# RchalYang/torchrl

Measured on AMD Instinct MI355X. Metric: env_steps_per_sec_ppo_2048env_halfcheetah_shape, higher is better.
Workload: dtype f32

## Files before the change

torchrl_amd/build.py:

```python
import os
import shutil
import subprocess
import sys

HERE = os.path.dirname(os.path.abspath(__file__))
CSRC = os.path.join(HERE, "csrc")
LIB_DIR = os.path.join(HERE, "lib")
LIB = os.path.join(LIB_DIR, "libtrl_hip.so")
NOISE_LIB = os.path.join(LIB_DIR, "libtrl_noise.so")
NOISE_SRC = "trl_noise_ext.cpp"
SOURCES = ["trl_host.cpp", "trl_mtjump.cpp", "k_gae.hip", "k_gather.hip", "k_ppo.hip", "k_ppo_generic.hip", "k_categorical.hip", "k_gauss_sd.hip", "k_layernorm.hip", "k_vmpo.hip", "k_trpo.hip", "k_rollout.hip", "k_gemm.hip", "k_mlp3.hip", "k_conv1.hip", "k_conv_dx.hip", "k_sac.hip", "k_conv.hip", "k_dqn.hip", "k_bootdqn.hip", "k_norm.hip", "k_frames.hip", "k_comm.hip", "k_peaks.hip"]
FLAGS = ["--offload-arch=gfx950", "-O3", "-std=c++17", "-fPIC", "-fno-gpu-rdc", "-Wall",
         "-Wno-unused-function", "-Wno-unused-variable"]


def _stale():
    if not os.path.exists(LIB):
        return True
    t = os.path.getmtime(LIB)
    deps = [os.path.join(CSRC, f) for f in os.listdir(CSRC) if f != NOISE_SRC]
    deps.append(os.path.join(os.path.dirname(HERE), "include", "trl_hip.h"))
    return any(os.path.getmtime(d) > t for d in deps)


def noise_helper_tag():
    import torch
    return "%s abi%d" % (torch.__version__, int(torch.compiled_with_cxx11_abi()))


def noise_helper_built_for(path=None):
    import re
    try:
        with open(path or NOISE_LIB, "rb") as f:
            blob = f.read()
    except OSError:
        return None
    m = re.search(rb"(\d+\.\d+[^\x00 ]* abi[01])\x00", blob)
    return m.group(1).decode() if m else None


def build_noise_helper(force=False, verbose=True):
    src = os.path.join(CSRC, NOISE_SRC)
    if not force and os.path.exists(NOISE_LIB) and os.path.getmtime(NOISE_LIB) >= os.path.getmtime(src) \
            and noise_helper_built_for() == noise_helper_tag():
        return NOISE_LIB
    try:
        import torch
        from torch.utils import cpp_extension as ce
        gxx = shutil.which("g++")
        if gxx is None:
            raise RuntimeError("g++ not found")
        libp = ce.library_paths()
        cmd = [gxx, "-O2", "-std=c++17", "-shared", "-fPIC"] + ["-I" + i for i in ce.include_paths()] + \
              ["-D_GLIBCXX_USE_CXX11_ABI=%d" % int(torch.compiled_with_cxx11_abi()),
               '-DTRL_NOISE_BUILT_FOR="%s"' % noise_helper_tag(), src, "-o", NOISE_LIB] + \
              ["-L" + p for p in libp] + ["-ltorch_cpu", "-lc10"] + ["-Wl,-rpath," + p for p in libp]
        os.makedirs(LIB_DIR, exist_ok=True)
        res = subprocess.run(cmd, stdout=subprocess.PIPE, stderr=subprocess.STDOUT)
        if res.returncode != 0:
            raise RuntimeError(res.stdout.decode()[-2000:])
        if verbose:
            print("built", NOISE_LIB)
        return NOISE_LIB
    except Exception as exc:
        if verbose:
            print("libtrl_noise.so not built (%s): the reference-noise chunks are drawn from Python threads" % (exc,))
        return None


def build(force=False, verbose=True, extra_flags=(), lib=None):
    LIB = lib or globals()["LIB"]
    FLAGS = globals()["FLAGS"] + list(extra_flags)
    if not lib:
        build_noise_helper(force=force, verbose=verbose)
    if not force and not lib and not _stale():
        return LIB
    hipcc = shutil.which("hipcc") or "/opt/rocm/bin/hipcc"
    if not os.path.exists(hipcc):
        raise RuntimeError("hipcc not found: libtrl_hip.so cannot be built")
    os.makedirs(LIB_DIR, exist_ok=True)
    objs = []
    procs = []
    for src in SOURCES:
        obj = os.path.join(LIB_DIR, os.path.splitext(src)[0] + (".exp.o" if lib else ".o"))
        cmd = [hipcc] + FLAGS + (["-x", "hip"] if src.endswith(".cpp") else []) + \
              ["-c", os.path.join(CSRC, src), "-o", obj]
        procs.append((src, subprocess.Popen(cmd, stdout=subprocess.PIPE, stderr=subprocess.STDOUT)))
        objs.append(obj)
    for src, p in procs:
        out, _ = p.communicate()
        if p.returncode != 0:
            raise RuntimeError("hipcc failed on %s:\n%s" % (src, out.decode()))
        if verbose and out.strip():
            print(out.decode())
    cmd = [hipcc, "--offload-arch=gfx950", "-shared", "-fPIC", "-o", LIB] + objs + ["-ldl"]
    subprocess.check_call(cmd)
    for o in objs:
        os.remove(o)
    if verbose:
        print("built", LIB)
    return LIB


if __name__ == "__main__":
    if "--exp" in sys.argv:
        k = sys.argv.index("--exp")
        build(force=True, extra_flags=sys.argv[k + 2:], lib=os.path.join(LIB_DIR, "libtrl_hip_%s.so" % sys.argv[k + 1]))
    else:
        build(force="--force" in sys.argv)
```

torchrl_amd/csrc/k_gae.hip:

```cpp
#include "trl_common.h"

#define ENV_TILE 8
#define T_CHUNK 256
#define GAE_THREADS 256

template <int MODE>
__global__ __launch_bounds__(GAE_THREADS) void gae_scan_kernel(
    const float* __restrict__ rew, const float* __restrict__ val, const float* __restrict__ term,
    const float* __restrict__ tl, const float* __restrict__ last_v, const float* __restrict__ last_t, float* __restrict__ adv,
    float* __restrict__ ret, int T, int N, float gamma, float tau, int tl_filter) {
  constexpr int LDT = T_CHUNK + 1;
  __shared__ float s_a[ENV_TILE * LDT];
  __shared__ float s_c[ENV_TILE * LDT];
  __shared__ float s_carry[ENV_TILE];

  const int tid = threadIdx.x, lane = tid & 63, wave = tid >> 6;
  const int G = gridDim.x, xcd = blockIdx.x & 7, q = blockIdx.x >> 3;
  int first = 0;
  for (int y = 0; y < xcd; ++y) first += (G - y + 7) >> 3;
  const int n0 = (first + q) * ENV_TILE;
  const int e_ld = tid % ENV_TILE, t_ld = tid / ENV_TILE;
  const int n_ld = n0 + e_ld;

  __shared__ float s_lastv[ENV_TILE];
  if (tid < ENV_TILE) {
    float lv = 0.0f;
    if (n0 + tid < N) lv = last_v[n0 + tid] * (last_t ? 1.0f - last_t[n0 + tid] : 1.0f);
    s_lastv[tid] = lv;
    s_carry[tid] = (MODE == 0) ? 0.0f : lv;
  }

  for (int t_hi = T; t_hi > 0; t_hi -= T_CHUNK) {
    const int t_lo = max(0, t_hi - T_CHUNK);
    const int len = t_hi - t_lo;
    __syncthreads();
    constexpr int TPT = T_CHUNK / (GAE_THREADS / ENV_TILE);
    float lr[TPT], lv[TPT], ld[TPT], ltl[TPT], lvn[TPT];
#pragma unroll
    for (int q = 0; q < TPT; ++q) {
      const int tt = t_ld + q * (GAE_THREADS / ENV_TILE);
      const int t = t_lo + tt;
      const bool ok = tt < len && n_ld < N;
      const size_t i = ok ? (size_t)t * N + n_ld : 0;
      lr[q] = ok ? rew[i] : 0.0f;
      lv[q] = ok ? val[i] : 0.0f;
      ld[q] = ok ? term[i] : 0.0f;
      ltl[q] = (ok && tl_filter) ? tl[i] : 0.0f;
      lvn[q] = (MODE == 0 && ok && t + 1 < T) ? val[i + N] : 0.0f;
    }
#pragma unroll
    for (int q = 0; q < TPT; ++q) {
      const int tt = t_ld + q * (GAE_THREADS / ENV_TILE);
      if (tt < len) {
        const int t = t_lo + tt;
        float a = 0.f, c = 0.f;
        if (n_ld < N) {
          const float r = lr[q], v = lv[q], nd = 1.0f - ld[q];
          const float tlv = ltl[q];
          if (MODE == 0) {
            const float vn = (t + 1 < T) ? lvn[q] : s_lastv[e_ld];
            const float f = 1.0f - tlv;
            a = (r + nd * gamma * vn - v) * f;
            c = nd * gamma * tau * f;
          } else {
            a = r + tlv * v;
            c = nd * gamma * (1.0f - tlv);
          }
        }
        s_a[e_ld * LDT + tt] = a;
        s_c[e_ld * LDT + tt] = c;
      }
    }
    __syncthreads();
    const int seg = (len + 63) >> 6;
    constexpr int EPW = ENV_TILE / (GAE_THREADS / 64);
    const int lo = min(lane * seg, len), hi = min(lo + seg, len);
    float fa[EPW], fb[EPW];
#pragma unroll
    for (int u = 0; u < EPW; ++u) {
      const float* pa = s_a + (wave + u * (GAE_THREADS / 64)) * LDT;
      const float* pc = s_c + (wave + u * (GAE_THREADS / 64)) * LDT;
      fa[u] = 0.f; fb[u] = 1.f;
      for (int t = hi - 1; t >= lo; --t) { fa[u] = pa[t] + pc[t] * fa[u]; fb[u] = pc[t] * fb[u]; }
    }
#pragma unroll
    for (int o = 1; o < 64; o <<= 1) {
      float a2[EPW], b2[EPW];
#pragma unroll
      for (int u = 0; u < EPW; ++u) { a2[u] = __shfl_down(fa[u], o, 64); b2[u] = __shfl_down(fb[u], o, 64); }
      if (lane + o < 64) {
#pragma unroll
        for (int u = 0; u < EPW; ++u) { fa[u] = fa[u] + fb[u] * a2[u]; fb[u] = fb[u] * b2[u]; }
      }
    }
#pragma unroll
    for (int u = 0; u < EPW; ++u) {
      const int e = wave + u * (GAE_THREADS / 64);
      float* pa = s_a + e * LDT;
      const float* pc = s_c + e * LDT;
      const float carry = s_carry[e];
      const float a_nx = __shfl_down(fa[u], 1, 64), b_nx = __shfl_down(fb[u], 1, 64);
      float y = (lane == 63) ? carry : (a_nx + b_nx * carry);
      for (int t = hi - 1; t >= lo; --t) { y = pa[t] + pc[t] * y; pa[t] = y; }
      const float y0 = __shfl(fa[u], 0, 64) + __shfl(fb[u], 0, 64) * carry;
      if (lane == 0) s_carry[e] = y0;
    }
    __syncthreads();
#pragma unroll
    for (int q = 0; q < TPT; ++q) {
      const int tt = t_ld + q * (GAE_THREADS / ENV_TILE);
      if (tt < len && n_ld < N) {
        const size_t i = (size_t)(t_lo + tt) * N + n_ld;
        const float y = s_a[e_ld * LDT + tt], v = lv[q];
        if (MODE == 0) { adv[i] = y; ret[i] = y + v; }
        else           { ret[i] = y; adv[i] = y - v; }
      }
    }
  }
}

static int launch_scan(int mode, const float* rew, const float* val, const float* term, const float* tl,
                       const float* last_v, const float* last_t, float* adv, float* ret, int T, int N,
                       float gamma, float tau, int tl_filter, void* stream) {
  if (!rew || !val || !term || !last_v || !adv || !ret) { trl_set_error("gae: null pointer"); return TRL_EINVAL; }
  if (tl_filter && !tl) { trl_set_error("gae: tl_filter set but time_limits is null"); return TRL_EINVAL; }
  if (T < 0 || N < 0) { trl_set_error("gae: negative size"); return TRL_EINVAL; }
  if (T == 0 || N == 0) return TRL_OK;
  dim3 grid(trl_ceil_div(N, ENV_TILE)), block(GAE_THREADS);
  hipStream_t s = (hipStream_t)stream;
  if (mode == 0)
    hipLaunchKernelGGL(gae_scan_kernel<0>, grid, block, 0, s, rew, val, term, tl, last_v, last_t, adv, ret, T, N, gamma, tau, tl_filter);
  else
    hipLaunchKernelGGL(gae_scan_kernel<1>, grid, block, 0, s, rew, val, term, tl, last_v, last_t, adv, ret, T, N, gamma, tau, tl_filter);
  TRL_LAUNCH_CHECK();
  return TRL_OK;
}

extern "C" int trl_gae_f32(const float* rewards, const float* values, const float* terminals,
                           const float* time_limits, const float* last_value, const float* last_terminal,
                           float* advs, float* rets, int T, int N, float gamma, float tau, int tl_filter,
                           void* stream) {
  return launch_scan(0, rewards, values, terminals, time_limits, last_value, last_terminal, advs, rets, T, N, gamma, tau, tl_filter, stream);
}

extern "C" int trl_discount_reward_f32(const float* rewards, const float* values, const float* terminals,
                                       const float* time_limits, const float* last_value,
                                       const float* last_terminal, float* advs, float* rets, int T, int N,
                                       float gamma, int tl_filter, void* stream) {
  return launch_scan(1, rewards, values, terminals, time_limits, last_value, last_terminal, advs, rets, T, N, gamma, 0.f, tl_filter, stream);
}
```

torchrl_amd/csrc/k_ppo.hip:

```cpp
#include <cstdlib>
#include "trl_common.h"
#include "trl_mlp.h"
#include "trl_head.h"
#include "trl_comm.h"

struct PpoDev {
  const float *obs, *acts, *advs, *rets, *old_values, *old_logp;
  const int64_t* row_idx;
  int rows_mb, N;
  const double* adv_raw;
  double n_global;
  const float *pf_params, *vf_params;
  float clip_para, entropy_coeff;
  int clipped_value_loss, tanh_action;
  int loss_mode;
  float* partial;
  double* scal_partial;
  int n_wg, n_pf, p_stride;
  int D, A;
};

template <int D, int H, int A> struct PpoShape {
  static_assert(H == 64 && D > 16 && D <= 32 && A <= 8, "instantiated for 16 < D <= 32, H == 64, A <= 8");
  static constexpr int P_PF = MlpFlat<D, H, A>::P_PF, P_VF = MlpFlat<D, H, 1>::P_VF;
  static constexpr int P_STRIDE = ((P_PF > P_VF ? P_PF : P_VF) + 63) & ~63;
};

#define WV_WAVES 4
#ifdef TRL_EXP_CLK
#define WCLK_DECL long long clk_prev = clock64(); float clk_acc[24]; for (int q_ = 0; q_ < 24; ++q_) clk_acc[q_] = 0.f;
#define WCLK(ph) { __builtin_amdgcn_sched_barrier(0); const long long c_ = clock64(); clk_acc[ph] += (float)(c_ - clk_prev); clk_prev = c_; __builtin_amdgcn_sched_barrier(0); }
#else
#define WCLK_DECL
#define WCLK(ph)
#endif
#define WV_THREADS (64 * WV_WAVES)
#define LDT 20
#define LDW 68

template <int D, int H, int A> struct WvShape {
  static_assert(H == 64 && (D == 17 || D == 32) && A <= 8, "instantiated for D == 17 / 32, H == 64, A <= 8");
  static constexpr int O_W2F = 0, O_W2B = H * LDW, O_B1 = 2 * H * LDW, O_B2 = O_B1 + H, O_SCR = O_B2 + H;
  static constexpr int O_H1 = 0, O_H2 = H * LDT, O_DZ2 = 2 * H * LDT, O_DO = 3 * H * LDT, WSCR = O_DO + 16 * LDT;
  static constexpr int P_STRIDE = PpoShape<D, H, A>::P_STRIDE;
  static constexpr int MAIN = O_SCR + WV_WAVES * WSCR;
  static constexpr int XS_W2 = 0, XS_W1 = 16, XS_W1B = 20, XS_W3 = D > 17 ? 24 : 20, XS_PF = XS_W3 + 4, XS_VF = XS_W3;
  static constexpr int XSC_PF = 3 * H + 32, XSC_VF = 4 * H + 16;
  static constexpr int XCH_PF = WV_WAVES * (XS_PF * 256 + XSC_PF), XCH_VF = WV_WAVES * (XS_VF * 256 + XSC_VF);
  static constexpr int XCH = XCH_PF > XCH_VF ? XCH_PF : XCH_VF;
  static constexpr int O_IMG = MAIN > XCH ? MAIN : XCH;
  static constexpr int IMG_HEAD = 8 * H + 16;
  static constexpr int IMG = (H * D + 2 * H + IMG_HEAD + WV_THREADS - 1) / WV_THREADS * WV_THREADS;
  static constexpr int LDS_FLOATS = O_IMG + IMG;
};

template <int D, int H, int A> struct WvShapeSD : WvShape<D, H, A> {
  static constexpr int P_PF_SD = H * D + H + H * H + H + 2 * A * H + 2 * A, P_VF = MlpFlat<D, H, 1>::P_VF;
  static constexpr int P_STRIDE = ((P_PF_SD > P_VF ? P_PF_SD : P_VF) + 63) & ~63;
  static constexpr int IMG_HEAD = 16 * H + 16;
  static constexpr int IMG = (H * D + 2 * H + IMG_HEAD + WV_THREADS - 1) / WV_THREADS * WV_THREADS;
  static constexpr int LDS_FLOATS = WvShape<D, H, A>::O_IMG + IMG;
};
template <int D, int H, int A, int HEAD> struct WvPick { using T = WvShape<D, H, A>; };
template <int D, int H, int A> struct WvPick<D, H, A, HEAD_SD> { using T = WvShapeSD<D, H, A>; };
#define SD_HALF_LOG_2PI_PLUS_HALF 1.4189385332046727f

__device__ __forceinline__ f32x4 lds4(const float* p) { return *reinterpret_cast<const f32x4*>(p); }
__device__ __forceinline__ float row_sum16(float v) {
  v += __builtin_bit_cast(float, __builtin_amdgcn_update_dpp(0, __builtin_bit_cast(int, v), 0x128, 0xF, 0xF, false));
  v += __builtin_bit_cast(float, __builtin_amdgcn_update_dpp(0, __builtin_bit_cast(int, v), 0x124, 0xF, 0xF, false));
  v += __builtin_bit_cast(float, __builtin_amdgcn_update_dpp(0, __builtin_bit_cast(int, v), 0x122, 0xF, 0xF, false));
  v += __builtin_bit_cast(float, __builtin_amdgcn_update_dpp(0, __builtin_bit_cast(int, v), 0x121, 0xF, 0xF, false));
  return v;
}

template <int D, int H, int A, int ACT, bool IS_PF, bool CONTIG, bool RT, int HEAD = HEAD_GAUSS>
__device__ void ppo_wave_pass(const PpoDev& a, float* lds, int wg_in_net, int n_wg_net) {
  using S = typename WvPick<D, H, A, HEAD>::T;
  constexpr bool WIDE = D > 17,
                 CAT = HEAD == HEAD_CAT, SD = HEAD == HEAD_SD,
                 SDP = SD && IS_PF;
  static_assert(!WIDE || RT, "the wide tile exists as a runtime-dims instantiation only");
  static_assert(!CAT || (IS_PF && RT), "the categorical head is a policy pass of the runtime-dims kernels");
  static_assert(!SD || RT, "the state-dependent-std head belongs to the runtime-dims kernels");
  constexpr int AS = CAT ? 1 : 0;
  const int Dr = RT ? a.D : D;
  const int O = IS_PF ? (RT ? a.A : A) : 1;
  const int OH = SDP ? 2 * O : O;
  const int F_W1 = 0, F_B1 = H * Dr, F_W2 = F_B1 + H, F_B2 = F_W2 + H * H, F_W3 = F_B2 + H, F_B3 = F_W3 + OH * H,
            F_LS = F_B3 + OH, F_END = (CAT || SDP) ? F_LS : F_LS + O;
  auto sd_has = [&](int o) -> bool { return (o & 7) < O; };
  auto sd_row = [&](int o) -> int { return o < 8 ? o : O + (o - 8); };
  const int PS = RT ? a.p_stride : S::P_STRIDE;
  const int tid = threadIdx.x, lane = tid & 63, wave = tid >> 6;
  const int j = lane & 15, g = lane >> 4, i = j;
  const float* gp = IS_PF ? a.pf_params : a.vf_params;
  WCLK_DECL
  float* W2F = lds + S::O_W2F;
  float* W2B = lds + S::O_W2B;
  float* scr = lds + S::O_SCR + wave * S::WSCR;
  float* H1S = scr + S::O_H1;
  float* H2S = scr + S::O_H2;
  float* DZ2S = scr + S::O_DZ2;
  float* DOS = scr + S::O_DO;

  const double adv_s1 = IS_PF ? a.adv_raw[0] : 0.0, adv_s2 = IS_PF ? a.adv_raw[1] : 0.0;
  const int B = a.rows_mb * a.N;
  const int n_tiles = (B + 15) / 16;
  const int tile_stride = n_wg_net * WV_WAVES;

  float xq[5], xtq[4], lq[6];
  float xq2[4], xtq2[4];
  int tile = wg_in_net * WV_WAVES + wave;
  const int tpr = a.N >> 4;
  int p1r = 0, p1c = 0, p2r = 0, p2c = 0, st_r = 0, st_c = 0;
  int64_t ridx1 = 0, ridx2 = 0;
  bool fv[4], fv2[4];
  const bool f16 = !WIDE && (!RT || Dr > 16), jv = !RT || i < Dr, jv2 = WIDE && 16 + i < Dr;
  const unsigned ox16 = (unsigned)(j * Dr + (f16 ? 16 : 0)) * 4u, os = (unsigned)j * 4u;
  unsigned oxq[4], oxt[4], oa_[4], oxq2[4], oxt2[4];
#pragma unroll
  for (int q = 0; q < 4; ++q) {
    fv[q] = !RT || 4 * g + q < Dr;
    fv2[q] = WIDE && 16 + 4 * g + q < Dr;
    oxq[q] = (unsigned)(j * Dr + (fv[q] ? 4 * g + q : 0)) * 4u;
    oxt[q] = (unsigned)((4 * g + q) * Dr + (jv ? i : 0)) * 4u;
    oxq2[q] = (unsigned)(j * Dr + (fv2[q] ? 16 + 4 * g + q : 0)) * 4u;
    oxt2[q] = (unsigned)((4 * g + q) * Dr + (jv2 ? 16 + i : 0)) * 4u;
    if constexpr (SDP) oa_[q] = (unsigned)(j * O + (4 * (g & 1) + q < O ? 4 * (g & 1) + q : 0)) * 4u;
    else oa_[q] = CAT ? (unsigned)j * 4u : (unsigned)(j * O + (4 * g + q < O ? 4 * g + q : 0)) * 4u;
  }
  auto ldb = [](const float* base, unsigned byte_off) -> float {
    return *reinterpret_cast<const float*>(reinterpret_cast<const char*>(base) + byte_off);
  };
  auto pos_advance = [&](int& r, int& c) { c += st_c; r += st_r; if (c >= tpr) { c -= tpr; ++r; } };
  auto load_ridx = [&](int r) -> int64_t {
    const int rr = r < a.rows_mb ? r : 0;
    return a.row_idx ? a.row_idx[rr] : (int64_t)rr;
  };
  auto fetch_contig = [&](int64_t ridx, int r, int c) {
    const int64_t cell0 = (r < a.rows_mb) ? ridx * a.N + 16 * c : 0;
    const float* ob = a.obs + cell0 * Dr;
#pragma unroll
    for (int q = 0; q < 4; ++q) xq[q] = ldb(ob, oxq[q]);
    xq[4] = ldb(ob, ox16);
#pragma unroll
    for (int q = 0; q < 4; ++q) xtq[q] = ldb(ob, oxt[q]);
    if constexpr (WIDE) {
#pragma unroll
      for (int q = 0; q < 4; ++q) { xq2[q] = ldb(ob, oxq2[q]); xtq2[q] = ldb(ob, oxt2[q]); }
    }
    if constexpr (IS_PF) {
      const float* ab = a.acts + cell0 * (CAT ? AS : O);
      if constexpr (CAT) { lq[0] = ldb(ab, oa_[0]); lq[1] = lq[2] = lq[3] = 0.0f; }
      else {
#pragma unroll
        for (int q = 0; q < 4; ++q) lq[q] = ldb(ab, oa_[q]);
      }
      lq[4] = ldb(a.advs + cell0, os);
      lq[5] = a.old_logp ? ldb(a.old_logp + cell0, os) : 0.0f;
    } else {
      lq[0] = lq[1] = lq[2] = lq[3] = 0.0f;
      lq[4] = ldb(a.rets + cell0, os);
      lq[5] = a.clipped_value_loss ? ldb(a.old_values + cell0, os) : 0.0f;
    }
  };
  auto row_of = [&](int smp, int& e) -> int { const int sm = smp < B ? smp : 0; const int r = sm / a.N; e = sm - r * a.N; return r; };
  auto fetch_inputs = [&](int64_t p, int s0) {
#pragma unroll
    for (int r = 0; r < 4; ++r) xq[r] = a.obs[p * Dr + (fv[r] ? 4 * g + r : 0)];
    xq[4] = a.obs[p * Dr + (f16 ? 16 : 0)];
#pragma unroll
    for (int q = 0; q < 4; ++q) {
      const int sj = 4 * g + q;
      const int64_t pr = __shfl(p, sj, 64);
      xtq[q] = a.obs[(s0 + sj < B ? pr : 0) * Dr + (jv ? i : 0)];
      if constexpr (WIDE) {
        xq2[q] = a.obs[p * Dr + (fv2[q] ? 16 + 4 * g + q : 0)];
        xtq2[q] = a.obs[(s0 + sj < B ? pr : 0) * Dr + (jv2 ? 16 + i : 0)];
      }
    }
    if constexpr (IS_PF) {
      if constexpr (CAT) { lq[0] = a.acts[p]; lq[1] = lq[2] = lq[3] = 0.0f; }
      else if constexpr (SDP) {
#pragma unroll
        for (int r = 0; r < 4; ++r) lq[r] = a.acts[p * O + (4 * (g & 1) + r < O ? 4 * (g & 1) + r : 0)];
      } else {
#pragma unroll
        for (int r = 0; r < 4; ++r) lq[r] = a.acts[p * O + (4 * g + r < O ? 4 * g + r : 0)];
      }
      lq[4] = a.advs[p]; lq[5] = a.old_logp ? a.old_logp[p] : 0.0f;
    } else {
      lq[0] = lq[1] = lq[2] = lq[3] = 0.0f;
      lq[4] = a.rets[p]; lq[5] = a.clipped_value_loss ? a.old_values[p] : 0.0f;
    }
  };
  int e_nn = 0;
  int64_t ridx_nn = 0;
  auto fetch_row = [&](int t) {
    const int r = row_of(t * 16 + j, e_nn);
    ridx_nn = a.row_idx ? a.row_idx[r] : (int64_t)r;
  };
  auto prefetch_next = [&](int nt) {
    if constexpr (CONTIG) {
      fetch_contig(ridx1, p1r, p1c);
      p1r = p2r; p1c = p2c; ridx1 = ridx2;
      pos_advance(p2r, p2c);
      ridx2 = load_ridx(p2r);
    } else {
      const int64_t pn = (nt * 16 + j < B) ? ridx_nn * a.N + e_nn : 0;
      fetch_inputs(pn, nt * 16);
      fetch_row(nt + tile_stride);
    }
  };
  int r0 = 0, c0 = 0;
  int64_t ridx0 = 0;
  if constexpr (CONTIG) {
    const int t0 = __builtin_amdgcn_readfirstlane(tile);
    const int ts = __builtin_amdgcn_readfirstlane(tile_stride);
    st_r = ts / tpr; st_c = ts - st_r * tpr;
    r0 = t0 / tpr; c0 = t0 - (t0 / tpr) * tpr;
    ridx0 = load_ridx(r0);
  } else {
    fetch_row(tile);
  }
  __builtin_amdgcn_sched_barrier(0);
  constexpr int NV = H * H / (4 * WV_THREADS);
  f32x4 wv[NV], wt[NV];
  const int tc = tid & 63, tq = tid >> 6;
  {
    static_assert(WV_THREADS == 256 && H == 64, "the transposed staging maps (column, 4 rows) onto 256 threads");
    const bool w2_al = !RT || ((reinterpret_cast<uintptr_t>(gp + F_W2) & 15) == 0);
#pragma unroll
    for (int t = 0; t < NV; ++t) {
      if (w2_al) wv[t] = *reinterpret_cast<const f32x4*>(gp + F_W2 + 4 * (tid + WV_THREADS * t));
      else {
#pragma unroll
        for (int x = 0; x < 4; ++x) wv[t][x] = gp[F_W2 + 4 * (tid + WV_THREADS * t) + x];
      }
    }
#pragma unroll
    for (int t = 0; t < NV; ++t)
#pragma unroll
      for (int x = 0; x < 4; ++x) wt[t][x] = gp[F_W2 + (4 * (tq + 4 * t) + x) * H + tc];
  }
  constexpr int NI = S::IMG / WV_THREADS;
  const int n_img = F_W2 + (F_END - F_B2);
  float im[NI];
#pragma unroll
  for (int k = 0; k < NI; ++k) {
    const int e = tid + WV_THREADS * k, ec = e < n_img ? e : n_img - 1;
    im[k] = gp[ec < F_W2 ? ec : ec + H * H];
  }
  __builtin_amdgcn_sched_barrier(0);
  if constexpr (CONTIG) {
    fetch_contig(ridx0, r0, c0);
    p1r = r0; p1c = c0;
    pos_advance(p1r, p1c);
    ridx1 = load_ridx(p1r);
    p2r = p1r; p2c = p1c;
    pos_advance(p2r, p2c);
    ridx2 = load_ridx(p2r);
  } else {
    const int64_t p0 = (tile * 16 + j < B) ? ridx_nn * a.N + e_nn : 0;
    fetch_inputs(p0, tile * 16);
    fetch_row(tile + tile_stride);
  }
#ifdef TRL_EXP_CLK
  WCLK(22)
  __builtin_amdgcn_s_waitcnt(0);
  WCLK(23)
#endif
  for (int e = lane; e < 16 * LDT; e += 64) DOS[e] = 0.0f;
#pragma unroll
  for (int t = 0; t < NV; ++t) {
    const int e = 4 * (tid + WV_THREADS * t), r = e / H, c = e - r * H;
    *reinterpret_cast<f32x4*>(W2F + r * LDW + c) = wv[t];
    *reinterpret_cast<f32x4*>(W2B + tc * LDW + 4 * (tq + 4 * t)) = wt[t];
  }
  float* img = lds + S::O_IMG;
  constexpr int KB_LO = H * (WIDE ? 18 : RT ? 2 : D) / WV_THREADS, KB_HI = (H * D + 2 * H - 1) / WV_THREADS;
#pragma unroll
  for (int k = 0; k < NI; ++k) {
    const int e = tid + WV_THREADS * k;
    img[e] = im[k];
    if (k >= KB_LO && k <= KB_HI && e >= F_B1 && e < F_B1 + 2 * H) lds[S::O_B1 + (e - F_B1)] = im[k];
  }
  static_assert(S::O_B2 == S::O_B1 + H, "b1 | b2 are stored as one run");
  __syncthreads();

  const int I_W3 = F_W3 - H * H, I_B3 = F_B3 - H * H, I_LS = F_LS - H * H;
  float w1[4][5], w3h[4][4], w3t[4][4];
  float w1b[4][4];
  float b3v[4], lsraw[4];
#pragma unroll
  for (int so = 0; so < 4; ++so) {
    const int row = 16 * so + i;
#pragma unroll
    for (int r = 0; r < 4; ++r) w1[so][r] = img[F_W1 + row * Dr + (fv[r] ? 4 * g + r : 0)];
    w1[so][4] = img[F_W1 + row * Dr + (f16 ? 16 : 0)];
    if constexpr (WIDE) {
#pragma unroll
      for (int r = 0; r < 4; ++r) w1b[so][r] = img[F_W1 + row * Dr + (fv2[r] ? 16 + 4 * g + r : 0)];
    }
#pragma unroll
    for (int r = 0; r < 4; ++r) {
      const int o = 4 * g + r;
      if constexpr (SDP) {
        w3h[so][r] = img[I_W3 + (sd_has(i) ? sd_row(i) : 0) * H + 16 * so + 4 * g + r];
        w3t[so][r] = img[I_W3 + (sd_has(o) ? sd_row(o) : 0) * H + row];
      } else if constexpr (IS_PF) {
        w3h[so][r] = img[I_W3 + (i < O ? i : 0) * H + 16 * so + 4 * g + r];
        w3t[so][r] = img[I_W3 + (o < O ? o : 0) * H + row];
      } else {
        w3h[so][r] = img[I_W3 + 16 * so + 4 * g + r];
        w3t[so][r] = 0.0f;
      }
    }
  }
#pragma unroll
  for (int r = 0; r < 4; ++r) {
    const int o = 4 * g + r;
    if constexpr (IS_PF && !CAT && !SDP) lsraw[r] = img[I_LS + (o < O ? o : 0)];
    else lsraw[r] = 0.0f;
    if constexpr (SDP) b3v[r] = img[I_B3 + (sd_has(o) ? sd_row(o) : 0)];
    else b3v[r] = img[I_B3 + (o < O ? o : 0)];
  }
  const float vb3 = IS_PF ? 0.0f : img[I_B3];
  __builtin_amdgcn_sched_barrier(0);
#pragma unroll
  for (int so = 0; so < 4; ++so) {
#pragma unroll
    for (int r = 0; r < 4; ++r) {
      const int o = 4 * g + r;
      w1[so][r] = fv[r] ? w1[so][r] : 0.0f;
      if constexpr (WIDE) w1b[so][r] = fv2[r] ? w1b[so][r] : 0.0f;
      if constexpr (SDP) {
        w3h[so][r] = sd_has(i) ? w3h[so][r] : 0.0f;
        w3t[so][r] = sd_has(o) ? w3t[so][r] : 0.0f;
      } else if constexpr (IS_PF) {
        w3h[so][r] = (i < O) ? w3h[so][r] : 0.0f;
        w3t[so][r] = (o < O) ? w3t[so][r] : 0.0f;
      }
    }
    w1[so][4] = (g == 0 && f16) ? w1[so][4] : 0.0f;
  }
  float lsv[4], ivv[4], lspass[4];
#pragma unroll
  for (int r = 0; r < 4; ++r) {
    const int o = 4 * g + r;
    const float raw = (IS_PF && !CAT && !SDP && o < O) ? lsraw[r] : 0.0f;
    lsv[r] = fminf(fmaxf(raw, -20.0f), 2.0f);
    ivv[r] = __expf(-2.0f * lsv[r]);
    lspass[r] = (raw >= -20.0f && raw <= 2.0f) ? 1.0f : 0.0f;
    if constexpr (SDP) b3v[r] = sd_has(o) ? b3v[r] : 0.0f;
    else b3v[r] = (o < O) ? b3v[r] : 0.0f;
  }

  const double ng = a.n_global;
  const double adv_mean = adv_s1 / ng;
  const double adv_var = (adv_s2 - adv_s1 * adv_s1 / ng) / (ng - 1.0);
  const float adv_mu = (float)adv_mean;
  const float adv_rstd = 1.0f / ((float)sqrt(fmax(adv_var, 0.0)) + 1e-5f);
  const float inv_b = (float)(1.0 / ng);

  f32x4 gW2[4][4], gW1[4], gW3[4];
  f32x4 gW1b[4];
  float gb1[4][4], gb2[4][4], gW1c[4][4];
  float db3[4], dls[4], stv[7];
  float ent_sum = 0.0f;
  float sdst[8] = {0.0f, 0.0f, -INFINITY, -INFINITY, 0.0f, 0.0f, -INFINITY, -INFINITY}, sd_cnt = 0.0f;
#pragma unroll
  for (int x = 0; x < 4; ++x) {
    gW1[x] = gW3[x] = gW1b[x] = f32x4{0.f, 0.f, 0.f, 0.f};
    db3[x] = dls[x] = 0.0f;
#pragma unroll
    for (int y = 0; y < 4; ++y) { gW2[x][y] = f32x4{0.f, 0.f, 0.f, 0.f}; gb1[x][y] = gb2[x][y] = gW1c[x][y] = 0.0f; }
  }
#pragma unroll
  for (int k = 0; k < 7; ++k) stv[k] = (k >= 2 && k <= 5) ? -INFINITY : 0.0f;

  WCLK(0)
  for (; tile < n_tiles; tile += tile_stride) {
    const int s = tile * 16 + j;
    const bool valid = CONTIG ? true : (s < B);
    float xb[5], xt[4], lin[6], xb2[4], xt2[4];
#pragma unroll
    for (int r = 0; r < 4; ++r) xb[r] = (valid && fv[r]) ? xq[r] : 0.0f;
    xb[4] = (valid && f16) ? xq[4] : 0.0f;
#pragma unroll
    for (int q = 0; q < 4; ++q) xt[q] = (jv && (CONTIG || tile * 16 + 4 * g + q < B)) ? xtq[q] : 0.0f;
    if constexpr (WIDE) {
#pragma unroll
      for (int q = 0; q < 4; ++q) {
        xb2[q] = (valid && fv2[q]) ? xq2[q] : 0.0f;
        xt2[q] = (jv2 && (CONTIG || tile * 16 + 4 * g + q < B)) ? xtq2[q] : 0.0f;
      }
    }
#pragma unroll
    for (int q = 0; q < 6; ++q) lin[q] = lq[q];
    const float x16 = xb[4];

#define PIN_DS() __builtin_amdgcn_sched_barrier(0x676)
    f32x4 h1[4], h2[4];
    f32x4 wq[4], bq;
#pragma unroll
    for (int so = 0; so < 4; ++so) h1[so] = lds4(lds + S::O_B1 + 16 * so + 4 * g);
#pragma unroll
    for (int sl = 0; sl < 4; ++sl) wq[sl] = lds4(W2F + i * LDW + 16 * sl + 4 * g);
    bq = lds4(lds + S::O_B2 + 4 * g);
    PIN_DS();
    WCLK(9)
#pragma unroll
    for (int q = 0; q < (WIDE ? 4 : 5); ++q)
#pragma unroll
      for (int so = 0; so < 4; ++so) h1[so] = mfma16(w1[so][q], xb[q], h1[so]);
    if constexpr (WIDE) {
#pragma unroll
      for (int q = 0; q < 4; ++q)
#pragma unroll
        for (int so = 0; so < 4; ++so) h1[so] = mfma16(w1b[so][q], xb2[q], h1[so]);
    }
    WCLK(10)
#pragma unroll
    for (int so = 0; so < 4; ++so)
#pragma unroll
      for (int r = 0; r < 4; ++r) {
        h1[so][r] = act_fn<ACT>(h1[so][r]);
        H1S[(16 * so + 4 * g + r) * LDT + j] = h1[so][r];
      }
    WCLK(1)
#pragma unroll
    for (int so = 0; so < 4; ++so) {
      f32x4 acc = bq;
      f32x4 wc[4];
#pragma unroll
      for (int sl = 0; sl < 4; ++sl) wc[sl] = wq[sl];
      if (so < 3) {
#pragma unroll
        for (int sl = 0; sl < 4; ++sl) wq[sl] = lds4(W2F + (16 * (so + 1) + i) * LDW + 16 * sl + 4 * g);
        bq = lds4(lds + S::O_B2 + 16 * (so + 1) + 4 * g);
        PIN_DS();
      }
#pragma unroll
      for (int sl = 0; sl < 4; ++sl)
#pragma unroll
        for (int r = 0; r < 4; ++r) acc = mfma16(wc[sl][r], h1[sl][r], acc);
      WCLK(11)
#pragma unroll
      for (int r = 0; r < 4; ++r) h2[so][r] = act_fn<ACT>(acc[r]);
      WCLK(12)
    }

    prefetch_next(tile + tile_stride);
    WCLK(2)
    f32x4 dz2[4];
    f32x4 wb[4];
    if constexpr (IS_PF) {
#pragma unroll
      for (int so = 0; so < 4; ++so)
#pragma unroll
        for (int r = 0; r < 4; ++r) H2S[(16 * so + 4 * g + r) * LDT + j] = h2[so][r];
      f32x4 oa = f32x4{b3v[0], b3v[1], b3v[2], b3v[3]}, ob = f32x4{0.f, 0.f, 0.f, 0.f};
#pragma unroll
      for (int sl = 0; sl < 4; sl += 2)
#pragma unroll
        for (int r = 0; r < 4; ++r) { oa = mfma16(w3h[sl][r], h2[sl][r], oa); ob = mfma16(w3h[sl + 1][r], h2[sl + 1][r], ob); }
      WCLK(14)
      float zc[4], lp = 0.0f;
      float pk[4], lpk[4], ent = 0.0f;
      int ai = 0;
      if constexpr (CAT) {
        float lg[4], ek[4], m = -INFINITY;
#pragma unroll
        for (int r = 0; r < 4; ++r) {
          lg[r] = oa[r] + ob[r];
          m = (4 * g + r < O) ? fmaxf(m, lg[r]) : m;
        }
        m = fmaxf(m, __shfl_xor(m, 16, 64));
        m = g < 2 ? m : 0.0f;
#pragma unroll
        for (int r = 0; r < 4; ++r) ek[r] = (4 * g + r < O) ? expf(lg[r] - m) : 0.0f;
        const float c_own = ((ek[0] + ek[1]) + ek[2]) + ek[3];
        const float c_lo = __shfl_xor(c_own, 16, 64);
        float Ssum = g == 1 ? (((c_lo + ek[0]) + ek[1]) + ek[2]) + ek[3] : c_own;
        const float S_hi = __shfl_xor(Ssum, 16, 64);
        Ssum = g == 0 ? S_hi : (g == 1 ? Ssum : 1.0f);
        const float logS = logf(Ssum);
        ai = min(max((int)lin[0], 0), O - 1);
#pragma unroll
        for (int r = 0; r < 4; ++r) {
          const bool has = 4 * g + r < O;
          lpk[r] = has ? (lg[r] - m) - logS : 0.0f;
          pk[r] = ek[r] / Ssum;
          lp += (has && 4 * g + r == ai) ? lpk[r] : 0.0f;
          ent -= pk[r] * lpk[r];
        }
        lp += __shfl_xor(lp, 16, 64);
        ent += __shfl_xor(ent, 16, 64);
      } else if constexpr (SDP) {
#pragma unroll
        for (int r = 0; r < 4; ++r) {
          const bool has = 4 * (g & 1) + r < O;
          const float mine = oa[r] + ob[r], oth = __shfl_xor(mine, 32, 64);
          const float mean = g < 2 ? mine : oth, raw = g < 2 ? oth : mine;
          lsv[r] = fminf(fmaxf(raw, -20.0f), 2.0f);
          ivv[r] = __expf(-2.0f * lsv[r]);
          lspass[r] = (raw >= -20.0f && raw <= 2.0f) ? 1.0f : 0.0f;
          const float t = gauss_logp_term((valid && has) ? lin[r] : 0.0f, has ? mean : 0.0f, ivv[r], lsv[r], a.tanh_action, zc[r]);
          lp += has ? t : 0.0f;
          ent += has ? SD_HALF_LOG_2PI_PLUS_HALF + lsv[r] : 0.0f;
          zc[r] = has ? zc[r] : 0.0f;
        }
        lp += __shfl_xor(lp, 16, 64);
        ent += __shfl_xor(ent, 16, 64);
      } else {
#pragma unroll
      for (int r = 0; r < 4; ++r) {
        const bool has = 4 * g + r < O;
        const float t = gauss_logp_term((valid && has) ? lin[r] : 0.0f, has ? oa[r] + ob[r] : 0.0f, ivv[r], lsv[r],
                                        a.tanh_action, zc[r]);
        lp += has ? t : 0.0f;
        zc[r] = has ? zc[r] : 0.0f;
      }
      WCLK(18)
      lp += __shfl_xor(lp, 16, 64);
      }
      WCLK(19)
      const float advn = valid ? (lin[4] - adv_mu) * adv_rstd : 0.0f;
      float ratio, s1, s2, g_lp;
      if (a.loss_mode == TRL_LOSS_A2C) {
        ratio = 1.0f;
        s1 = s2 = lp * advn;
        g_lp = (valid && (SDP || g < 2)) ? -advn * inv_b : 0.0f;
      } else {
        ratio = __expf(lp - lin[5]);
        s1 = ratio * advn;
        s2 = fminf(fmaxf(ratio, 1.0f - a.clip_para), 1.0f + a.clip_para) * advn;
        g_lp = (valid && (SDP || g < 2) && s1 <= s2) ? -advn * ratio * inv_b : 0.0f;
      }
      WCLK(20)
      float dout[4];
      if constexpr (CAT) {
        const float ce = a.entropy_coeff * inv_b;
#pragma unroll
        for (int r = 0; r < 4; ++r) {
          const bool own = valid && g < 2 && 4 * g + r < O;
          dout[r] = own ? g_lp * ((4 * g + r == ai ? 1.0f : 0.0f) - pk[r]) + ce * pk[r] * (lpk[r] + ent) : 0.0f;
          db3[r] += dout[r];
          if (g < 2) DOS[(4 * g + r) * LDT + j] = dout[r];
        }
        if (valid && g == 0) ent_sum += ent;
      } else if constexpr (SDP) {
        const float ce = a.entropy_coeff * inv_b;
#pragma unroll
        for (int r = 0; r < 4; ++r) {
          const bool own = valid && 4 * (g & 1) + r < O;
          const float dm = g_lp * zc[r] * ivv[r], dr = lspass[r] * (g_lp * (zc[r] * zc[r] * ivv[r] - 1.0f) - ce);
          dout[r] = own ? (g < 2 ? dm : dr) : 0.0f;
          db3[r] += dout[r];
          DOS[(4 * g + r) * LDT + j] = dout[r];
          if (own && g < 2) {
            const float x = lsv[r], ex = expf(x);
            sdst[0] += x; sdst[1] = fmaf(x, x, sdst[1]); sdst[2] = fmaxf(sdst[2], x); sdst[3] = fmaxf(sdst[3], -x);
            sdst[4] += ex; sdst[5] = fmaf(ex, ex, sdst[5]); sdst[6] = fmaxf(sdst[6], ex); sdst[7] = fmaxf(sdst[7], -ex);
          }
        }
        if (valid && g == 0) { ent_sum += ent; sd_cnt += 1.0f; }
      } else {
#pragma unroll
      for (int r = 0; r < 4; ++r) {
        const bool own = valid && g < 2 && 4 * g + r < O;
        dout[r] = own ? g_lp * zc[r] * ivv[r] : 0.0f;
        db3[r] += dout[r];
        dls[r] += own ? lspass[r] * (g_lp * (zc[r] * zc[r] * ivv[r] - 1.0f) - a.entropy_coeff * inv_b) : 0.0f;
        if (g < 2) DOS[(4 * g + r) * LDT + j] = dout[r];
      }
      }
      WCLK(21)
      if (valid && g == 0) {
        stv[0] += lp; stv[1] = fmaf(lp, lp, stv[1]); stv[6] -= fminf(s1, s2);
        stv[2] = fmaxf(stv[2], lp); stv[3] = fmaxf(stv[3], -lp);
        stv[4] = fmaxf(stv[4], ratio); stv[5] = fmaxf(stv[5], -ratio);
      }
      WCLK(15)
      const f32x4 da = lds4(DOS + i * LDT + 4 * g);
      f32x4 hb3[4];
#pragma unroll
      for (int so = 0; so < 4; ++so) hb3[so] = lds4(H2S + (16 * so + j) * LDT + 4 * g);
#pragma unroll
      for (int so = 0; so < 4; ++so) wb[so] = lds4(W2B + (16 * so + i) * LDW + 4 * g);
      PIN_DS();
#pragma unroll
      for (int so = 0; so < 4; ++so) dz2[so] = f32x4{0.f, 0.f, 0.f, 0.f};
#pragma unroll
      for (int r = 0; r < 4; ++r)
#pragma unroll
        for (int so = 0; so < 4; ++so) dz2[so] = mfma16(w3t[so][r], dout[r], dz2[so]);
#pragma unroll
      for (int so = 0; so < 4; ++so)
#pragma unroll
        for (int q = 0; q < 4; ++q) gW3[so] = mfma16(da[q], hb3[so][q], gW3[so]);
      WCLK(16)
    } else {
#pragma unroll
      for (int so = 0; so < 4; ++so) wb[so] = lds4(W2B + (16 * so + i) * LDW + 4 * g);
      PIN_DS();
      float v = 0.0f;
#pragma unroll
      for (int so = 0; so < 4; ++so)
#pragma unroll
        for (int r = 0; r < 4; ++r) v = fmaf(w3h[so][r], h2[so][r], v);
      v += __shfl_xor(v, 16, 64);
      v += __shfl_xor(v, 32, 64);
      v += vb3;
      const float R = lin[4];
      float dv, l;
      if (a.clipped_value_loss) {
        const float vo = lin[5];
        const float dc = v - vo;
        const float vc = vo + fminf(fmaxf(dc, -a.clip_para), a.clip_para);
        const float l1 = (v - R) * (v - R), l2 = (vc - R) * (vc - R);
        const float wa = l1 > l2 ? 1.0f : (l1 == l2 ? 0.5f : 0.0f), wb_ = 1.0f - wa;
        const float pass = (dc >= -a.clip_para && dc <= a.clip_para) ? 1.0f : 0.0f;
        l = 0.5f * fmaxf(l1, l2);
        dv = inv_b * (wa * (v - R) + wb_ * pass * (vc - R));
      } else {
        l = (v - R) * (v - R);
        dv = 2.0f * (v - R) * inv_b;
      }
      dv = valid ? dv : 0.0f;
      if (valid && g == 0) {
        stv[6] += l; db3[0] += dv;
        stv[0] += v; stv[1] = fmaf(v, v, stv[1]); stv[2] = fmaxf(stv[2], v); stv[3] = fmaxf(stv[3], -v);
      }
#pragma unroll
      for (int so = 0; so < 4; ++so)
#pragma unroll
        for (int r = 0; r < 4; ++r) {
          dz2[so][r] = dv * w3h[so][r];
          gW3[so][r] = fmaf(dv, h2[so][r], gW3[so][r]);
        }
    }
#pragma unroll
    for (int so = 0; so < 4; ++so)
#pragma unroll
      for (int r = 0; r < 4; ++r) {
        dz2[so][r] *= act_grad<ACT>(h2[so][r]);
        gb2[so][r] += dz2[so][r];
        DZ2S[(16 * so + 4 * g + r) * LDT + j] = dz2[so][r];
      }

    WCLK(3)
    f32x4 dz1[4];
    f32x4 hb[4], za2;
#pragma unroll
    for (int so = 0; so < 4; ++so) dz1[so] = f32x4{0.f, 0.f, 0.f, 0.f};
#pragma unroll
    for (int sl = 0; sl < 4; ++sl) {
      f32x4 w[4];
#pragma unroll
      for (int so = 0; so < 4; ++so) w[so] = wb[so];
      if (sl < 3) {
#pragma unroll
        for (int so = 0; so < 4; ++so) wb[so] = lds4(W2B + (16 * so + i) * LDW + 16 * (sl + 1) + 4 * g);
      } else {
#pragma unroll
        for (int c = 0; c < 4; ++c) hb[c] = lds4(H1S + (16 * c + j) * LDT + 4 * g);
        za2 = lds4(DZ2S + i * LDT + 4 * g);
      }
      PIN_DS();
#pragma unroll
      for (int r = 0; r < 4; ++r)
#pragma unroll
        for (int so = 0; so < 4; ++so) dz1[so] = mfma16(w[so][r], dz2[sl][r], dz1[so]);
    }
    WCLK(17)
#pragma unroll
    for (int so = 0; so < 4; ++so)
#pragma unroll
      for (int r = 0; r < 4; ++r) {
        dz1[so][r] *= act_grad<ACT>(h1[so][r]);
        gb1[so][r] += dz1[so][r];
        if constexpr (!WIDE) gW1c[so][r] = fmaf(dz1[so][r], x16, gW1c[so][r]);
        H2S[(16 * so + 4 * g + r) * LDT + j] = dz1[so][r];
      }
    f32x4 za1[4];
#pragma unroll
    for (int so = 0; so < 4; ++so) za1[so] = lds4(H2S + (16 * so + i) * LDT + 4 * g);
    PIN_DS();

    WCLK(4)
#pragma unroll
    for (int so = 0; so < 4; ++so) {
      const f32x4 za = za2;
      if (so < 3) { za2 = lds4(DZ2S + (16 * (so + 1) + i) * LDT + 4 * g); PIN_DS(); }
#pragma unroll
      for (int q = 0; q < 4; ++q)
#pragma unroll
        for (int c = 0; c < 4; ++c) gW2[so][c] = mfma16(za[q], hb[c][q], gW2[so][c]);
    }
    WCLK(5)
#pragma unroll
    for (int so = 0; so < 4; ++so)
#pragma unroll
      for (int q = 0; q < 4; ++q) gW1[so] = mfma16(za1[so][q], xt[q], gW1[so]);
    if constexpr (WIDE) {
#pragma unroll
      for (int so = 0; so < 4; ++so)
#pragma unroll
        for (int q = 0; q < 4; ++q) gW1b[so] = mfma16(za1[so][q], xt2[q], gW1b[so]);
    }
#undef PIN_DS
    WCLK(6)
  }

  __syncthreads();
  const int wg = blockIdx.x;
  {
    constexpr int NS = IS_PF ? S::XS_PF : S::XS_VF, SC = IS_PF ? S::XSC_PF : S::XSC_VF;
    f32x4* xch = reinterpret_cast<f32x4*>(lds);
    float* xsc = lds + WV_WAVES * NS * 256;
    f32x4* xw = xch + (wave * NS) * 64 + lane;
    float* sw = xsc + wave * SC;
    {
      constexpr int NK = IS_PF ? 3 : 4, TS = 17;
      static_assert(NK * 16 <= 64 && NK * 16 * TS <= NS * 64, "one task per lane, inside the wave's own region");
      f32x4* tr = xch + (wave * NS) * 64;
#pragma unroll
      for (int so = 0; so < 4; ++so) {
        f32x4* te = tr + (4 * so + g) * TS + j;
        te[0] = f32x4{gb1[so][0], gb1[so][1], gb1[so][2], gb1[so][3]};
        te[16 * TS] = f32x4{gb2[so][0], gb2[so][1], gb2[so][2], gb2[so][3]};
        te[32 * TS] = f32x4{gW1c[so][0], gW1c[so][1], gW1c[so][2], gW1c[so][3]};
        if constexpr (!IS_PF) te[48 * TS] = gW3[so];
      }
      if (lane < NK * 16) {
        const f32x4* x = tr + lane * TS;
        const f32x4 even = ((x[0] + x[8]) + (x[4] + x[12])) + ((x[2] + x[10]) + (x[6] + x[14]));
        const f32x4 odd = ((x[1] + x[9]) + (x[5] + x[13])) + ((x[3] + x[11]) + (x[7] + x[15]));
        *reinterpret_cast<f32x4*>(sw + 4 * lane) = even + odd;
      }
    }
#pragma unroll
    for (int so = 0; so < 4; ++so) {
#pragma unroll
      for (int c = 0; c < 4; ++c) xw[(S::XS_W2 + 4 * so + c) * 64] = gW2[so][c];
      xw[(S::XS_W1 + so) * 64] = gW1[so];
      if constexpr (WIDE) xw[(S::XS_W1B + so) * 64] = gW1b[so];
      if constexpr (IS_PF) xw[(S::XS_W3 + so) * 64] = gW3[so];
    }
#pragma unroll
    for (int r = 0; r < 4; ++r) {
      const int o = 4 * g + r;
      const float b3 = row_sum16(db3[r]), dl = row_sum16(dls[r]);
      if (j == 0) {
        if constexpr (IS_PF) { sw[3 * H + o] = b3; sw[3 * H + 16 + o] = dl; }
        else sw[4 * H + o] = b3;
      }
    }
    WCLK(7)
    __syncthreads();
    float* prow = a.partial + (size_t)wg * a.p_stride;
    auto fold4 = [&](int slot) -> f32x4 {
      const f32x4* p = xch + slot * 64 + lane;
      f32x4 acc = p[0];
#pragma unroll
      for (int w = 1; w < WV_WAVES; ++w) acc += p[w * NS * 64];
      return acc;
    };
    {
      const int so = wave;
      f32x4 t2[4];
#pragma unroll
      for (int c = 0; c < 4; ++c) t2[c] = fold4(S::XS_W2 + 4 * so + c);
      const f32x4 t1 = fold4(S::XS_W1 + so);
      f32x4 t1b = f32x4{0.f, 0.f, 0.f, 0.f}, t3 = f32x4{0.f, 0.f, 0.f, 0.f};
      if constexpr (WIDE) t1b = fold4(S::XS_W1B + so);
      if constexpr (IS_PF) t3 = fold4(S::XS_W3 + so);
#pragma unroll
      for (int r = 0; r < 4; ++r) {
        const int f = 16 * so + 4 * g + r;
#pragma unroll
        for (int c = 0; c < 4; ++c) prow[F_W2 + f * H + 16 * c + j] = t2[c][r];
        if (jv) prow[F_W1 + f * Dr + j] = t1[r];
        if (WIDE && jv2) prow[F_W1 + f * Dr + 16 + j] = t1b[r];
        if constexpr (IS_PF) {
          const int o = 4 * g + r;
          if constexpr (SDP) { if (sd_has(o)) prow[F_W3 + sd_row(o) * H + 16 * so + j] = t3[r]; }
          else if (o < O) prow[F_W3 + o * H + 16 * so + j] = t3[r];
        }
      }
    }
    for (int k = tid; k < SC; k += WV_THREADS) {
      float acc = xsc[k];
#pragma unroll
      for (int w = 1; w < WV_WAVES; ++w) acc += xsc[w * SC + k];
      const int q = k & (H - 1);
      int dst = -1;
      if (k < H) dst = F_B1 + q;
      else if (k < 2 * H) dst = F_B2 + q;
      else if (k < 3 * H) { if (f16) dst = F_W1 + q * Dr + 16; }
      else if constexpr (IS_PF) {
        const int o = q & 15;
        if (q < 16) { if constexpr (SDP) { if (sd_has(o)) dst = F_B3 + sd_row(o); } else if (o < O) dst = F_B3 + o; }
        else if (!CAT && !SDP && o < O) dst = F_LS + o;
      } else {
        if (k < 4 * H) dst = F_W3 + q;
        else if (q < O) dst = F_B3 + q;
      }
      if (dst >= 0) prow[dst] = acc;
    }
    for (int e = (IS_PF ? F_END : F_LS) + tid; e < PS; e += WV_THREADS) prow[e] = 0.0f;
  }
  WCLK(8)
#ifdef TRL_EXP_CLK
  __syncthreads();
  if (tid == 0) for (int ph = 0; ph < 24; ++ph) a.partial[(size_t)wg * a.p_stride + PS - 40 + ph] = clk_acc[ph];
#endif
  __syncthreads();
  double* sred = reinterpret_cast<double*>(lds);
  {
    const bool own = g == 0;
    const double v0 = wave_sum(own ? (double)stv[0] : 0.0), v1 = wave_sum(own ? (double)stv[1] : 0.0),
                 v6 = wave_sum(own ? (double)stv[6] : 0.0);
    const float v2 = wave_max(own ? stv[2] : -INFINITY), v3 = wave_max(own ? stv[3] : -INFINITY),
                v4 = wave_max(own ? stv[4] : -INFINITY), v5 = wave_max(own ? stv[5] : -INFINITY);
    double v7 = 0.0;
    if constexpr (CAT || SDP) v7 = wave_sum(own ? (double)ent_sum : 0.0);
    if (lane == 0) {
      double* p = sred + wave * 8;
      p[0] = v0; p[1] = v1; p[2] = v2; p[3] = v3; p[4] = v4; p[5] = v5; p[6] = v6; p[7] = v7;
    }
    if constexpr (SDP) {
      double e[SD_SCAL];
#pragma unroll
      for (int k = 0; k < 8; ++k) e[k] = (k & 2) ? (double)wave_max(sdst[k]) : wave_sum((double)sdst[k]);
      e[8] = wave_sum((double)sd_cnt);
      if (lane == 0) {
#pragma unroll
        for (int k = 0; k < SD_SCAL; ++k) sred[WV_WAVES * 8 + wave * SD_SCAL + k] = k < 9 ? e[k] : 0.0;
      }
    }
  }
  __syncthreads();
  if (tid < 8) {
    double r = sred[tid];
    for (int w = 1; w < WV_WAVES; ++w) {
      const double o = sred[w * 8 + tid];
      r = (tid >= 2 && tid <= 5) ? fmax(r, o) : r + o;
    }
    a.scal_partial[(size_t)wg * 8 + tid] = r;
  }
  if constexpr (SDP) {
    if (tid >= 64 && tid < 64 + SD_SCAL) {
      const int k = tid - 64;
      double r = sred[WV_WAVES * 8 + k];
      for (int w = 1; w < WV_WAVES; ++w) {
        const double o = sred[WV_WAVES * 8 + w * SD_SCAL + k];
        r = (k < 8 && (k & 2)) ? fmax(r, o) : r + o;
      }
      a.scal_partial[(size_t)a.n_wg * 8 + (size_t)wg * SD_SCAL + k] = r;
    }
  }
}

#define RED_CHUNK 64
#ifndef RED_WAVES
#define RED_WAVES 8
#endif
#ifndef RED_DEPTH
#define RED_DEPTH 16
#endif
__device__ __forceinline__ float fold_chain_tree(float (&acc)[RED_DEPTH]) {
#pragma unroll
  for (int st = RED_DEPTH / 2; st > 0; st >>= 1)
#pragma unroll
    for (int k = 0; k < st; ++k) acc[k] += acc[k + st];
  return acc[0];
}
__device__ __forceinline__ float fold_rows_wave(const float* __restrict__ src, int nrow, int p_stride, int w, bool in_range) {
  float acc[RED_DEPTH];
#pragma unroll
  for (int k = 0; k < RED_DEPTH; ++k) acc[k] = 0.0f;
  if (in_range) {
    for (; w < nrow; w += RED_DEPTH * RED_WAVES) {
      float v[RED_DEPTH];
#pragma unroll
      for (int k = 0; k < RED_DEPTH; ++k) v[k] = (w + RED_WAVES * k < nrow) ? src[(size_t)(w + RED_WAVES * k) * p_stride] : 0.0f;
#pragma unroll
      for (int k = 0; k < RED_DEPTH; ++k) acc[k] += v[k];
    }
  }
  return fold_chain_tree(acc);
}
__device__ __forceinline__ float fold_waves_tree(const float (*s_acc)[RED_CHUNK], int lane) {
  float t4[RED_WAVES / 4];
#pragma unroll
  for (int q = 0; q < RED_WAVES / 4; ++q)
    t4[q] = (s_acc[4 * q][lane] + s_acc[4 * q + 1][lane]) + (s_acc[4 * q + 2][lane] + s_acc[4 * q + 3][lane]);
  float gval = t4[0];
#pragma unroll
  for (int q = 1; q < RED_WAVES / 4; ++q) gval += t4[q];
  return gval;
}
__device__ __noinline__ void fold_scalar_stats(const double* __restrict__ base, int nrow, int net, int lane,
                                                  double* __restrict__ info) {
  double v[7];
#pragma unroll
  for (int k = 0; k < 7; ++k) v[k] = (k >= 2 && k <= 5) ? -INFINITY : 0.0;
  for (int w0 = 0; w0 < nrow; w0 += 192) {
    double o[3][7];
#pragma unroll
    for (int q = 0; q < 3; ++q) {
      const int w = w0 + lane + 64 * q;
#pragma unroll
      for (int k = 0; k < 7; ++k) {
        double x = (k >= 2 && k <= 5) ? -INFINITY : 0.0;
        if (w < nrow) x = base[(size_t)w * 8 + k];
        o[q][k] = x;
      }
    }
#pragma unroll
    for (int q = 0; q < 3; ++q)
#pragma unroll
      for (int k = 0; k < 7; ++k) v[k] = (k >= 2 && k <= 5) ? fmax(v[k], o[q][k]) : v[k] + o[q][k];
  }
#pragma unroll
  for (int k = 0; k < 7; ++k) v[k] = (k >= 2 && k <= 5) ? wave_max(v[k]) : wave_sum(v[k]);
  if (lane == 0) {
    if (net == 0) {
      info[0] = v[6]; info[1] = v[0]; info[2] = v[1]; info[3] = v[2]; info[4] = v[3]; info[5] = v[4]; info[6] = v[5];
    } else {
      info[7] = v[6];
      info[12] = v[0]; info[13] = v[1]; info[14] = v[2]; info[15] = v[3];
    }
  }
}
__device__ __noinline__ void fold_logstd_stats_raw(float raw, int n_act, int lane, double* __restrict__ info) {
  const bool has = lane < n_act;
  const double x = has ? fmin(fmax((double)raw, -20.0), 2.0) : 0.0;
  const double e = has ? exp(x) : 0.0;
  const double sm = wave_sum(x), sq = wave_sum(x * x), es = wave_sum(e), eq = wave_sum(e * e);
  const double mx = wave_max(has ? x : -INFINITY), mn = -wave_max(has ? -x : -INFINITY);
  const double emx = wave_max(has ? e : -INFINITY), emn = -wave_max(has ? -e : -INFINITY);
  if (lane == 0) {
    const double mean = sm / n_act, em = es / n_act;
    info[8] = mean;
    info[9] = n_act > 1 ? sqrt(fmax((sq - sm * mean) / (n_act - 1), 0.0)) : NAN;
    info[10] = mx; info[11] = mn;
    info[16] = em;
    info[17] = n_act > 1 ? sqrt(fmax((eq - es * em) / (n_act - 1), 0.0)) : NAN;
    info[18] = emx; info[19] = emn;
  }
}
__device__ __forceinline__ void fold_logstd_stats(const float* __restrict__ logstd, int n_act, int lane, double* __restrict__ info) {
  fold_logstd_stats_raw(logstd[lane < n_act ? lane : 0], n_act, lane, info);
}

__device__ __noinline__ void fold_entropy_stats(const double* __restrict__ base, int nrow, int lane, double* __restrict__ info) {
  double v = 0.0;
  for (int w = lane; w < nrow; w += 64) v += base[(size_t)w * 8 + 7];
  v = wave_sum(v);
  if (lane == 0) {
    info[20] = v;
#pragma unroll
    for (int k = 0; k < 4; ++k) info[8 + k] = info[16 + k] = 0.0;
  }
}

__device__ __noinline__ void fold_sd_stats(const double* __restrict__ base, const double* __restrict__ sd, int nrow, int n_act,
                                           int lane, double* __restrict__ info) {
  double v[10];
#pragma unroll
  for (int k = 0; k < 10; ++k) v[k] = (k < 8 && (k & 2)) ? -INFINITY : 0.0;
  for (int w = lane; w < nrow; w += 64) {
#pragma unroll
    for (int k = 0; k < 9; ++k) {
      const double o = sd[(size_t)w * SD_SCAL + k];
      v[k] = (k < 8 && (k & 2)) ? fmax(v[k], o) : v[k] + o;
    }
    v[9] += base[(size_t)w * 8 + 7];
  }
#pragma unroll
  for (int k = 0; k < 10; ++k) v[k] = (k < 8 && (k & 2)) ? wave_max(v[k]) : wave_sum(v[k]);
  if (lane == 0) {
    const double n = v[8] * (double)n_act, lm = v[0] / n, em = v[4] / n;
    info[8] = lm; info[9] = n > 1.0 ? sqrt(fmax((v[1] - v[0] * lm) / (n - 1.0), 0.0)) : NAN;
    info[10] = v[2]; info[11] = -v[3];
    info[16] = em; info[17] = n > 1.0 ? sqrt(fmax((v[5] - v[4] * em) / (n - 1.0), 0.0)) : NAN;
    info[18] = v[6]; info[19] = -v[7];
    info[20] = v[9];
  }
}

template <int HEAD = HEAD_GAUSS>
__device__ __forceinline__ float ppo_reduce_block(const float* __restrict__ partial,
                                                  const double* __restrict__ scal, int n_wg, int n_pf,
                                                  int p_stride, int p_pf, int p_vf,
                                                  const float* __restrict__ logstd, int n_act,
                                                  float* __restrict__ grads, double* __restrict__ info,
                                                  int net, int bx, bool stats) {
  __shared__ float s_acc[RED_WAVES][RED_CHUNK];
  const int row0 = net == 0 ? 0 : n_pf, nrow = net == 0 ? n_pf : n_wg - n_pf;
  const int lane = threadIdx.x & 63, wave = threadIdx.x >> 6;
  const int p = bx * RED_CHUNK + lane;
  const int pn = net == 0 ? p_pf : p_vf;
  s_acc[wave][lane] = fold_rows_wave(partial + (size_t)row0 * p_stride + p, nrow, p_stride, wave, p < pn);
  __syncthreads();
  float gval = 0.0f;
  if (wave == 0 && p < pn) {
    gval = fold_waves_tree(s_acc, lane);
    grads[(net == 0 ? 0 : p_pf) + p] = gval;
  }
  if (stats && wave == 2) fold_scalar_stats(scal + (size_t)row0 * 8, nrow, net, lane, info);
  if constexpr (HEAD == HEAD_SD) {
    if (stats && net == 0 && wave == 3)
      fold_sd_stats(scal + (size_t)row0 * 8, scal + (size_t)n_wg * 8 + (size_t)row0 * SD_SCAL, nrow, n_act, lane, info);
  } else if constexpr (HEAD == HEAD_CAT) {
    if (stats && net == 0 && wave == 3) fold_entropy_stats(scal + (size_t)row0 * 8, nrow, lane, info);
  } else {
    if (stats && net == 0 && wave == 3 && logstd) fold_logstd_stats(logstd, n_act, lane, info);
  }
  return gval;
}

template <int HEAD = HEAD_GAUSS>
__global__ __launch_bounds__(64 * RED_WAVES) void ppo_reduce_kernel(const float* __restrict__ partial,
                                                         const double* __restrict__ scal, int n_wg, int n_pf,
                                                         int p_stride, int p_pf, int p_vf,
                                                         const float* __restrict__ logstd, int n_act,
                                                         float* __restrict__ grads, double* __restrict__ info) {
  ppo_reduce_block<HEAD>(partial, scal, n_wg, n_pf, p_stride, p_pf, p_vf, logstd, n_act, grads, info, blockIdx.y, blockIdx.x,
                        blockIdx.x == gridDim.x - 1);
}

struct AdamDev {
  float* params; const float* grads; float* m; float* v;
  int n_groups; int off[5]; float lr[4];
  float max_norm, beta1, beta2, eps, grad_scale, bc1, bc2_sqrt;
  float* norms_out;
  double* step_state;
  const float* device_lr;
  int self_tick;
};
__global__ __launch_bounds__(256) void clip_adam_kernel(AdamDev a) {
  __shared__ float s_part[4][4];
  __shared__ float s_coef[4];
  __shared__ float s_bc[2];
  const int tid = threadIdx.x, lane = tid & 63, wave = tid >> 6;
  if (a.step_state && tid == 0) {
    s_bc[0] = (float)(1.0 - a.step_state[1] * (double)a.beta1);
    s_bc[1] = (float)sqrt(1.0 - a.step_state[2] * (double)a.beta2);
    if (a.self_tick) {
      unsigned* cnt = reinterpret_cast<unsigned*>(a.step_state + 3);
      const unsigned before = __hip_atomic_fetch_add(cnt, 1u, __ATOMIC_ACQ_REL, __HIP_MEMORY_SCOPE_AGENT);
      if (before == gridDim.x - 1) {
        a.step_state[0] += 1.0; a.step_state[1] *= (double)a.beta1; a.step_state[2] *= (double)a.beta2;
        __hip_atomic_store(cnt, 0u, __ATOMIC_RELAXED, __HIP_MEMORY_SCOPE_AGENT);
      }
    }
  }
  const bool need_norm = a.max_norm > 0.0f;
  for (int g = 0; g < a.n_groups; ++g) {
    if (!need_norm) { if (lane == 0) s_part[g][wave] = 0.0f; continue; }
    float s0 = 0.f, s1 = 0.f, s2 = 0.f, s3 = 0.f;
    int e = a.off[g] + tid;
    for (; e + 7 * 256 < a.off[g + 1]; e += 8 * 256) {
      float x[8];
#pragma unroll
      for (int k = 0; k < 8; ++k) x[k] = a.grads[e + 256 * k];
      s0 = fmaf(x[0], x[0], s0); s1 = fmaf(x[1], x[1], s1); s2 = fmaf(x[2], x[2], s2); s3 = fmaf(x[3], x[3], s3);
      s0 = fmaf(x[4], x[4], s0); s1 = fmaf(x[5], x[5], s1); s2 = fmaf(x[6], x[6], s2); s3 = fmaf(x[7], x[7], s3);
    }
    for (; e < a.off[g + 1]; e += 256) { const float x = a.grads[e]; s0 = fmaf(x, x, s0); }
    float ss = wave_sum((s0 + s1) + (s2 + s3)) * a.grad_scale * a.grad_scale;
    if (lane == 0) s_part[g][wave] = ss;
  }
  __syncthreads();
  if (tid < a.n_groups) {
    const float norm = sqrtf(s_part[tid][0] + s_part[tid][1] + s_part[tid][2] + s_part[tid][3]);
    s_coef[tid] = (a.max_norm > 0.0f) ? fminf(a.max_norm / (norm + 1e-6f), 1.0f) : 1.0f;
    if (blockIdx.x == 0 && a.norms_out) a.norms_out[tid] = norm;
  }
  __syncthreads();
  const float bc1 = a.step_state ? s_bc[0] : a.bc1, bc2_sqrt = a.step_state ? s_bc[1] : a.bc2_sqrt;
  const int e = blockIdx.x * 256 + tid;
  if (e < a.off[a.n_groups]) {
    int g = 0;
    while (e >= a.off[g + 1]) ++g;
    const float gr = a.grads[e] * a.grad_scale * s_coef[g];
    const float m = a.beta1 * a.m[e] + (1.0f - a.beta1) * gr;
    const float v = a.beta2 * a.v[e] + (1.0f - a.beta2) * gr * gr;
    a.m[e] = m; a.v[e] = v;
    const float denom = sqrtf(v) / bc2_sqrt + a.eps;
    const float lr = a.device_lr ? a.device_lr[g] : a.lr[g];
    a.params[e] -= (lr / bc1) * (m / denom);
  }
}

__global__ void adam_tick_kernel(double* __restrict__ st, float beta1, float beta2) {
  st[0] += 1.0; st[1] *= (double)beta1; st[2] *= (double)beta2;
}

__device__ __forceinline__ void adam_element(const AdamDev& a, int e, float gr) {
  const float m = a.beta1 * a.m[e] + (1.0f - a.beta1) * gr;
  const float v = a.beta2 * a.v[e] + (1.0f - a.beta2) * gr * gr;
  a.m[e] = m; a.v[e] = v;
  const float denom = sqrtf(v) / a.bc2_sqrt + a.eps;
  int g = 0;
  while (e >= a.off[g + 1]) ++g;
  a.params[e] -= (a.lr[g] / a.bc1) * (m / denom);
}

template <bool LOOP, int HEAD = HEAD_GAUSS>
__global__ __launch_bounds__(64 * RED_WAVES, 4) void ppo_reduce_adam_kernel(const float* __restrict__ partial,
                                                              const double* __restrict__ scal, int n_wg, int n_pf,
                                                              int p_stride, int p_pf, int p_vf,
                                                              const float* __restrict__ logstd, int n_act,
                                                              float* __restrict__ grads, double* __restrict__ info,
                                                              AdamDev a, float* __restrict__ ws, unsigned epoch,
                                                              int device_state, int xrank, XrArgs xr, int only_net) {
  __shared__ float s_coef[2];
  __shared__ float s_hyper[4];
  const int tid = threadIdx.x, lane = tid & 63, wave = tid >> 6;
  const int nb = (p_stride + RED_CHUNK - 1) / RED_CHUNK, grid = gridDim.x, job0 = only_net == 1 ? nb : 0;
  const int n_jobs = only_net >= 0 ? job0 + nb : 2 * nb, blk = job0 + (int)blockIdx.x;
  double* bpow = reinterpret_cast<double*>(ws + 4);
  double b1p = 0.0, b2p = 0.0;
  float lr0 = 0.0f, lr1 = 0.0f;
  if (device_state) {
    epoch = reinterpret_cast<const unsigned*>(ws)[1] + 1u;
    if (tid == 64 * (RED_WAVES - 1)) { b1p = bpow[0]; b2p = bpow[1]; lr0 = ws[2]; lr1 = ws[3]; }
  }
  unsigned long long* slots = reinterpret_cast<unsigned long long*>(ws + 16);
  unsigned xepoch = 0u;
  if (xrank) {
    const unsigned e4 = __hip_atomic_load(xr.ctl + 4, __ATOMIC_RELAXED, __HIP_MEMORY_SCOPE_AGENT);
    const unsigned e6 = __hip_atomic_load(xr.ctl + 6, __ATOMIC_RELAXED, __HIP_MEMORY_SCOPE_AGENT);
    xepoch = (only_net == 0 ? e4 : only_net == 1 ? e6 : (e4 > e6 ? e4 : e6)) + 1u;
  }
  float gval0 = 0.0f;
  for (int j = blk; j < (LOOP ? n_jobs : blk + 1); j += LOOP ? grid : 1) {
    const int net = j / nb, bx = j - net * nb;
    if (j != blk) __syncthreads();
    float gval = ppo_reduce_block<HEAD>(partial, scal, n_wg, n_pf, p_stride, p_pf, p_vf, logstd, n_act, grads, info, net, bx, bx == nb - 1);
    if (wave == 0) {
      if (xrank) {
        const int pe = bx * RED_CHUNK + lane;
        const bool act = pe < (net == 0 ? p_pf : p_vf);
        const int ge = (net == 0 ? 0 : p_pf) + pe;
        gval = xr_allsum_f32(xr, xepoch, act ? ge : 0, gval, act);
        if (act) grads[ge] = gval;
      }
      if (j == blk) gval0 = gval;
      const float ss = wave_sum(gval * gval);
      if (lane == 0)
        __hip_atomic_store(slots + net * nb + bx, ((unsigned long long)epoch << 32) | (unsigned long long)__float_as_uint(ss),
                           __ATOMIC_RELAXED, __HIP_MEMORY_SCOPE_AGENT);
    }
  }
  if (device_state && tid == 64 * (RED_WAVES - 1)) {
    b1p *= (double)a.beta1; b2p *= (double)a.beta2;
    s_hyper[0] = (float)(1.0 - b1p);
    s_hyper[1] = (float)sqrt(1.0 - b2p);
    s_hyper[2] = lr0; s_hyper[3] = lr1;
  }
  if (LOOP && blk >= n_jobs) return;
  const int net_ = blk / nb, pe_ = (blk - net_ * nb) * RED_CHUNK + lane;
  const bool own_ = wave == 0 && pe_ < (net_ == 0 ? p_pf : p_vf);
  const int ge_ = (net_ == 0 ? 0 : p_pf) + pe_;
  float m_old = 0.0f, v_old = 0.0f, p_old = 0.0f;
  if (own_) { m_old = a.m[ge_]; v_old = a.v[ge_]; p_old = a.params[ge_]; }
  if (wave < 2 && (only_net < 0 || wave == only_net)) {
    float acc = 0.0f;
    for (int b = lane; b < nb; b += 64) {
      unsigned long long v;
      unsigned it = 0;
      unsigned long long t0 = 0;
      while ((unsigned)((v = __hip_atomic_load(slots + wave * nb + b, __ATOMIC_RELAXED, __HIP_MEMORY_SCOPE_AGENT)) >> 32) != epoch) {
        __builtin_amdgcn_s_sleep(1);
        if ((++it & 1023u) == 0) {
          const unsigned long long now = wall_clock64();
          if (t0 == 0) t0 = now;
          if (now - t0 > (xrank ? xr.wait_ticks + xr.wait_ticks / 4 : 200000000ull)) {
            __hip_atomic_store(reinterpret_cast<unsigned*>(ws), 1u, __ATOMIC_RELAXED, __HIP_MEMORY_SCOPE_AGENT);
            break;
          }
        }
      }
      acc += __uint_as_float((unsigned)v);
    }
    acc = wave_sum(acc) * a.grad_scale * a.grad_scale;
    if (lane == 0) {
      const float norm = sqrtf(acc);
      s_coef[wave] = (a.max_norm > 0.0f) ? fminf(a.max_norm / (norm + 1e-6f), 1.0f) : 1.0f;
      if (a.norms_out && blk == job0) a.norms_out[wave] = norm;
    }
  }
  __syncthreads();
  float bc1 = a.bc1, bc2_sqrt = a.bc2_sqrt, lr_pf = a.lr[0], lr_vf = a.lr[1];
  if (device_state) {
    bc1 = s_hyper[0]; bc2_sqrt = s_hyper[1]; lr_pf = s_hyper[2]; lr_vf = s_hyper[3];
    if (blk == job0) {
      if (tid == 0) __hip_atomic_store(reinterpret_cast<unsigned*>(ws) + 1, epoch, __ATOMIC_RELAXED, __HIP_MEMORY_SCOPE_AGENT);
      if (tid == 64 * (RED_WAVES - 1)) { bpow[0] = b1p; bpow[1] = b2p; }
    }
  }
  if (xrank && blk == job0 && tid == 0) {
    if (only_net != 1) __hip_atomic_store(xr.ctl + 4, xepoch, __ATOMIC_RELAXED, __HIP_MEMORY_SCOPE_AGENT);
    if (only_net != 0) __hip_atomic_store(xr.ctl + 6, xepoch, __ATOMIC_RELAXED, __HIP_MEMORY_SCOPE_AGENT);
  }
  const bool xfail = xrank && __hip_atomic_load(xr.ctl + 2, __ATOMIC_RELAXED, __HIP_MEMORY_SCOPE_AGENT) != 0u;
  if (wave == 0 && !xfail) {
    for (int j = blk; j < (LOOP ? n_jobs : blk + 1); j += LOOP ? grid : 1) {
      const int net = j / nb, pe = (j - net * nb) * RED_CHUNK + lane;
      if (pe >= (net == 0 ? p_pf : p_vf)) continue;
      const int ge = (net == 0 ? 0 : p_pf) + pe;
      const bool first = j == blk;
      const float g_ = first ? gval0 : grads[ge];
      const float mo = first ? m_old : a.m[ge], vo = first ? v_old : a.v[ge], po = first ? p_old : a.params[ge];
      const float gr = g_ * a.grad_scale * s_coef[net];
      const float m = a.beta1 * mo + (1.0f - a.beta1) * gr;
      const float v = a.beta2 * vo + (1.0f - a.beta2) * gr * gr;
      a.m[ge] = m; a.v[ge] = v;
      const float denom = sqrtf(v) / bc2_sqrt + a.eps;
      a.params[ge] = po - ((net == 0 ? lr_pf : lr_vf) / bc1) * (m / denom);
    }
  }
}

template <int D, int H, int A, int ACT, bool CONTIG, bool RT, int HEAD = HEAD_GAUSS>
__global__ __launch_bounds__(WV_THREADS, 1) void ppo_grad_wave_kernel(PpoDev a) {
  static_assert(HEAD == HEAD_GAUSS || RT, "categorical / state-dependent-std head: runtime-dims tiles");
  constexpr int HEAD_VF = HEAD == HEAD_CAT ? HEAD_GAUSS : HEAD;
  extern __shared__ __attribute__((aligned(16))) float lds[];
#ifdef TRL_CHAIN_CLK
  const unsigned long long clk0 = wall_clock64();
#endif
  if ((int)blockIdx.x < a.n_pf) ppo_wave_pass<D, H, A, ACT, true, CONTIG, RT, HEAD>(a, lds, blockIdx.x, a.n_pf);
  else                          ppo_wave_pass<D, H, A, ACT, false, CONTIG, RT, HEAD_VF>(a, lds, blockIdx.x - a.n_pf, a.n_wg - a.n_pf);
#ifdef TRL_CHAIN_CLK
  __syncthreads();
  if (threadIdx.x == 0) {
    a.scal_partial[(size_t)blockIdx.x * 8 + 7] = (double)wall_clock64();
    float* pad = a.partial + (size_t)blockIdx.x * a.p_stride + a.p_stride - 3;
    pad[0] = (float)(clk0 >> 40); pad[1] = (float)((clk0 >> 20) & 0xFFFFFull); pad[2] = (float)(clk0 & 0xFFFFFull);
  }
#endif
}

template <int D, int H, int O, int ACT>
__global__ __launch_bounds__(256) void mlp2_forward_kernel(const float* __restrict__ params,
                                                           const float* __restrict__ x,
                                                           float* __restrict__ out, int M) {
  using L = MlpLds<D, H, O>;
  constexpr int NT = H / 32, KS = ksteps_for(D);
  __shared__ __attribute__((aligned(16))) float sp[L::SIZE];
  const int tid = threadIdx.x, lane = tid & 63, wave = tid >> 6, i = lane & 31, hi = lane >> 5;
  L::load(sp, params, false, tid, 256);
  __syncthreads();
  const int n_tiles = (M + 31) / 32;
  for (int tile = blockIdx.x * 4 + wave; tile < n_tiles; tile += gridDim.x * 4) {
    const int s = tile * 32 + i;
    float xb[KS];
#pragma unroll
    for (int q = 0; q < KS; ++q) { const int k = rowmap(q, hi); xb[q] = (k < D && s < M) ? x[(size_t)s * D + k] : 0.0f; }
    f32x16 h1[NT], h2[NT];
#pragma unroll
    for (int mo = 0; mo < NT; ++mo)
      h1[mo] = act_tile<ACT>(layer1_tile<D, L::LD1, KS>(bias_tile(sp + L::B1 + 32 * mo, hi), sp + L::W1, mo, xb, i, hi));
#pragma unroll
    for (int mo = 0; mo < NT; ++mo)
      h2[mo] = act_tile<ACT>(layer_tile<NT, L::LD2>(bias_tile(sp + L::B2 + 32 * mo, hi), sp + L::W2, mo, h1, i, hi));
    float o[O];
    head_fwd<NT, H, O>(sp + L::W3, sp + L::B3, h2, hi, o);
    if (hi == 0 && s < M) {
#pragma unroll
      for (int c = 0; c < O; ++c) out[(size_t)s * O + c] = o[c];
    }
  }
}

#define SHAPE_IS(d, h, o) (D == (d) && H == (h) && A == (o))

static int ppo_stride_for(int D, int H, int A, int head) {
  if (head == HEAD_GAUSS && SHAPE_IS(17, 64, 6)) return PpoShape<17, 64, 6>::P_STRIDE;
  if (head_shape_ok(head, D, H, A)) {
    const int p_pf = ppo_p_pf(D, H, A, head), p_vf = ppo_p_vf(D, H);
    return ((p_pf > p_vf ? p_pf : p_vf) + 63) & ~63;
  }
  trl_set_error("trl_ppo_%spartial_stride: shape D=%d H=%d A=%d not instantiated (H == 64, 2 <= D <= 32, %d <= A <= %d)",
                HEADS[head].tag, D, H, A, HEADS[head].a_min, HEADS[head].a_max);
  return TRL_EUNSUPPORTED;
}
extern "C" int trl_ppo_partial_stride(int D, int H, int A) { return ppo_stride_for(D, H, A, HEAD_GAUSS); }
extern "C" int trl_ppo_cat_partial_stride(int D, int H, int A) { return ppo_stride_for(D, H, A, HEAD_CAT); }
extern "C" int trl_ppo_sd_partial_stride(int D, int H, int A) { return ppo_stride_for(D, H, A, HEAD_SD); }
extern "C" int trl_ppo_cat_supported(int D, int H, int A, int act) { return head_supported(HEAD_CAT, D, H, A, act); }
extern "C" int trl_ppo_sd_supported(int D, int H, int A, int act) { return head_supported(HEAD_SD, D, H, A, act); }
extern "C" int trl_ppo_sd_scalar_stride(void) { return HEADS[HEAD_SD].scal_stride; }
static_assert(WvShapeSD<17, 64, 8>::P_STRIDE == 6400 && WvShapeSD<32, 64, 8>::P_STRIDE == 7360, "SD image strides at A = 8");
static_assert(WvShapeSD<32, 64, 8>::LDS_FLOATS * sizeof(float) <= 160 * 1024, "the wide tile's exchange area fits the LDS");

template <int D, int H, int A, int ACT, bool CONTIG, bool RT, int HEAD>
static int launch_ppo_v(const PpoDev& d, hipStream_t s) {
  using S = typename WvPick<D, H, A, HEAD>::T;
  const size_t lds = S::LDS_FLOATS * sizeof(float);
  static bool attr_set = false;
  if (!attr_set) {
    hipError_t e = hipFuncSetAttribute((const void*)ppo_grad_wave_kernel<D, H, A, ACT, CONTIG, RT, HEAD>,
                                       hipFuncAttributeMaxDynamicSharedMemorySize, (int)lds);
    if (e != hipSuccess) { trl_set_error("ppo_grad: hipFuncSetAttribute: %s", hipGetErrorString(e)); return (int)e; }
    attr_set = true;
  }
  hipLaunchKernelGGL((ppo_grad_wave_kernel<D, H, A, ACT, CONTIG, RT, HEAD>), dim3(d.n_wg), dim3(WV_THREADS), lds, s, d);
  TRL_LAUNCH_CHECK();
  return TRL_OK;
}
template <int D, int H, int A, int ACT, bool RT, int HEAD = HEAD_GAUSS>
static int launch_ppo(const PpoDev& d, hipStream_t s) {
  return (d.N % 16 == 0) ? launch_ppo_v<D, H, A, ACT, true, RT, HEAD>(d, s) : launch_ppo_v<D, H, A, ACT, false, RT, HEAD>(d, s);
}

extern "C" int trl_ppo_wg_split(int D, int H, int A, int n_tiles, int n_wg) {
  if (n_wg < 2 || n_tiles <= 0) { trl_set_error("trl_ppo_wg_split: need n_wg >= 2 and n_tiles > 0"); return TRL_EINVAL; }
  const double c_pf = 16.7, c_vf = 12.1;
  int best = n_wg / 2;
  double best_t = 1e300;
  for (int x = 1; x < n_wg; ++x) {
    const double t_pf = (double)((n_tiles + WV_WAVES * x - 1) / (WV_WAVES * x)) * c_pf;
    const double t_vf = (double)((n_tiles + WV_WAVES * (n_wg - x) - 1) / (WV_WAVES * (n_wg - x))) * c_vf;
    const double t = t_pf > t_vf ? t_pf : t_vf;
    if (t < best_t - 1e-9 || (t < best_t + 1e-9 && abs(2 * x - n_wg) < abs(2 * best - n_wg))) { best_t = t; best = x; }
  }
  (void)D; (void)H; (void)A;
  return best;
}
static int resolve_pf_wgs(int n_wg, int n_wg_pf) { return n_wg_pf < 0 ? 0 : (n_wg_pf > 0 ? n_wg_pf : n_wg / 2); }

static int ppo_grad_launch(const trl_ppo_batch_t* p, void* stream, int head = HEAD_GAUSS) {
  if (!p) { trl_set_error("ppo_grad: null descriptor"); return TRL_EINVAL; }
  if (!head_supported(head, p->D, p->H, p->A, p->act)) {
    trl_set_error("ppo_%sgrad: shape D=%d H=%d A=%d act=%d not instantiated (H == 64, 2 <= D <= 32, %d <= A <= %d, Tanh / ReLU)",
                  HEADS[head].tag, p->D, p->H, p->A, p->act, HEADS[head].a_min, HEADS[head].a_max);
    return TRL_EUNSUPPORTED;
  }
  const bool reinforce = p->loss_mode == TRL_LOSS_REINFORCE;
  TRL_REQUIRE(p->obs && p->acts && p->advs && (p->rets || reinforce), "null rollout tensor");
  TRL_REQUIRE(p->loss_mode == TRL_LOSS_PPO_CLIP || p->loss_mode == TRL_LOSS_A2C || reinforce, "unknown loss_mode");
  TRL_REQUIRE(!reinforce || p->n_wg_pf == p->n_wg, "TRL_LOSS_REINFORCE runs in an all-policy launch only (n_wg_pf == n_wg)");
  TRL_REQUIRE(!reinforce || !p->clipped_value_loss, "TRL_LOSS_REINFORCE has no value loss: clipped_value_loss must be 0");
  TRL_REQUIRE(p->loss_mode != TRL_LOSS_PPO_CLIP || p->old_logp, "the clipped surrogate needs old_logp");
  TRL_REQUIRE(!p->clipped_value_loss || p->old_values, "the clipped value loss needs old_values");
  TRL_REQUIRE(p->adv_raw && (p->pf_params || p->vf_params) && p->partial && p->scal_partial, "null pointer");
  TRL_REQUIRE(p->rows_mb > 0 && p->N > 0, "empty minibatch");
  TRL_REQUIRE(p->n_wg >= 1 && (p->n_wg >= 2 || p->n_wg_pf == -1 || p->n_wg_pf == p->n_wg), "n_wg must be >= 2 (>= 1 for one network)");
  TRL_REQUIRE(p->n_wg_pf >= -1 && p->n_wg_pf <= p->n_wg, "n_wg_pf must be 0 (even split), in [1, n_wg], or -1 (value net only)");
  TRL_REQUIRE(p->n_wg_pf == p->n_wg || p->vf_params, "null value parameters");
  TRL_REQUIRE(p->n_wg_pf == -1 || p->pf_params, "null policy parameters");
  TRL_REQUIRE(p->n_global > 1.0, "n_global must exceed 1 (unbiased std)");
  const int D = p->D, H = p->H, A = p->A;
  TRL_REQUIRE(((uintptr_t)p->partial & 15) == 0 && (((uintptr_t)p->pf_params | (uintptr_t)p->vf_params) & 3) == 0,
              "partial rows must be 16-byte aligned, parameter blocks 4-byte aligned");
  TRL_REQUIRE(head != HEAD_GAUSS || !SHAPE_IS(17, 64, 6) || (((uintptr_t)p->pf_params | (uintptr_t)p->vf_params) & 15) == 0,
              "parameter blocks of the benchmark shape must be 16-byte aligned");
  PpoDev d;
  d.obs = p->obs; d.acts = p->acts; d.advs = p->advs; d.rets = p->rets; d.old_values = p->old_values;
  d.old_logp = p->old_logp; d.row_idx = p->row_idx; d.rows_mb = p->rows_mb; d.N = p->N;
  d.adv_raw = p->adv_raw; d.n_global = p->n_global; d.pf_params = p->pf_params; d.vf_params = p->vf_params;
  d.clip_para = p->clip_para; d.entropy_coeff = p->entropy_coeff;
  d.clipped_value_loss = p->clipped_value_loss; d.tanh_action = p->tanh_action;
  d.loss_mode = reinforce ? TRL_LOSS_A2C : p->loss_mode;
  d.partial = p->partial; d.scal_partial = p->scal_partial; d.n_wg = p->n_wg;
  d.n_pf = resolve_pf_wgs(p->n_wg, p->n_wg_pf);
  d.D = D; d.A = A;
  hipStream_t s = (hipStream_t)stream;
  d.p_stride = ppo_stride_for(D, H, A, head);
  if (head == HEAD_CAT) d.tanh_action = 0;
  if (head == HEAD_GAUSS && SHAPE_IS(17, 64, 6))
    return p->act == TRL_ACT_TANH ? launch_ppo<17, 64, 6, TRL_ACT_TANH, false>(d, s) : launch_ppo<17, 64, 6, TRL_ACT_RELU, false>(d, s);
  return with_head(head, [&](auto hd) {
    return with_tile_act(D, p->act, [&](auto tile, auto act) {
      return launch_ppo<decltype(tile)::value, 64, 8, decltype(act)::value, true, decltype(hd)::value>(d, s);
    });
  });
}

extern "C" int trl_ppo_minibatch_grad_f32(const trl_ppo_batch_t* p, void* stream) { return ppo_grad_launch(p, stream); }
extern "C" int trl_ppo_cat_minibatch_grad_f32(const trl_ppo_batch_t* p, void* stream) { return ppo_grad_launch(p, stream, HEAD_CAT); }
extern "C" int trl_ppo_sd_minibatch_grad_f32(const trl_ppo_batch_t* p, void* stream) { return ppo_grad_launch(p, stream, HEAD_SD); }

static int launch_reduce(const float* partial, const double* scal_partial, int n_wg, int n_wg_pf, int D, int H, int A,
                         const float* pf_params, float* grads, double* info, void* stream, int head) {
  TRL_REQUIRE(partial && scal_partial && grads && info, "null pointer");
  TRL_REQUIRE(n_wg >= 2 && n_wg_pf >= 0 && n_wg_pf < n_wg, "need n_wg >= 2 and n_wg_pf in [0, n_wg)");
  const int ps = ppo_stride_for(D, H, A, head);
  if (ps < 0) return ps;
  const int p_pf = ppo_p_pf(D, H, A, head), p_vf = ppo_p_vf(D, H);
  const float* logstd = (HEADS[head].logstd_tail && pf_params) ? pf_params + (p_pf - A) : nullptr;
  with_head(head, [&](auto hd) {
    hipLaunchKernelGGL(ppo_reduce_kernel<decltype(hd)::value>, dim3(trl_ceil_div(ps, RED_CHUNK), 2), dim3(64 * RED_WAVES), 0,
                       (hipStream_t)stream, partial, scal_partial, n_wg, resolve_pf_wgs(n_wg, n_wg_pf), ps, p_pf, p_vf,
                       logstd, A, grads, info);
    return 0;
  });
  TRL_LAUNCH_CHECK();
  return TRL_OK;
}
extern "C" int trl_ppo_reduce_f32(const float* partial, const double* scal_partial, int n_wg, int n_wg_pf, int D,
                                  int H, int A, const float* pf_params, float* grads, double* info, void* stream) {
  return launch_reduce(partial, scal_partial, n_wg, n_wg_pf, D, H, A, pf_params, grads, info, stream, HEAD_GAUSS);
}
extern "C" int trl_ppo_cat_reduce_f32(const float* partial, const double* scal_partial, int n_wg, int n_wg_pf, int D,
                                      int H, int A, const float* pf_params, float* grads, double* info, void* stream) {
  return launch_reduce(partial, scal_partial, n_wg, n_wg_pf, D, H, A, pf_params, grads, info, stream, HEAD_CAT);
}
extern "C" int trl_ppo_sd_reduce_f32(const float* partial, const double* scal_partial, int n_wg, int n_wg_pf, int D,
                                     int H, int A, const float* pf_params, float* grads, double* info, void* stream) {
  return launch_reduce(partial, scal_partial, n_wg, n_wg_pf, D, H, A, pf_params, grads, info, stream, HEAD_SD);
}

static int fill_adam(const trl_adam_t* p, AdamDev& d) {
  if (!p) { trl_set_error("clip_adam: null descriptor"); return TRL_EINVAL; }
  TRL_REQUIRE(p->params && p->grads && p->exp_avg && p->exp_avg_sq, "null pointer");
  TRL_REQUIRE(p->n_groups >= 1 && p->n_groups <= 4, "n_groups must be 1..4");
  TRL_REQUIRE(p->step_count >= 1 || p->device_state || p->step_state, "step_count starts at 1");
  d.params = p->params; d.grads = p->grads; d.m = p->exp_avg; d.v = p->exp_avg_sq;
  d.n_groups = p->n_groups; d.off[0] = 0;
  for (int g = 0; g < p->n_groups; ++g) {
    TRL_REQUIRE(p->group_sizes[g] >= 0, "negative group size");
    d.off[g + 1] = d.off[g] + p->group_sizes[g];
    d.lr[g] = p->group_lr[g];
  }
  for (int g = p->n_groups; g < 4; ++g) { d.off[g + 1] = d.off[g]; if (g < 4) d.lr[g] = 0.f; }
  d.max_norm = p->max_norm; d.beta1 = p->beta1; d.beta2 = p->beta2; d.eps = p->eps;
  d.grad_scale = p->grad_scale;
  d.bc1 = (float)(1.0 - pow((double)p->beta1, (double)p->step_count));
  d.bc2_sqrt = (float)sqrt(1.0 - pow((double)p->beta2, (double)p->step_count));
  d.norms_out = p->norms_out;
  d.step_state = p->step_state;
  d.device_lr = p->device_lr;
  d.self_tick = 0;
  return TRL_OK;
}

static int reduce_adam_workspace(int D, int H, int A, int head) {
  const int ps = ppo_stride_for(D, H, A, head);
  if (ps < 0) return ps;
  return 16 + 4 * trl_ceil_div(ps, RED_CHUNK);
}
extern "C" int trl_ppo_reduce_adam_workspace(int D, int H, int A) { return reduce_adam_workspace(D, H, A, HEAD_GAUSS); }
extern "C" int trl_ppo_cat_reduce_adam_workspace(int D, int H, int A) { return reduce_adam_workspace(D, H, A, HEAD_CAT); }
extern "C" int trl_ppo_sd_reduce_adam_workspace(int D, int H, int A) { return reduce_adam_workspace(D, H, A, HEAD_SD); }

static int launch_reduce_adam(const float* partial, const double* scal_partial, int n_wg, int n_wg_pf, int D, int H, int A,
                              float* grads, double* info, const trl_adam_t* adam, float* workspace, const XrArgs* xr,
                              int max_blocks, void* stream, int only_net = -1, int head = HEAD_GAUSS) {
  TRL_REQUIRE(partial && scal_partial && grads && info && workspace, "null pointer");
  TRL_REQUIRE(only_net >= 0 ? n_wg >= 1 : (n_wg >= 2 && n_wg_pf >= 0 && n_wg_pf < n_wg), "need n_wg >= 2 and n_wg_pf in [0, n_wg)");
  const int ps = ppo_stride_for(D, H, A, head);
  if (ps < 0) return ps;
  AdamDev d;
  int rc = fill_adam(adam, d);
  if (rc) return rc;
  const int p_pf = ppo_p_pf(D, H, A, head), p_vf = ppo_p_vf(D, H);
  TRL_REQUIRE((adam->n_groups == 2 && adam->group_sizes[0] == p_pf && adam->group_sizes[1] == p_vf) ||
              (only_net == 0 && !xr && adam->n_groups == 1 && adam->group_sizes[0] == p_pf),
              "optimiser groups must be [policy | value] of this shape");
  TRL_REQUIRE(adam->grads == grads, "adam->grads must be the reduce output");
  TRL_REQUIRE(!xr || p_pf + p_vf <= TRL_XR_CAP_GRAD, "gradient exceeds the peer buffer");
  XrArgs none;
  none.rank = 0; none.world = 1; none.ctl = nullptr; none.wait_ticks = 0;
  for (int r = 0; r < TRL_MAX_RANKS; ++r) none.peer[r] = nullptr;
  int grid = (only_net >= 0 ? 1 : 2) * trl_ceil_div(ps, RED_CHUNK);
  if (max_blocks > 0 && max_blocks < grid) grid = max_blocks;
  const int n_pf = only_net == 0 ? n_wg : (only_net == 1 ? 0 : resolve_pf_wgs(n_wg, n_wg_pf));
  const int jobs = (only_net >= 0 ? 1 : 2) * trl_ceil_div(ps, RED_CHUNK);
  const float* logstd = HEADS[head].logstd_tail ? adam->params + (p_pf - A) : nullptr;
  const unsigned epoch = (unsigned)adam->step_count;
  with_head(head, [&](auto hd) {
    auto launch = [&](auto loop) {
      hipLaunchKernelGGL((ppo_reduce_adam_kernel<decltype(loop)::value, decltype(hd)::value>), dim3(grid), dim3(64 * RED_WAVES), 0,
                         (hipStream_t)stream, partial, scal_partial, n_wg, n_pf, ps, p_pf, p_vf, logstd, A, grads, info, d,
                         workspace, epoch, adam->device_state, xr ? 1 : 0, xr ? *xr : none, only_net);
    };
    if (grid == jobs) launch(std::false_type{}); else launch(std::true_type{});
    return 0;
  });
  TRL_LAUNCH_CHECK();
  return TRL_OK;
}

extern "C" int trl_ppo_reduce_adam_f32(const float* partial, const double* scal_partial, int n_wg, int n_wg_pf,
                                       int D, int H, int A, float* grads, double* info, const trl_adam_t* adam,
                                       float* workspace, void* stream) {
  return launch_reduce_adam(partial, scal_partial, n_wg, n_wg_pf, D, H, A, grads, info, adam, workspace, nullptr, 0, stream);
}

extern "C" int trl_ppo_reduce_adam_net_f32(const float* partial, const double* scal_partial, int n_wg, int net,
                                           int D, int H, int A, float* grads, double* info, const trl_adam_t* adam,
                                           float* workspace, void* stream) {
  TRL_REQUIRE(net == 0 || net == 1, "net: 0 = policy, 1 = value function");
  return launch_reduce_adam(partial, scal_partial, n_wg, 0, D, H, A, grads, info, adam, workspace, nullptr, 0, stream, net);
}

extern "C" int trl_ppo_cat_reduce_adam_f32(const float* partial, const double* scal_partial, int n_wg, int n_wg_pf,
                                           int D, int H, int A, float* grads, double* info, const trl_adam_t* adam,
                                           float* workspace, void* stream) {
  return launch_reduce_adam(partial, scal_partial, n_wg, n_wg_pf, D, H, A, grads, info, adam, workspace, nullptr, 0, stream, -1, HEAD_CAT);
}
extern "C" int trl_ppo_cat_reduce_adam_net_f32(const float* partial, const double* scal_partial, int n_wg, int net,
                                               int D, int H, int A, float* grads, double* info, const trl_adam_t* adam,
                                               float* workspace, void* stream) {
  TRL_REQUIRE(net == 0 || net == 1, "net: 0 = policy, 1 = value function");
  return launch_reduce_adam(partial, scal_partial, n_wg, 0, D, H, A, grads, info, adam, workspace, nullptr, 0, stream, net, HEAD_CAT);
}

extern "C" int trl_ppo_sd_reduce_adam_f32(const float* partial, const double* scal_partial, int n_wg, int n_wg_pf,
                                          int D, int H, int A, float* grads, double* info, const trl_adam_t* adam,
                                          float* workspace, void* stream) {
  return launch_reduce_adam(partial, scal_partial, n_wg, n_wg_pf, D, H, A, grads, info, adam, workspace, nullptr, 0, stream, -1, HEAD_SD);
}
extern "C" int trl_ppo_sd_reduce_adam_net_f32(const float* partial, const double* scal_partial, int n_wg, int net,
                                              int D, int H, int A, float* grads, double* info, const trl_adam_t* adam,
                                              float* workspace, void* stream) {
  TRL_REQUIRE(net == 0 || net == 1, "net: 0 = policy, 1 = value function");
  return launch_reduce_adam(partial, scal_partial, n_wg, 0, D, H, A, grads, info, adam, workspace, nullptr, 0, stream, net, HEAD_SD);
}

extern "C" int trl_ppo_reduce_adam_xrank_f32(const float* partial, const double* scal_partial, int n_wg, int n_wg_pf,
                                             int D, int H, int A, float* grads, double* info, const trl_adam_t* adam,
                                             float* workspace, trl_comm_t* comm, void* stream) {
  const XrArgs* xr = trl_comm_xr(comm);
  if (!xr) { trl_set_error("trl_ppo_reduce_adam_xrank_f32: communicator without mapped peers"); return TRL_EINVAL; }
  return launch_reduce_adam(partial, scal_partial, n_wg, n_wg_pf, D, H, A, grads, info, adam, workspace, xr,
                            trl_comm_wait_blocks(comm), stream);
}

extern "C" int trl_ppo_reduce_adam_xrank_net_f32(const float* partial, const double* scal_partial, int n_wg, int net,
                                                 int D, int H, int A, float* grads, double* info, const trl_adam_t* adam,
                                                 float* workspace, trl_comm_t* comm, void* stream) {
  TRL_REQUIRE(net == 0 || net == 1, "net: 0 = policy, 1 = value function");
  const XrArgs* xr = trl_comm_xr(comm);
  if (!xr) { trl_set_error("trl_ppo_reduce_adam_xrank_net_f32: communicator without mapped peers"); return TRL_EINVAL; }
  const int wb = trl_comm_wait_blocks(comm);
  return launch_reduce_adam(partial, scal_partial, n_wg, 0, D, H, A, grads, info, adam, workspace, xr,
                            wb > 0 ? (wb + 1) / 2 : 0, stream, net);
}

#define TICK_PENDING 0x70000001
static int clip_adam_launch(const trl_adam_t* p, void* stream, bool tick_here);
extern "C" int trl_clip_adam_f32(const trl_adam_t* p, void* stream) { return clip_adam_launch(p, stream, true); }

struct FileRing { const uint32_t* raw; uint32_t* ring; const double* count; int words, slots, ticked; };
__global__ __launch_bounds__(256) void polyak_tick_kernel(float* __restrict__ tgt, const float* __restrict__ src, int64_t n,
                                                          float tau, double* __restrict__ st, float beta1, float beta2,
                                                          FileRing file) {
  if (file.ring && blockIdx.x == 0) {
    const int64_t u = (int64_t)file.count[0] - file.ticked;
    __syncthreads();
    uint32_t* row = file.ring + (int64_t)(((u % file.slots) + file.slots) % file.slots) * file.words;
    for (int w = threadIdx.x; w < file.words; w += 256) row[w] = file.raw[w];
  }
  if (st && blockIdx.x == 0 && threadIdx.x == 0) { st[0] += 1.0; st[1] *= (double)beta1; st[2] *= (double)beta2; }
  for (int64_t e = (int64_t)blockIdx.x * 256 + threadIdx.x; e < n; e += (int64_t)gridDim.x * 256)
    tgt[e] = tgt[e] * (1.0f - tau) + src[e] * tau;
}
static int clip_adam_polyak(const trl_adam_t* p, float* target, const float* source, int64_t n, float tau,
                            const void* raw, int raw_bytes, void* ring, int slots, void* stream) {
  TRL_REQUIRE(n > 0 && target && source, "polyak: empty / null");
  int rc = clip_adam_launch(p, stream, false);
  if (rc != TRL_OK && rc != TICK_PENDING) return rc;
  int grid = trl_ceil_div(n, 256);
  if (grid > 1024) grid = 1024;
  FileRing file = {(const uint32_t*)raw, (uint32_t*)ring, p->step_state, raw_bytes / 4, slots, rc == TICK_PENDING ? 0 : 1};
  hipLaunchKernelGGL(polyak_tick_kernel, dim3(grid), dim3(256), 0, (hipStream_t)stream, target, source, n, tau,
                     rc == TICK_PENDING ? p->step_state : (double*)nullptr, p->beta1, p->beta2, file);
  TRL_LAUNCH_CHECK();
  return TRL_OK;
}
extern "C" int trl_clip_adam_polyak_f32(const trl_adam_t* p, float* target, const float* source, int64_t n, float tau,
                                        const void* raw, int raw_bytes, void* ring, int slots, void* stream) {
  if (!ring) return clip_adam_polyak(p, target, source, n, tau, nullptr, 0, nullptr, 0, stream);
  TRL_REQUIRE(raw && raw_bytes > 0 && raw_bytes % 4 == 0 && slots > 0, "clip_adam_polyak: bad ring");
  TRL_REQUIRE(p && p->step_state, "clip_adam_polyak: the ring row is picked by the device-resident step state");
  return clip_adam_polyak(p, target, source, n, tau, raw, raw_bytes, ring, slots, stream);
}

#define FAP_THREADS 1024
#define FAP_MAX_WG 256
#define FAP_MAX_ENTRIES 32
struct FapDev {
  int count;
  int off[FAP_MAX_ENTRIES + 1];
  int splits[FAP_MAX_ENTRIES];
  const float* part[FAP_MAX_ENTRIES];
  float* target; int target_off, target_n; float tau;
  unsigned long long* slots;
  unsigned* err;
  float* grads_out;
};
__global__ __launch_bounds__(FAP_THREADS) void fold_adam_polyak_kernel(AdamDev a, FapDev f, FileRing file) {
  __shared__ float s_ss[4][FAP_THREADS / 64];
  __shared__ float s_coef[4];
  __shared__ float s_bc[2];
  __shared__ int s_fail;
  __shared__ int s_off[FAP_MAX_ENTRIES + 1], s_splits[FAP_MAX_ENTRIES];
  __shared__ const float* s_part[FAP_MAX_ENTRIES];
  const int tid = threadIdx.x, lane = tid & 63, wave = tid >> 6, nb = gridDim.x;
  if (tid <= f.count) s_off[tid] = f.off[tid];
  if (tid < f.count) { s_splits[tid] = f.splits[tid]; s_part[tid] = f.part[tid]; }
  const int total = a.off[a.n_groups];
  const int per = (total + nb - 1) / nb, lo = blockIdx.x * per, hi = min(total, lo + per);
  const double steps = a.step_state[0];
  const unsigned epoch = (unsigned)(long long)steps + 1u;
  if (tid == 0) {
    s_bc[0] = (float)(1.0 - a.step_state[1] * (double)a.beta1);
    s_bc[1] = (float)sqrt(1.0 - a.step_state[2] * (double)a.beta2);
    s_fail = 0;
  }
  __syncthreads();
  float ss[4] = {0.0f, 0.0f, 0.0f, 0.0f};
  for (int e = lo + tid; e < hi; e += FAP_THREADS) {
    int k = 0;
    while (k + 1 < f.count && e >= s_off[k + 1]) ++k;
    const int n = s_off[k + 1] - s_off[k], splits = s_splits[k];
    const float* p = s_part[k] + (e - s_off[k]);
    float c[4] = {0.0f, 0.0f, 0.0f, 0.0f};
    int s0 = 0;
    for (; s0 + 16 <= splits; s0 += 16) {
      float x[16];
#pragma unroll
      for (int q = 0; q < 16; ++q) x[q] = p[(size_t)(s0 + q) * n];
#pragma unroll
      for (int q = 0; q < 16; ++q) c[q & 3] += x[q];
    }
    for (; s0 < splits; ++s0) c[s0 & 3] += p[(size_t)s0 * n];
    const float gsum = (c[0] + c[1]) + (c[2] + c[3]);
    f.grads_out[e] = gsum;
    int g = 0;
    while (e >= a.off[g + 1]) ++g;
    const float gs = gsum * a.grad_scale;
#pragma unroll
    for (int q = 0; q < 4; ++q) ss[q] = fmaf(q == g ? gs : 0.0f, gs, ss[q]);
  }
#pragma unroll
  for (int q = 0; q < 4; ++q) {
    const float w = wave_sum(ss[q]);
    if (lane == 0) s_ss[q][wave] = w;
  }
  __syncthreads();
  if (tid < a.n_groups) {
    float t = 0.0f;
    for (int w = 0; w < FAP_THREADS / 64; ++w) t += s_ss[tid][w];
    __hip_atomic_store(f.slots + tid * FAP_MAX_WG + blockIdx.x, ((unsigned long long)epoch << 32) | __float_as_uint(t),
                       __ATOMIC_RELAXED, __HIP_MEMORY_SCOPE_AGENT);
  }
  {
    const int g = wave >> 2, r = wave & 3, b = 64 * r + lane;
    float v = 0.0f;
    if (g < a.n_groups && b < nb) {
      const unsigned long long* slot = f.slots + g * FAP_MAX_WG + b;
      unsigned long long x = __hip_atomic_load(slot, __ATOMIC_RELAXED, __HIP_MEMORY_SCOPE_AGENT);
      const unsigned long long t0 = wall_clock64();
      while ((unsigned)(x >> 32) != epoch) {
        __builtin_amdgcn_s_sleep(1);
        x = __hip_atomic_load(slot, __ATOMIC_RELAXED, __HIP_MEMORY_SCOPE_AGENT);
        if (wall_clock64() - t0 > 100000000ull) { s_fail = 1; break; }
      }
      v = __uint_as_float((unsigned)x);
    }
    v = wave_sum(v);
    if (lane == 0) s_ss[g & 3][r] = v;
  }
  __syncthreads();
  if (tid < a.n_groups) {
    const float t = ((s_ss[tid][0] + s_ss[tid][1]) + s_ss[tid][2]) + s_ss[tid][3];
    const float norm = sqrtf(t);
    s_coef[tid] = (a.max_norm > 0.0f) ? fminf(a.max_norm / (norm + 1e-6f), 1.0f) : 1.0f;
    if (blockIdx.x == 0 && a.norms_out) a.norms_out[tid] = norm;
  }
  __syncthreads();
  if (s_fail) { if (tid == 0) __hip_atomic_store(f.err, 1u, __ATOMIC_RELAXED, __HIP_MEMORY_SCOPE_AGENT); return; }
  const float bc1 = s_bc[0], bc2_sqrt = s_bc[1];
  for (int e = lo + tid; e < hi; e += FAP_THREADS) {
    int g = 0;
    while (e >= a.off[g + 1]) ++g;
    const float gr = f.grads_out[e] * a.grad_scale * s_coef[g];
    const float m = a.beta1 * a.m[e] + (1.0f - a.beta1) * gr;
    const float v = a.beta2 * a.v[e] + (1.0f - a.beta2) * gr * gr;
    a.m[e] = m; a.v[e] = v;
    const float denom = sqrtf(v) / bc2_sqrt + a.eps;
    const float lr = a.device_lr ? a.device_lr[g] : a.lr[g];
    const float pn = a.params[e] - (lr / bc1) * (m / denom);
    a.params[e] = pn;
    const int te = e - f.target_off;
    if (te >= 0 && te < f.target_n) f.target[te] = f.target[te] * (1.0f - f.tau) + pn * f.tau;
  }
  if (blockIdx.x == 0) {
    if (file.ring) {
      const int64_t u = (int64_t)steps;
      uint32_t* row = file.ring + (int64_t)(((u % file.slots) + file.slots) % file.slots) * file.words;
      for (int w = tid; w < file.words; w += FAP_THREADS) row[w] = file.raw[w];
    }
    if (tid == 0) { a.step_state[0] = steps + 1.0; a.step_state[1] *= (double)a.beta1; a.step_state[2] *= (double)a.beta2; }
  }
}
extern "C" int trl_fold_clip_adam_polyak_workspace(void) { return (int)(16 + 4 * FAP_MAX_WG * sizeof(unsigned long long)); }
extern "C" int trl_fold_clip_adam_polyak_f32(int count, const float* const* part, const int* n, const int* splits,
                                             const trl_adam_t* adam, float* target, int64_t target_off, int64_t target_n,
                                             float tau, const void* raw, int raw_bytes, void* ring, int slots,
                                             void* workspace, void* stream) {
  TRL_REQUIRE(count >= 1 && count <= FAP_MAX_ENTRIES && part && n && splits, "fold_clip_adam_polyak: 1..32 fold entries");
  TRL_REQUIRE(adam && adam->step_state && workspace, "fold_clip_adam_polyak: needs the device-resident step state and a workspace");
  TRL_REQUIRE((!target_n) || (target && target_off >= 0), "fold_clip_adam_polyak: bad target range");
  TRL_REQUIRE(!ring || (raw && raw_bytes > 0 && raw_bytes % 4 == 0 && slots > 0), "fold_clip_adam_polyak: bad ring");
  AdamDev d;
  int rc = fill_adam(adam, d);
  if (rc) return rc;
  FapDev f{};
  f.count = count;
  for (int k = 0; k < count; ++k) {
    TRL_REQUIRE(part[k] && n[k] > 0 && splits[k] >= 1, "fold_clip_adam_polyak: bad entry");
    f.part[k] = part[k]; f.splits[k] = splits[k]; f.off[k + 1] = f.off[k] + n[k];
  }
  const int total = d.off[d.n_groups];
  TRL_REQUIRE(f.off[count] == total, "fold_clip_adam_polyak: the fold entries must cover the parameter block exactly, in order");
  TRL_REQUIRE(target_off + target_n <= total, "fold_clip_adam_polyak: target range outside the parameter block");
  f.target = target; f.target_off = (int)target_off; f.target_n = (int)target_n; f.tau = tau;
  f.err = (unsigned*)workspace;
  f.slots = (unsigned long long*)((char*)workspace + 16);
  f.grads_out = const_cast<float*>(adam->grads);
  FileRing file = {(const uint32_t*)raw, (uint32_t*)ring, adam->step_state, raw_bytes / 4, slots, 0};
  const int grid = std::max(1, std::min(FAP_MAX_WG, trl_ceil_div(total, FAP_THREADS)));
  hipLaunchKernelGGL(fold_adam_polyak_kernel, dim3(grid), dim3(FAP_THREADS), 0, (hipStream_t)stream, d, f, file);
  TRL_LAUNCH_CHECK();
  return TRL_OK;
}

static int clip_adam_launch(const trl_adam_t* p, void* stream, bool tick_here) {
  AdamDev d;
  int rc = fill_adam(p, d);
  if (rc) return rc;
  TRL_REQUIRE(!p->device_state, "device_state is a feature of trl_ppo_reduce_adam_f32");
  const int total = d.off[p->n_groups];
  if (total == 0) return TRL_OK;
  const int blocks = trl_ceil_div(total, 256);
  d.self_tick = (d.step_state && blocks <= 128) ? 1 : 0;
  hipLaunchKernelGGL(clip_adam_kernel, dim3(blocks), dim3(256), 0, (hipStream_t)stream, d);
  TRL_LAUNCH_CHECK();
  if (d.step_state && !d.self_tick) {
    if (!tick_here) return TICK_PENDING;
    hipLaunchKernelGGL(adam_tick_kernel, dim3(1), dim3(1), 0, (hipStream_t)stream, d.step_state, d.beta1, d.beta2);
    TRL_LAUNCH_CHECK();
  }
  return TRL_OK;
}

template <int D, int H, int O>
static int launch_fwd(const float* params, const float* x, float* out, int M, int act, hipStream_t s) {
  int grid = trl_ceil_div(M, 128);
  if (grid > 1024) grid = 1024;
  if (act == TRL_ACT_TANH)
    hipLaunchKernelGGL((mlp2_forward_kernel<D, H, O, TRL_ACT_TANH>), dim3(grid), dim3(256), 0, s, params, x, out, M);
  else
    hipLaunchKernelGGL((mlp2_forward_kernel<D, H, O, TRL_ACT_RELU>), dim3(grid), dim3(256), 0, s, params, x, out, M);
  TRL_LAUNCH_CHECK();
  return TRL_OK;
}

extern "C" int trl_mlp2_forward_supported(int D, int H, int O) {
  return (D == 17 && H == 64 && (O == 6 || O == 1)) ? 1 : 0;
}

extern "C" int trl_mlp2_forward_f32(const float* params, const float* x, float* out, int M, int D, int H,
                                    int O, int act, void* stream) {
  TRL_REQUIRE(M >= 0, "negative M");
  if (M == 0) return TRL_OK;
  TRL_REQUIRE(params && x && out, "null pointer");
  TRL_REQUIRE(act == TRL_ACT_TANH || act == TRL_ACT_RELU, "unknown activation");
  hipStream_t s = (hipStream_t)stream;
  if (D == 17 && H == 64 && O == 6) return launch_fwd<17, 64, 6>(params, x, out, M, act, s);
  if (D == 17 && H == 64 && O == 1) return launch_fwd<17, 64, 1>(params, x, out, M, act, s);
  trl_set_error("mlp2_forward: shape D=%d H=%d O=%d not instantiated", D, H, O);
  return TRL_EUNSUPPORTED;
}
```

torchrl_amd/csrc/k_rollout.hip:

```cpp
#include <algorithm>
#include "trl_common.h"
#include "trl_mlp.h"
#include "trl_head.h"
#include "trl_philox.h"

#define RO_THREADS 256
#define RO_ENVS 16
#ifdef TRL_EXP_CLK
#define CLK_DECL long long clk_prev = clock64(); float clk_acc[8] = {0, 0, 0, 0, 0, 0, 0, 0};
#define CLK(ph) { const long long c_ = clock64(); clk_acc[ph] += (float)(c_ - clk_prev); clk_prev = c_; }
#else
#define CLK_DECL
#define CLK(ph)
#endif
#define RO_NB 16

struct RolloutDev {
  const float *pf_params, *vf_params, *env_A, *env_B;
  float reward_scale; int horizon; int64_t env_seed_base;
  float* cur_obs; int32_t *t_env, *cur_step, *episode_idx; float* ep_return;
  const float* noise; int64_t noise_step0;
  float *obs, *next_obs, *acts, *values, *rewards, *terminals, *time_limits, *old_logp;
  int rows, top, N, n_steps, max_episode_frames; float discount;
  double* epoch_reward; int32_t* ep_count; float* ep_log; int ep_cap; int step0;
  int tanh_action, deterministic, store;
  double* norm_state; float* policy_obs; double* norm_ws; float norm_clip; int norm_update, norm_partial_reset;
  double* clear_hdr;
  float* boot;
  uint32_t* pub_dst; const uint32_t* pub_src; int64_t pub_words;
  const uint32_t* noise_flag; uint32_t noise_stamp;
  int D, A;
  int n_ro_wg; const f32x4* stg_src; unsigned long long* stg_dst; int64_t stg_n4;
  const uint32_t* stg_ready; uint32_t stg_job; uint32_t* stg_state; uint32_t* stg_ack;
  int64_t cat_seed, cat_env0;
};
#define RO_STAGERS 16

template <int CTRL> __device__ __forceinline__ double ro_dpp_f64(double v) {
  const unsigned long long u = __builtin_bit_cast(unsigned long long, v);
  const unsigned lo = (unsigned)__builtin_amdgcn_update_dpp(0, (int)(unsigned)(u & 0xFFFFFFFFull), CTRL, 0xF, 0xF, false);
  const unsigned hi = (unsigned)__builtin_amdgcn_update_dpp(0, (int)(unsigned)(u >> 32), CTRL, 0xF, 0xF, false);
  return __builtin_bit_cast(double, ((unsigned long long)hi << 32) | lo);
}
__device__ __forceinline__ double ro_row_sum16(double v) {
  v += ro_dpp_f64<0x128>(v);
  v += ro_dpp_f64<0x124>(v);
  v += ro_dpp_f64<0x122>(v);
  v += ro_dpp_f64<0x121>(v);
  return v;
}
#define NORM_SLOT 40

template <int D, int H, int A, int HC_ = 8> struct RoShape {
  static_assert(H == 64 && D > 16 && D <= 32 && A <= 8, "instantiated for 16 < D <= 32, H == 64, A <= 8");
  static_assert(HC_ == 8 || HC_ == 16, "the head exchange carries half or all of the 16-row head tile");
  static constexpr int HC = HC_;
  static constexpr int O_B1 = 0, O_B2 = H, O_B3 = 2 * H, O_LS = O_B3 + HC, O_H1 = O_LS + 8, O_HP = O_H1 + H * TL,
                       O_EPS = O_HP + 4 * HC * 16, LDS_FLOATS = O_EPS + RO_NB * 8 * 16;
};

__device__ __forceinline__ void stage_block(const f32x4* __restrict__ src, unsigned long long* __restrict__ dst, int64_t n4,
                                            int wg, int wgs, int threads, uint32_t* __restrict__ state, uint32_t stamp,
                                            uint32_t* __restrict__ host_ack) {
  const int64_t stride = (int64_t)wgs * threads;
  for (int64_t e = (int64_t)wg * threads + threadIdx.x; e < n4; e += 4 * stride) {
    f32x4 v[4];
#pragma unroll
    for (int q = 0; q < 4; ++q) if (e + q * stride < n4) v[q] = src[e + q * stride];
#pragma unroll
    for (int q = 0; q < 4; ++q)
      if (e + q * stride < n4) {
        const unsigned long long lo = ((unsigned long long)__float_as_uint(v[q][1]) << 32) | __float_as_uint(v[q][0]);
        const unsigned long long hi = ((unsigned long long)__float_as_uint(v[q][3]) << 32) | __float_as_uint(v[q][2]);
        __hip_atomic_store(dst + 2 * (e + q * stride), lo, __ATOMIC_RELAXED, __HIP_MEMORY_SCOPE_AGENT);
        __hip_atomic_store(dst + 2 * (e + q * stride) + 1, hi, __ATOMIC_RELAXED, __HIP_MEMORY_SCOPE_AGENT);
      }
  }
  asm volatile("s_waitcnt vmcnt(0)" ::: "memory");
  __syncthreads();
  if (threadIdx.x == 0) {
    const unsigned before = __hip_atomic_fetch_add(state + 1, 1u, __ATOMIC_RELAXED, __HIP_MEMORY_SCOPE_AGENT);
    if (before == (unsigned)wgs - 1) {
      __hip_atomic_store(state + 1, 0u, __ATOMIC_RELAXED, __HIP_MEMORY_SCOPE_AGENT);
      __hip_atomic_store(state, stamp, __ATOMIC_RELAXED, __HIP_MEMORY_SCOPE_AGENT);
      if (host_ack) __hip_atomic_store(host_ack, stamp, __ATOMIC_RELAXED, __HIP_MEMORY_SCOPE_SYSTEM);
    }
  }
}

template <int D, int H, int A, int ACT, bool NORM, bool RT = false, int HEAD = HEAD_GAUSS>
__global__ __launch_bounds__(RO_THREADS, 1) void rollout_kernel(RolloutDev a) {
  using S = RoShape<D, H, A, HEAD == HEAD_SD ? 16 : 8>;
  constexpr bool WIDE = D > 17, CAT = HEAD == HEAD_CAT, SD = HEAD == HEAD_SD;
  static_assert(!CAT || RT, "the categorical head exists as a runtime-dims instantiation only");
  static_assert(!SD || (RT && !NORM), "the state-dependent-std head exists as a runtime-dims instantiation only");
  static_assert(!WIDE || RT, "the wide tile exists as a runtime-dims instantiation only");
  static_assert(!(RT && NORM), "the cooperative (normalised) rollout is instantiated for the benchmark shape");
  const int Dr = RT ? a.D : D, Ar = RT ? a.A : A;
  const int HW = SD ? 2 * Ar : Ar;
  const int F_W1 = 0, F_B1 = H * Dr, F_W2 = F_B1 + H, F_B2 = F_W2 + H * H, F_W3 = F_B2 + H, F_B3 = F_W3 + HW * H,
            F_LS = F_B3 + HW;
  __shared__ __attribute__((aligned(16))) float lds[S::LDS_FLOATS];
  if (!NORM && (int)blockIdx.x >= a.n_ro_wg) {
    __shared__ int s_go;
    if (threadIdx.x == 0) {
      const unsigned long long t0 = wall_clock64();
      int go = 1;
      while (__hip_atomic_load(a.stg_ready, __ATOMIC_RELAXED, __HIP_MEMORY_SCOPE_SYSTEM) != a.stg_job) {
        __builtin_amdgcn_s_sleep(64);
        if (wall_clock64() - t0 > 3000ull) { go = 0; break; }
      }
      s_go = go;
    }
    __syncthreads();
    if (s_go)
      stage_block(a.stg_src, a.stg_dst, a.stg_n4, (int)blockIdx.x - a.n_ro_wg, (int)gridDim.x - a.n_ro_wg, RO_THREADS,
                  a.stg_state, a.stg_job, a.stg_ack);
    return;
  }
  const int tid = threadIdx.x, lane = tid & 63;
  const int mo = __builtin_amdgcn_readfirstlane(tid >> 6);
  const int j = lane & 15, g = lane >> 4, i = j;
  const int n = blockIdx.x * RO_ENVS + j;
  const bool valid = n < a.N;
  const float* gp = a.pf_params;
  const bool has_lo = g < Ar, has_hi = 4 + g < Ar;
  const int o_lo = has_lo ? g : 0, o_hi = has_hi ? 4 + g : 0;
  if (blockIdx.x == 0 && tid == 0 && a.clear_hdr) { a.clear_hdr[0] = 0.0; a.clear_hdr[1] = 0.0; }
  if (a.noise_flag && tid == 0) {
    unsigned spins = 0;
    while (__hip_atomic_load(a.noise_flag, __ATOMIC_RELAXED, __HIP_MEMORY_SCOPE_AGENT) != a.noise_stamp) {
      __builtin_amdgcn_s_sleep(32);
      if (++spins > (1u << 24)) {
        if (blockIdx.x == 0 && a.epoch_reward) a.epoch_reward[0] = __builtin_nan("");
        break;
      }
    }
    if (spins) __threadfence();
  }

  for (int e = tid; e < H; e += RO_THREADS) { lds[S::O_B1 + e] = gp[F_B1 + e]; lds[S::O_B2 + e] = gp[F_B2 + e]; }
  if constexpr (SD) {
    if (tid < 16) lds[S::O_B3 + tid] = tid < HW ? gp[F_B3 + (tid < HW ? tid : 0)] : 0.0f;
    if (tid < 8) lds[S::O_LS + tid] = 0.0f;
  } else if (tid < 8) {
    lds[S::O_B3 + tid] = tid < Ar ? gp[F_B3 + (tid < Ar ? tid : 0)] : 0.0f;
    lds[S::O_LS + tid] = (!CAT && tid < Ar) ? gp[F_LS + (tid < Ar ? tid : 0)] : 0.0f;
  }
  bool fv[4], fv2[4];
#pragma unroll
  for (int q = 0; q < 4; ++q) { fv[q] = 4 * g + q < Dr; fv2[q] = WIDE && 16 + 4 * g + q < Dr; }
  const bool f16 = !WIDE && 16 + g < Dr;
  const bool row_f = i < Dr, row_f2 = WIDE && 16 + i < Dr;
  constexpr int XK = WIDE ? 8 : 5, EK = XK + 2;
  float w1r[XK], w2r[4][4], w3a[4], we0[EK], w16[EK], we1[WIDE ? EK : 1];
  {
    const int row = 16 * mo + i;
#pragma unroll
    for (int r = 0; r < 4; ++r) w1r[r] = fv[r] ? gp[F_W1 + row * Dr + (fv[r] ? 4 * g + r : 0)] : 0.0f;
    if constexpr (WIDE) {
#pragma unroll
      for (int r = 0; r < 4; ++r) w1r[4 + r] = fv2[r] ? gp[F_W1 + row * Dr + (fv2[r] ? 16 + 4 * g + r : 0)] : 0.0f;
    } else {
      w1r[4] = f16 ? gp[F_W1 + row * Dr + (f16 ? 16 + g : 0)] : 0.0f;
    }
#pragma unroll
    for (int sl = 0; sl < 4; ++sl)
#pragma unroll
      for (int r = 0; r < 4; ++r) w2r[sl][r] = gp[F_W2 + row * H + 16 * sl + 4 * g + r];
#pragma unroll
    for (int r = 0; r < 4; ++r) w3a[r] = (i < HW) ? gp[F_W3 + (i < HW ? i : 0) * H + 16 * mo + 4 * g + r] : 0.0f;
    static_assert(WIDE || D == 17, "the narrow env step keeps exactly one feature outside the 16-row MFMA tile");
    const bool has16 = !WIDE && Dr > 16;
#pragma unroll
    for (int q = 0; q < EK; ++q) {
      const float* mat = q < XK ? a.env_A : a.env_B;
      int k; bool kin;
      if (q < 4) { k = 4 * g + q; kin = k < Dr; }
      else if (q < XK) { k = WIDE ? 16 + 4 * g + (q - 4) : 16 + g; kin = k < Dr; }
      else { k = (q == XK) ? g : 4 + g; kin = k < Ar; }
      const int kc = kin ? k : 0;
      we0[q] = (kin && row_f) ? mat[kc * Dr + (row_f ? i : 0)] : 0.0f;
      w16[q] = (kin && has16) ? mat[kc * Dr + (has16 ? 16 : 0)] : 0.0f;
      if constexpr (WIDE) we1[q] = (kin && row_f2) ? mat[kc * Dr + (row_f2 ? 16 + i : 0)] : 0.0f;
    }
  }
  __syncthreads();

  float* S_H1 = lds + S::O_H1;
  float* headp = lds + S::O_HP;
  float* S_EPS = lds + S::O_EPS;
  const float* b1s = lds + S::O_B1 + 16 * mo + 4 * g;
  const float* b2s = lds + S::O_B2 + 16 * mo + 4 * g;

  float ls_lo = fminf(fmaxf(lds[S::O_LS + o_lo], -20.0f), 2.0f), ls_hi = fminf(fmaxf(lds[S::O_LS + o_hi], -20.0f), 2.0f);
  float std_lo = __expf(ls_lo), std_hi = __expf(ls_hi);
  float iv_lo = __expf(-2.0f * ls_lo), iv_hi = __expf(-2.0f * ls_hi);
  const float b3_lo = lds[S::O_B3 + o_lo], b3_hi = lds[S::O_B3 + o_hi];

  float xb[XK];
#pragma unroll
  for (int r = 0; r < 4; ++r) xb[r] = (valid && fv[r]) ? a.cur_obs[(size_t)n * Dr + (fv[r] ? 4 * g + r : 0)] : 0.0f;
  if constexpr (WIDE) {
#pragma unroll
    for (int r = 0; r < 4; ++r) xb[4 + r] = (valid && fv2[r]) ? a.cur_obs[(size_t)n * Dr + (fv2[r] ? 16 + 4 * g + r : 0)] : 0.0f;
  } else {
    xb[4] = (valid && f16) ? a.cur_obs[(size_t)n * Dr + (f16 ? 16 + g : 0)] : 0.0f;
  }
  float xp[XK];
  __shared__ double s_mean[NORM ? D : 1], s_var[NORM ? D : 1], s_sum[NORM ? 2 * D + 1 : 1];
  __shared__ double s_cnt;
  unsigned* nhdr = NORM ? reinterpret_cast<unsigned*>(a.norm_ws) : nullptr;
  if constexpr (NORM) {
#pragma unroll
    for (int r = 0; r < 4; ++r) xp[r] = valid ? a.policy_obs[(size_t)n * D + 4 * g + r] : 0.0f;
    xp[4] = (valid && g == 0) ? a.policy_obs[(size_t)n * D + 16] : 0.0f;
    if (tid < D) { s_mean[tid] = a.norm_state[tid]; s_var[tid] = a.norm_state[D + tid]; }
    if (tid == 0) s_cnt = a.norm_state[2 * D];
    __syncthreads();
  } else {
#pragma unroll
    for (int q = 0; q < XK; ++q) xp[q] = xb[q];
  }
  int t_env = valid ? a.t_env[n] : 0;
  int cur_step = valid ? a.cur_step[n] : 0;
  int ep_idx = valid ? a.episode_idx[n] : 0;
  float ep_ret = valid ? a.ep_return[n] : 0.0f;
  const int64_t env_seed = a.env_seed_base + n;
  double rew_sum = 0.0;
  const bool dev_noise = !a.deterministic && !a.noise;
  CLK_DECL

  for (int t = 0; t < a.n_steps; ++t) {
    const int row = (a.top + t) % a.rows;
    const size_t cell = (size_t)row * a.N + n;

    float cat_u = 0.0f;
    if constexpr (CAT) {
      if (dev_noise && (t % RO_NB) == 0) {
        const int ts = 4 * mo + g;
        S_EPS[ts * 16 + j] = trl_cat_uniform(a.cat_seed, a.noise_step0 + t + ts, a.cat_env0 + n);
        __syncthreads();
      }
      if (dev_noise) cat_u = S_EPS[(t % RO_NB) * 16 + j];
    }
    if (!CAT && dev_noise && (t % RO_NB) == 0) {
      const int ts = 4 * mo + g;
      const int64_t gs = a.noise_step0 + t + ts;
      float z0[4], z1[4];
      philox_normals4((uint32_t)(gs & 0xFFFFFFFFll), (uint32_t)((gs >> 32) & 0xFFFFFFFFll), 0u, TRL_TAG_NOISE, env_seed, z0);
      if (Ar > 4)
        philox_normals4((uint32_t)(gs & 0xFFFFFFFFll), (uint32_t)((gs >> 32) & 0xFFFFFFFFll), 1u, TRL_TAG_NOISE, env_seed, z1);
#pragma unroll
      for (int c = 0; c < 4; ++c) {
        S_EPS[(ts * 8 + c) * 16 + j] = z0[c];
        if (4 + c < Ar) S_EPS[(ts * 8 + 4 + c) * 16 + j] = z1[c];
      }
      __syncthreads();
    }
    float eps_lo = 0.0f, eps_hi = 0.0f;
    if (!CAT && dev_noise) {
      eps_lo = S_EPS[((t % RO_NB) * 8 + o_lo) * 16 + j];
      eps_hi = S_EPS[((t % RO_NB) * 8 + o_hi) * 16 + j];
    } else if (!CAT && a.noise) {
      eps_lo = valid ? a.noise[((size_t)t * a.N + n) * Ar + o_lo] : 0.0f;
      eps_hi = valid ? a.noise[((size_t)t * a.N + n) * Ar + o_hi] : 0.0f;
    }

    CLK(0)
    f32x4 h1 = *reinterpret_cast<const f32x4*>(b1s);
#pragma unroll
    for (int q = 0; q < XK; ++q) h1 = mfma16(w1r[q], xp[q], h1);
    f32x4 e0 = f32x4{0.f, 0.f, 0.f, 0.f}, e1 = f32x4{0.f, 0.f, 0.f, 0.f};
    float p16 = 0.0f;
#pragma unroll
    for (int q = 0; q < XK; ++q) {
      e0 = mfma16(we0[q], xb[q], e0);
      if constexpr (WIDE) e1 = mfma16(we1[q], xb[q], e1);
      else p16 = fmaf(w16[q], xb[q], p16);
    }
#pragma unroll
    for (int r = 0; r < 4; ++r) h1[r] = act_fn<ACT>(h1[r]);
    store_T(S_H1, mo, h1, j, g);
    CLK(1)
    __syncthreads();
    CLK(2)
    f32x4 h2 = *reinterpret_cast<const f32x4*>(b2s), h2b = f32x4{0.f, 0.f, 0.f, 0.f};
#pragma unroll
    for (int sl = 0; sl < 4; sl += 2) {
      const f32x4 b0 = load_T(S_H1, sl, j, g), b1 = load_T(S_H1, sl + 1, j, g);
#pragma unroll
      for (int r = 0; r < 4; ++r) { h2 = mfma16(w2r[sl][r], b0[r], h2); h2b = mfma16(w2r[sl + 1][r], b1[r], h2b); }
    }
#pragma unroll
    for (int r = 0; r < 4; ++r) h2[r] = act_fn<ACT>(h2[r] + h2b[r]);
    f32x4 hp = f32x4{0.f, 0.f, 0.f, 0.f};
#pragma unroll
    for (int r = 0; r < 4; ++r) hp = mfma16(w3a[r], h2[r], hp);
    if (SD || g < 2) {
#pragma unroll
      for (int r = 0; r < 4; ++r) headp[(mo * S::HC + 4 * g + r) * 16 + j] = hp[r];
    }
    CLK(3)
    __syncthreads();
    CLK(4)
    float mean_lo = b3_lo, mean_hi = b3_hi;
#pragma unroll
    for (int w = 0; w < 4; ++w) { mean_lo += headp[(w * S::HC + o_lo) * 16 + j]; mean_hi += headp[(w * S::HC + o_hi) * 16 + j]; }
    if constexpr (SD) {
      float raw_lo = lds[S::O_B3 + Ar + o_lo], raw_hi = lds[S::O_B3 + Ar + o_hi];
#pragma unroll
      for (int w = 0; w < 4; ++w) {
        raw_lo += headp[(w * S::HC + Ar + o_lo) * 16 + j];
        raw_hi += headp[(w * S::HC + Ar + o_hi) * 16 + j];
      }
      ls_lo = fminf(fmaxf(raw_lo, -20.0f), 2.0f); ls_hi = fminf(fmaxf(raw_hi, -20.0f), 2.0f);
      std_lo = __expf(ls_lo); std_hi = __expf(ls_hi);
      iv_lo = __expf(-2.0f * ls_lo); iv_hi = __expf(-2.0f * ls_hi);
    }

    int cat_k = 0;
    float cat_lsel = 0.0f, cat_m = 0.0f, cat_S = 1.0f;
    if constexpr (CAT) {
      float lg[8], ex[8];
#pragma unroll
      for (int k = 0; k < 8; ++k) {
        float l = lds[S::O_B3 + k];
#pragma unroll
        for (int w = 0; w < 4; ++w) l += headp[(w * 8 + k) * 16 + j];
        lg[k] = l;
      }
      cat_m = lg[0];
#pragma unroll
      for (int k = 1; k < 8; ++k)
        if (k < Ar && lg[k] > cat_m) { cat_m = lg[k]; cat_k = k; }
      cat_S = 0.0f;
#pragma unroll
      for (int k = 0; k < 8; ++k)
        if (k < Ar) { ex[k] = expf(lg[k] - cat_m); cat_S += ex[k]; }
      if (dev_noise) {
        const float thr = cat_u * cat_S;
        float c = 0.0f;
        bool hit = false;
        cat_k = Ar - 1;
#pragma unroll
        for (int k = 0; k < 8; ++k)
          if (k < Ar) {
            c += ex[k];
            if (!hit && c >= thr) { cat_k = k; hit = true; }
          }
      }
#pragma unroll
      for (int k = 0; k < 8; ++k) cat_lsel = k == cat_k ? lg[k] : cat_lsel;
    }
    const float z_lo = fmaf(std_lo, eps_lo, mean_lo), z_hi = fmaf(std_hi, eps_hi, mean_hi);
    const float act_lo = CAT ? (g == cat_k ? 1.0f : 0.0f) : has_lo ? (a.tanh_action ? trl_tanh(z_lo) : z_lo) : 0.0f;
    const float act_hi = CAT ? (4 + g == cat_k ? 1.0f : 0.0f) : has_hi ? (a.tanh_action ? trl_tanh(z_hi) : z_hi) : 0.0f;
    e0 = mfma16(we0[XK], act_lo, e0);
    e0 = mfma16(we0[XK + 1], act_hi, e0);
    if constexpr (WIDE) {
      e1 = mfma16(we1[XK], act_lo, e1);
      e1 = mfma16(we1[XK + 1], act_hi, e1);
    } else {
      p16 = fmaf(w16[XK], act_lo, p16);
      p16 = fmaf(w16[XK + 1], act_hi, p16);
    }
    const f32x4 zero4 = f32x4{0.f, 0.f, 0.f, 0.f};
    const float e16 = WIDE ? 0.0f : mfma16(1.0f, p16, zero4)[0];
    const float act_sq = mfma16(1.0f, fmaf(act_lo, act_lo, act_hi * act_hi), zero4)[0];
    float logp = 0.0f;
    if (mo == 3) {
      if constexpr (CAT) {
        logp = (cat_lsel - cat_m) - logf(cat_S);
      } else {
        float zc, lp = 0.0f;
        if (has_lo) lp += gauss_logp_term(act_lo, mean_lo, iv_lo, ls_lo, a.tanh_action, zc);
        if (has_hi) lp += gauss_logp_term(act_hi, mean_hi, iv_hi, ls_hi, a.tanh_action, zc);
        logp = mfma16(1.0f, lp, zero4)[0];
      }
    }
    CLK(5)
    float nx[XK];
#pragma unroll
    for (int r = 0; r < 4; ++r) nx[r] = trl_tanh(e0[r]);
    if constexpr (WIDE) {
#pragma unroll
      for (int r = 0; r < 4; ++r) nx[4 + r] = trl_tanh(e1[r]);
    } else {
      nx[4] = (g == 0 && Dr > 16) ? trl_tanh(e16) : 0.0f;
    }

    CLK(6)
    const float nx0 = mfma16(1.0f, g == 0 ? nx[0] : 0.0f, zero4)[0];
    float raw_rew = a.reward_scale * (nx0 - 0.1f * act_sq);
    asm volatile("" : "+v"(raw_rew));
    t_env += 1; cur_step += 1;
    const bool done = t_env >= a.horizon;
    const bool surpass = cur_step >= a.max_episode_frames;
    float nxn[XK];
    bool any_reset = false;
    if constexpr (NORM) {
      if (a.norm_update) {
        double* part = a.norm_ws + 2 + (size_t)((t & 1) * gridDim.x + blockIdx.x) * NORM_SLOT;
        if (mo == 0) {
#pragma unroll
          for (int q = 0; q < 5; ++q) {
            const int f = q < 4 ? 4 * g + q : 16;
            const double d = (valid && (q < 4 || g == 0)) ? (double)nx[q] - s_mean[f] : 0.0;
            const double s1 = ro_row_sum16(d), s2 = ro_row_sum16(d * d);
            if (j == 0 && (q < 4 || g == 0)) {
              __hip_atomic_store(part + f, s1, __ATOMIC_RELAXED, __HIP_MEMORY_SCOPE_AGENT);
              __hip_atomic_store(part + D + f, s2, __ATOMIC_RELAXED, __HIP_MEMORY_SCOPE_AGENT);
            }
          }
          const bool fl = __ballot(valid && (done || surpass)) != 0ull;
          if (lane == 0) __hip_atomic_store(part + 2 * D, fl ? 1.0 : 0.0, __ATOMIC_RELAXED, __HIP_MEMORY_SCOPE_AGENT);
          asm volatile("s_waitcnt vmcnt(0)" ::: "memory");
          const unsigned long long stamp = (unsigned long long)(a.noise_step0 + t + 1);
          if (lane == 0)
            __hip_atomic_store(reinterpret_cast<unsigned long long*>(part + NORM_SLOT - 1), stamp, __ATOMIC_RELAXED,
                               __HIP_MEMORY_SCOPE_AGENT);
          for (int w = lane; w < (int)gridDim.x; w += 64) {
            const unsigned long long* st = reinterpret_cast<const unsigned long long*>(
                a.norm_ws + 2 + (size_t)((t & 1) * gridDim.x + w) * NORM_SLOT + NORM_SLOT - 1);
            int it = 0;
            while (__hip_atomic_load(st, __ATOMIC_RELAXED, __HIP_MEMORY_SCOPE_AGENT) != stamp) {
              __builtin_amdgcn_s_sleep(1);
              if (++it > (1 << 22)) { __hip_atomic_store(nhdr + 2, 1u, __ATOMIC_RELAXED, __HIP_MEMORY_SCOPE_AGENT); break; }
            }
          }
        }
        __syncthreads();
        if (tid < 2 * D + 1) {
          const double* col = a.norm_ws + 2 + (size_t)((t & 1) * gridDim.x) * NORM_SLOT + tid;
          double acc = 0.0;
          int w = 0;
          for (; w + 8 <= (int)gridDim.x; w += 8) {
            double v[8];
#pragma unroll
            for (int k = 0; k < 8; ++k) v[k] = __hip_atomic_load(col + (size_t)(w + k) * NORM_SLOT, __ATOMIC_RELAXED, __HIP_MEMORY_SCOPE_AGENT);
#pragma unroll
            for (int k = 0; k < 8; ++k) acc += v[k];
          }
          for (; w < (int)gridDim.x; ++w) acc += __hip_atomic_load(col + (size_t)w * NORM_SLOT, __ATOMIC_RELAXED, __HIP_MEMORY_SCOPE_AGENT);
          s_sum[tid] = acc;
        }
        __syncthreads();
        if (tid < D) {
          const double bn = (double)a.N, cnt = s_cnt;
          const double delta = s_sum[tid] / bn, bvar = fmax(s_sum[D + tid] / bn - delta * delta, 0.0);
          const double tot = cnt + bn;
          const double m2 = s_var[tid] * cnt + bvar * bn + delta * delta * cnt * bn / tot;
          s_mean[tid] += delta * bn / tot;
          s_var[tid] = m2 / tot;
        }
        __syncthreads();
        if (tid == 0) s_cnt += (double)a.N;
        any_reset = s_sum[2 * D] != 0.0;
      } else {
        any_reset = __ballot(valid && (done || surpass)) != 0ull;
      }
#pragma unroll
      for (int q = 0; q < 5; ++q) {
        const int f = q < 4 ? 4 * g + q : 16;
        const double z = ((double)nx[q] - s_mean[f]) / (sqrt(s_var[f]) + 1e-4);
        nxn[q] = (q < 4 || g == 0) ? (float)fmin(fmax(z, -(double)a.norm_clip), (double)a.norm_clip) : 0.0f;
      }
    } else {
#pragma unroll
      for (int q = 0; q < XK; ++q) nxn[q] = nx[q];
    }
    ep_ret += raw_rew;
    if (mo == 0 && g == 0 && valid) {
      rew_sum += (double)raw_rew;
      if (done) {
        const int slot = atomicAdd(a.ep_count, 1);
        if (slot < a.ep_cap) { a.ep_log[slot * 3 + 0] = (float)(a.step0 + t); a.ep_log[slot * 3 + 1] = (float)n; a.ep_log[slot * 3 + 2] = ep_ret; }
      }
    }
    if (done) ep_ret = 0.0f;

    float xn[XK];
#pragma unroll
    for (int q = 0; q < XK; ++q) xn[q] = nx[q];
    if (done || surpass) {
      ep_idx += 1; t_env = 0; cur_step = 0;
      float z[4];
      philox_normals4((uint32_t)ep_idx, 0u, (uint32_t)g, TRL_TAG_RESET, env_seed, z);
#pragma unroll
      for (int c = 0; c < 4; ++c) xn[c] = fv[c] ? z[c] : 0.0f;
      if constexpr (WIDE) {
        philox_normals4((uint32_t)ep_idx, 0u, (uint32_t)(4 + g), TRL_TAG_RESET, env_seed, z);
#pragma unroll
        for (int c = 0; c < 4; ++c) xn[4 + c] = fv2[c] ? z[c] : 0.0f;
      } else {
        xn[4] = 0.0f;
        if (g == 0 && Dr > 16) {
          philox_normals4((uint32_t)ep_idx, 0u, 4u, TRL_TAG_RESET, env_seed, z);
          xn[4] = z[0];
        }
      }
    }

    if (valid && a.store) {
      if (mo == 0 || mo == 1) {
        float* dst = (mo == 0 ? a.obs : a.next_obs) + cell * Dr;
        const float* src = mo == 0 ? xp : nxn;
#pragma unroll
        for (int r = 0; r < 4; ++r) if (!RT || fv[r]) dst[4 * g + r] = src[r];
        if constexpr (WIDE) {
#pragma unroll
          for (int r = 0; r < 4; ++r) if (fv2[r]) dst[16 + 4 * g + r] = src[4 + r];
        } else {
          if (g == 0 && (!RT || Dr > 16)) dst[16] = src[4];
        }
      } else if (mo == 2) {
        if constexpr (CAT) {
          if (g == 0) a.acts[cell] = (float)cat_k;
        } else {
          if (has_lo) a.acts[cell * Ar + g] = act_lo;
          if (has_hi) a.acts[cell * Ar + 4 + g] = act_hi;
        }
      } else {
        float* dst = g == 0 ? a.values : g == 1 ? a.rewards : g == 2 ? a.terminals : a.time_limits;
        const float val = g == 0 ? (surpass ? 1.0f : 0.0f) : g == 1 ? raw_rew
                        : g == 2 ? ((done || surpass) ? 1.0f : 0.0f) : (done ? 1.0f : 0.0f);
        dst[cell] = val;
        if (g == 0 && a.old_logp) a.old_logp[cell] = logp;
      }
    }
    if constexpr (NORM) {
#pragma unroll
      for (int q = 0; q < 5; ++q) {
        float alt = xn[q];
        if (a.norm_partial_reset) {
          const int f = q < 4 ? 4 * g + q : 16;
          const double z = ((double)xn[q] - s_mean[f]) / (sqrt(s_var[f]) + 1e-4);
          alt = (q < 4 || g == 0) ? (float)fmin(fmax(z, -(double)a.norm_clip), (double)a.norm_clip) : 0.0f;
        }
        xp[q] = any_reset ? alt : nxn[q];
      }
    } else {
#pragma unroll
      for (int q = 0; q < XK; ++q) xp[q] = xn[q];
    }
#pragma unroll
    for (int q = 0; q < XK; ++q) xb[q] = xn[q];
    CLK(7)
  }
  if constexpr (NORM) {
    if (mo == 0 && valid) {
#pragma unroll
      for (int r = 0; r < 4; ++r) a.policy_obs[(size_t)n * D + 4 * g + r] = xp[r];
      if (g == 0) a.policy_obs[(size_t)n * D + 16] = xp[4];
    }
    if (blockIdx.x == 0 && a.norm_update) {
      if (tid < D) { a.norm_state[tid] = s_mean[tid]; a.norm_state[D + tid] = s_var[tid]; }
      if (tid == 0) a.norm_state[2 * D] = s_cnt;
    }
  }
#ifdef TRL_EXP_CLK
  if (blockIdx.x == 0 && lane == 0)
    for (int ph = 0; ph < 8; ++ph) a.ep_log[(a.ep_cap - 16) * 3 + mo * 8 + ph] = clk_acc[ph];
#endif

  if (mo == 0 && valid) {
    float* dst = a.cur_obs + (size_t)n * Dr;
#pragma unroll
    for (int r = 0; r < 4; ++r) if (!RT || fv[r]) dst[4 * g + r] = xb[r];
    if constexpr (WIDE) {
#pragma unroll
      for (int r = 0; r < 4; ++r) if (fv2[r]) dst[16 + 4 * g + r] = xb[4 + r];
    }
    if (g == 0) {
      if (!WIDE && (!RT || Dr > 16)) dst[16] = xb[4];
      a.t_env[n] = t_env; a.cur_step[n] = cur_step; a.episode_idx[n] = ep_idx; a.ep_return[n] = ep_ret;
    }
  }
  if (mo == 0) {
    const double tot = wave_sum(rew_sum);
    if (lane == 0 && a.epoch_reward) atomicAdd(a.epoch_reward, tot);
  }
}

#define VP_THREADS 256

struct ValueDev {
  const float* vf_params; const float *obs, *next_obs; float *values, *rewards;
  int rows, top, N, n_steps; float discount;
  float* boot;
  uint32_t* pub_dst; const uint32_t* pub_src; int64_t pub_words;
  int D;
};

template <int D, int H, int ACT, bool RT = false>
__global__ __launch_bounds__(VP_THREADS, RT ? 1 : 2) void value_pass_kernel(ValueDev a) {
  static_assert(H == 64 && D > 16 && D <= 32, "instantiated for 16 < D <= 32, H == 64");
  constexpr bool WIDE = D > 17;
  static_assert(!WIDE || RT, "the wide tile exists as a runtime-dims instantiation only");
  constexpr int XK = WIDE ? 8 : 5;
  const int Dr = RT ? a.D : D;
  const int F_W1 = 0, F_B1 = H * Dr, F_W2 = F_B1 + H, F_B2 = F_W2 + H * H, F_W3 = F_B2 + H, F_B3 = F_W3 + H;
  __shared__ __attribute__((aligned(16))) float sb[2 * H];
  const int tid = threadIdx.x, lane = tid & 63, wave = tid >> 6;
  const int j = lane & 15, g = lane >> 4, i = j;
  const float* gp = a.vf_params;
  for (int e = tid; e < H; e += VP_THREADS) { sb[e] = gp[F_B1 + e]; sb[H + e] = gp[F_B2 + e]; }
  bool fv[4], fv2[4];
#pragma unroll
  for (int q = 0; q < 4; ++q) { fv[q] = 4 * g + q < Dr; fv2[q] = WIDE && 16 + 4 * g + q < Dr; }
  const bool f16 = !WIDE && 16 + g < Dr;
  const bool w2_al = !RT || ((reinterpret_cast<uintptr_t>(gp + F_W2) & 15) == 0);
  float w1[4][XK], w2[4][4][4], w3[4][4];
#pragma unroll
  for (int so = 0; so < 4; ++so) {
    const int row = 16 * so + i;
#pragma unroll
    for (int r = 0; r < 4; ++r) w1[so][r] = fv[r] ? gp[F_W1 + row * Dr + (fv[r] ? 4 * g + r : 0)] : 0.0f;
    if constexpr (WIDE) {
#pragma unroll
      for (int r = 0; r < 4; ++r) w1[so][4 + r] = fv2[r] ? gp[F_W1 + row * Dr + (fv2[r] ? 16 + 4 * g + r : 0)] : 0.0f;
    } else {
      w1[so][4] = f16 ? gp[F_W1 + row * Dr + (f16 ? 16 + g : 0)] : 0.0f;
    }
#pragma unroll
    for (int sl = 0; sl < 4; ++sl) {
      f32x4 w;
      if (w2_al) w = *reinterpret_cast<const f32x4*>(gp + F_W2 + row * H + 16 * sl + 4 * g);
      else __builtin_memcpy(&w, gp + F_W2 + row * H + 16 * sl + 4 * g, 16);
#pragma unroll
      for (int r = 0; r < 4; ++r) w2[so][sl][r] = w[r];
    }
#pragma unroll
    for (int r = 0; r < 4; ++r) w3[so][r] = gp[F_W3 + 16 * so + 4 * g + r];
  }
  const float b3 = gp[F_B3];
  __syncthreads();

  auto fetch = [&](const float* src, size_t cell, bool ok, float (&xb)[XK]) {
#pragma unroll
    for (int r = 0; r < 4; ++r) xb[r] = (ok && fv[r]) ? src[cell * Dr + (fv[r] ? 4 * g + r : 0)] : 0.0f;
    if constexpr (WIDE) {
#pragma unroll
      for (int r = 0; r < 4; ++r) xb[4 + r] = (ok && fv2[r]) ? src[cell * Dr + (fv2[r] ? 16 + 4 * g + r : 0)] : 0.0f;
    } else {
      xb[4] = (ok && f16) ? src[cell * Dr + (f16 ? 16 + g : 0)] : 0.0f;
    }
  };
  auto forward = [&](const float (&xb)[XK]) -> float {
    f32x4 h1[4], h2[4];
#pragma unroll
    for (int so = 0; so < 4; ++so) {
      f32x4 acc = *reinterpret_cast<const f32x4*>(sb + 16 * so + 4 * g);
#pragma unroll
      for (int q = 0; q < XK; ++q) acc = mfma16(w1[so][q], xb[q], acc);
#pragma unroll
      for (int r = 0; r < 4; ++r) acc[r] = act_fn<ACT>(acc[r]);
      h1[so] = acc;
    }
#pragma unroll
    for (int so = 0; so < 4; ++so) {
      f32x4 acc = *reinterpret_cast<const f32x4*>(sb + H + 16 * so + 4 * g);
#pragma unroll
      for (int sl = 0; sl < 4; ++sl)
#pragma unroll
        for (int r = 0; r < 4; ++r) acc = mfma16(w2[so][sl][r], h1[sl][r], acc);
#pragma unroll
      for (int r = 0; r < 4; ++r) acc[r] = act_fn<ACT>(acc[r]);
      h2[so] = acc;
    }
    float v = 0.0f;
#pragma unroll
    for (int so = 0; so < 4; ++so)
#pragma unroll
      for (int r = 0; r < 4; ++r) v = fmaf(w3[so][r], h2[so][r], v);
    v += __shfl_xor(v, 16, 64);
    v += __shfl_xor(v, 32, 64);
    return v + b3;
  };

  for (int64_t e = (int64_t)blockIdx.x * VP_THREADS + tid; e < a.pub_words; e += (int64_t)gridDim.x * VP_THREADS)
    a.pub_dst[e] = a.pub_src[e];
  const int64_t M = (int64_t)a.n_steps * a.N;
  const int64_t n_tiles = (M + 15) / 16;
  auto locate = [&](int64_t tile, bool& ok, int& t, int& n) -> size_t {
    const int64_t m = tile * 16 + j;
    ok = tile < n_tiles && m < M;
    t = ok ? (int)(m / a.N) : 0;
    n = ok ? (int)(m - (int64_t)t * a.N) : 0;
    return (size_t)((a.top + t) % a.rows) * a.N + n;
  };
  const int64_t stride = (int64_t)gridDim.x * 4;
  int64_t tile = (int64_t)blockIdx.x * 4 + wave;
  bool ok, ok_n;
  int t, n, t_n, n_n;
  float xb[XK], xn[XK];
  size_t cell = locate(tile, ok, t, n), cell_n;
  fetch(a.obs, cell, ok, xb);
  float marker = ok ? a.values[cell] : 0.0f, marker_n;
  for (; tile < n_tiles; tile += stride) {
    cell_n = locate(tile + stride, ok_n, t_n, n_n);
    fetch(a.obs, cell_n, ok_n, xn);
    marker_n = ok_n ? a.values[cell_n] : 0.0f;
    const float v = forward(xb);
    if (ok && g == 0) a.values[cell] = v;
    const bool last = ok && a.boot && t == a.n_steps - 1;
    if (__ballot(marker != 0.0f || last) != 0ull) {
      float x2[XK];
      fetch(a.next_obs, cell, ok, x2);
      const float v2 = forward(x2);
      if (ok && g == 0 && marker != 0.0f) a.rewards[cell] += a.discount * v2;
      if (last && g == 0) a.boot[n] = v2;
    }
#pragma unroll
    for (int q = 0; q < XK; ++q) xb[q] = xn[q];
    cell = cell_n; ok = ok_n; t = t_n; n = n_n; marker = marker_n;
  }
}

__global__ __launch_bounds__(256) void zero_value_pass_kernel(float* __restrict__ values, int rows, int top, int N, int n_steps,
                                                              float* __restrict__ boot, uint32_t* __restrict__ pub_dst,
                                                              const uint32_t* __restrict__ pub_src, int64_t pub_words) {
  const int64_t e0 = (int64_t)blockIdx.x * 256 + threadIdx.x, stride = (int64_t)gridDim.x * 256;
  for (int64_t e = e0; e < pub_words; e += stride) pub_dst[e] = pub_src[e];
  const int64_t M = (int64_t)n_steps * N;
  for (int64_t m = e0; m < M; m += stride) {
    const int t = (int)(m / N), n = (int)(m - (int64_t)t * N);
    values[(size_t)((top + t) % rows) * N + n] = 0.0f;
  }
  if (boot)
    for (int64_t n = e0; n < N; n += stride) boot[n] = 0.0f;
}

template <int D, int H, int A, int ACT>
static int rollout_norm_capacity() {
  int dev = 0, cus = 0, per_cu = 0;
  if (hipGetDevice(&dev) != hipSuccess) return 0;
  if (hipDeviceGetAttribute(&cus, hipDeviceAttributeMultiprocessorCount, dev) != hipSuccess) return 0;
  if (hipOccupancyMaxActiveBlocksPerMultiprocessor(&per_cu, rollout_kernel<D, H, A, ACT, true>, RO_THREADS, 0) != hipSuccess)
    return 0;
  return cus * per_cu * RO_ENVS;
}

template <int D, int H, int A, int ACT, bool RT = false, int HEAD = HEAD_GAUSS>
static int launch_rollout(const RolloutDev& d, hipStream_t s, hipEvent_t value_wait = nullptr) {
  const int n_wg = trl_ceil_div(d.N, RO_ENVS);
  if constexpr (RT) {
    if (d.norm_state) { trl_set_error("rollout: the normalised rollout is instantiated for the benchmark shape only"); return TRL_EUNSUPPORTED; }
    RolloutDev e = d;
    e.n_ro_wg = n_wg;
    hipLaunchKernelGGL((rollout_kernel<D, H, A, ACT, false, true, HEAD>), dim3(n_wg + (e.stg_n4 ? RO_STAGERS : 0)), dim3(RO_THREADS), 0, s, e);
  } else if (d.norm_state) {
    const int cap = rollout_norm_capacity<D, H, A, ACT>();
    if (d.norm_update && d.N > cap) {
      trl_set_error("rollout: %d envs with a running normaliser exceed the %d that can be co-resident", d.N, cap);
      return TRL_EUNSUPPORTED;
    }
    hipLaunchKernelGGL((rollout_kernel<D, H, A, ACT, true>), dim3(n_wg), dim3(RO_THREADS), 0, s, d);
  } else {
    RolloutDev e = d;
    e.n_ro_wg = n_wg;
    hipLaunchKernelGGL((rollout_kernel<D, H, A, ACT, false>), dim3(n_wg + (e.stg_n4 ? RO_STAGERS : 0)), dim3(RO_THREADS), 0, s, e);
  }
  TRL_LAUNCH_CHECK();
  if (d.store && !d.vf_params) {
    const int64_t blocks = ((int64_t)d.n_steps * d.N + 255) / 256;
    hipLaunchKernelGGL(zero_value_pass_kernel, dim3((unsigned)(blocks > 1024 ? 1024 : blocks)), dim3(256), 0, s, d.values, d.rows,
                       d.top, d.N, d.n_steps, d.boot, d.pub_dst, d.pub_src, d.pub_words);
    TRL_LAUNCH_CHECK();
  } else if (d.store) {
    if (value_wait) {
      hipError_t e = hipStreamWaitEvent(s, value_wait, 0);
      if (e != hipSuccess) { trl_set_error("rollout: hipStreamWaitEvent(value_wait_event): %s", hipGetErrorString(e)); return (int)e; }
    }
    ValueDev v{d.vf_params, d.obs, d.next_obs, d.values, d.rewards, d.rows, d.top, d.N, d.n_steps, d.discount, d.boot,
               d.pub_dst, d.pub_src, d.pub_words, d.D};
    const int64_t n_tiles = ((int64_t)d.n_steps * d.N + 15) / 16;
    const int grid = (int)(n_tiles / 4 + 1 < 512 ? n_tiles / 4 + 1 : 512);
    hipLaunchKernelGGL((value_pass_kernel<D, H, ACT, RT>), dim3(grid), dim3(VP_THREADS), 0, s, v);
    TRL_LAUNCH_CHECK();
  }
  return TRL_OK;
}

__global__ __launch_bounds__(256) void stage_h2d_kernel(const f32x4* __restrict__ src, unsigned long long* __restrict__ dst,
                                                        int64_t n4, uint32_t* __restrict__ state, uint32_t stamp) {
  stage_block(src, dst, n4, (int)blockIdx.x, (int)gridDim.x, 256, state, stamp, nullptr);
}
extern "C" int trl_stage_h2d_f32(const float* host_src, float* dev_dst, int64_t n, uint32_t* state, uint32_t stamp,
                                 void* stream) {
  TRL_REQUIRE(n >= 0 && (n & 3) == 0, "stage_h2d: n must be a multiple of 4");
  TRL_REQUIRE(state, "stage_h2d: null state");
  TRL_REQUIRE(!n || (host_src && dev_dst && ((reinterpret_cast<uintptr_t>(host_src) | reinterpret_cast<uintptr_t>(dev_dst)) & 15) == 0),
              "stage_h2d: null / misaligned pointer");
  const int grid = (int)std::max<int64_t>(1, std::min<int64_t>(16, (n / 4 + 1023) / 1024));
  hipLaunchKernelGGL(stage_h2d_kernel, dim3(grid), dim3(256), 0, (hipStream_t)stream, reinterpret_cast<const f32x4*>(host_src),
                     reinterpret_cast<unsigned long long*>(dev_dst), n / 4, state, stamp);
  TRL_LAUNCH_CHECK();
  return TRL_OK;
}

extern "C" int trl_rollout_supported(int D, int H, int A, int act) { return head_supported(HEAD_GAUSS, D, H, A, act); }
extern "C" int trl_rollout_cat_supported(int D, int H, int A, int act) { return head_supported(HEAD_CAT, D, H, A, act); }
extern "C" int trl_rollout_sd_supported(int D, int H, int A, int act) { return head_supported(HEAD_SD, D, H, A, act); }

static int rollout_synth(const trl_rollout_t* p, void* stream, int head, int64_t cat_seed = 0, int64_t cat_env0 = 0) {
  if (!p) { trl_set_error("rollout: null descriptor"); return TRL_EINVAL; }
  TRL_REQUIRE(p->pf_params && p->env_A && p->env_B, "null network / env pointer");
  TRL_REQUIRE(p->cur_obs && p->t_env && p->cur_step && p->episode_idx && p->ep_return, "null env state pointer");
  const bool all_ring = p->obs && p->next_obs && p->acts && p->values && p->rewards && p->terminals && p->time_limits;
  const bool no_ring = !p->obs && !p->next_obs && !p->acts && !p->values && !p->rewards && !p->terminals && !p->time_limits;
  TRL_REQUIRE(all_ring || no_ring, "ring tensors must be all set or all NULL");
  TRL_REQUIRE(p->ep_count && p->ep_log && p->ep_cap >= 0, "null episode log");
  TRL_REQUIRE(p->N > 0 && p->n_steps >= 0 && p->rows > 0, "bad sizes");
  TRL_REQUIRE(p->top >= 0 && p->top < p->rows, "top outside ring");
  TRL_REQUIRE(no_ring || p->n_steps <= p->rows, "n_steps exceeds ring rows");
  TRL_REQUIRE(p->horizon > 0 && p->max_episode_frames > 0, "horizon / max_episode_frames must be positive");
  if (head == HEAD_CAT) {
    TRL_REQUIRE(cat_env0 >= 0, "categorical: negative env offset");
    TRL_REQUIRE(!p->noise && !p->noise_flag && !p->stage_n,
                "categorical: actions are drawn from the device Philox stream only (no host noise block, nothing staged)");
    TRL_REQUIRE(!p->norm_state, "categorical: no running observation normaliser in the persistent rollout");
  }
  if (head == HEAD_SD) {
    TRL_REQUIRE(!p->norm_state, "state-dependent std: no running observation normaliser in the persistent rollout");
    TRL_REQUIRE(!p->noise_flag && !p->stage_n,
                "state-dependent std: the noise block is stream-ordered in front of the launch (no noise gate, nothing staged)");
  }
  if (head != HEAD_GAUSS && !head_supported(head, p->D, p->H, p->A, p->act)) {
    trl_set_error("rollout: %s shape D=%d H=%d A=%d act=%d not instantiated", HEADS[head].name, p->D, p->H, p->A, p->act);
    return TRL_EUNSUPPORTED;
  }
  if (p->n_steps == 0) return TRL_OK;
  RolloutDev d;
  d.pf_params = p->pf_params; d.vf_params = p->vf_params; d.env_A = p->env_A; d.env_B = p->env_B;
  d.reward_scale = p->reward_scale; d.horizon = p->horizon; d.env_seed_base = p->env_seed_base;
  d.cur_obs = p->cur_obs; d.t_env = p->t_env; d.cur_step = p->cur_step; d.episode_idx = p->episode_idx;
  d.ep_return = p->ep_return; d.noise = p->noise; d.noise_step0 = p->noise_step0;
  d.obs = p->obs; d.next_obs = p->next_obs; d.acts = p->acts; d.values = p->values; d.rewards = p->rewards;
  d.terminals = p->terminals; d.time_limits = p->time_limits; d.old_logp = p->old_logp;
  d.rows = p->rows; d.top = p->top; d.N = p->N; d.n_steps = p->n_steps;
  d.max_episode_frames = p->max_episode_frames; d.discount = p->discount;
  d.epoch_reward = p->epoch_reward; d.ep_count = p->ep_count; d.ep_log = p->ep_log; d.ep_cap = p->ep_cap;
  d.step0 = p->step0; d.tanh_action = p->tanh_action; d.deterministic = p->deterministic; d.store = all_ring ? 1 : 0;
  d.norm_state = p->norm_state; d.policy_obs = p->policy_obs; d.norm_ws = p->norm_workspace; d.norm_clip = p->norm_clip;
  d.norm_update = p->norm_update; d.norm_partial_reset = p->normalize_partial_reset;
  d.clear_hdr = p->clear_header; d.boot = all_ring ? p->boot_values : nullptr;
  TRL_REQUIRE(p->publish_words >= 0 && (!p->publish_words || (p->publish_dst && p->publish_src && all_ring)) &&
              ((reinterpret_cast<uintptr_t>(p->publish_dst) | reinterpret_cast<uintptr_t>(p->publish_src)) & 3) == 0,
              "publish: needs ring tensors, non-null 4-byte aligned pointers");
  d.pub_dst = (uint32_t*)p->publish_dst; d.pub_src = (const uint32_t*)p->publish_src; d.pub_words = p->publish_words;
  d.noise_flag = p->noise ? p->noise_flag : nullptr; d.noise_stamp = p->noise_stamp;
  d.n_ro_wg = 0; d.stg_n4 = 0;
  d.cat_seed = cat_seed; d.cat_env0 = cat_env0;
  if (p->stage_n) {
    TRL_REQUIRE(p->stage_n > 0 && (p->stage_n & 3) == 0 && p->stage_src && p->stage_dst && p->stage_ready && p->stage_state &&
                p->stage_ack && !p->norm_state, "stage: n % 4 == 0, non-null pointers, no observation normaliser");
    TRL_REQUIRE(((reinterpret_cast<uintptr_t>(p->stage_src) | reinterpret_cast<uintptr_t>(p->stage_dst)) & 15) == 0,
                "stage: 16-byte aligned blocks");
    d.stg_src = reinterpret_cast<const f32x4*>(p->stage_src); d.stg_dst = reinterpret_cast<unsigned long long*>(p->stage_dst);
    d.stg_n4 = p->stage_n / 4; d.stg_ready = p->stage_ready; d.stg_job = p->stage_job; d.stg_state = p->stage_state;
    d.stg_ack = p->stage_ack;
  }
  TRL_REQUIRE(!p->clear_header || (p->clear_header != p->epoch_reward && (void*)p->clear_header != (void*)p->ep_count),
              "clear_header must not be the header this launch accumulates into");
  TRL_REQUIRE(!p->norm_state || (p->policy_obs && p->norm_workspace), "normaliser needs policy_obs and its workspace");
  hipStream_t s = (hipStream_t)stream;
  hipEvent_t vw = (hipEvent_t)p->value_wait_event;
  d.D = p->D; d.A = p->A;
  if (head == HEAD_GAUSS && p->D == 17 && p->H == 64 && p->A == 6) {
    if (p->act == TRL_ACT_TANH) return launch_rollout<17, 64, 6, TRL_ACT_TANH>(d, s, vw);
    if (p->act == TRL_ACT_RELU) return launch_rollout<17, 64, 6, TRL_ACT_RELU>(d, s, vw);
  }
  if (head_supported(head, p->D, p->H, p->A, p->act) && !p->norm_state)
    return with_head(head, [&](auto hd) {
      return with_tile_act(p->D, p->act, [&](auto tile, auto act) {
        return launch_rollout<decltype(tile)::value, 64, 8, decltype(act)::value, true, decltype(hd)::value>(d, s, vw);
      });
    });
  trl_set_error("rollout: shape D=%d H=%d A=%d act=%d not instantiated", p->D, p->H, p->A, p->act);
  return TRL_EUNSUPPORTED;
}

extern "C" int trl_rollout_synth_f32(const trl_rollout_t* p, void* stream) { return rollout_synth(p, stream, HEAD_GAUSS); }

extern "C" int trl_rollout_synth_cat_f32(const trl_rollout_t* p, int64_t noise_seed, int64_t env_offset, void* stream) {
  return rollout_synth(p, stream, HEAD_CAT, noise_seed, env_offset);
}

extern "C" int trl_rollout_synth_sd_f32(const trl_rollout_t* p, void* stream) { return rollout_synth(p, stream, HEAD_SD); }

extern "C" int trl_rollout_norm_workspace(int N) {
  if (N <= 0) { trl_set_error("trl_rollout_norm_workspace: N must be positive"); return TRL_EINVAL; }
  return 2 + 2 * trl_ceil_div(N, RO_ENVS) * NORM_SLOT;
}
extern "C" int trl_rollout_norm_max_envs(int D, int H, int A, int act) {
  if (D == 17 && H == 64 && A == 6) {
    if (act == TRL_ACT_TANH) return rollout_norm_capacity<17, 64, 6, TRL_ACT_TANH>();
    if (act == TRL_ACT_RELU) return rollout_norm_capacity<17, 64, 6, TRL_ACT_RELU>();
  }
  trl_set_error("rollout: shape D=%d H=%d A=%d act=%d not instantiated", D, H, A, act);
  return TRL_EUNSUPPORTED;
}

__global__ __launch_bounds__(256) void synth_reset_kernel(float* __restrict__ cur_obs, int32_t* __restrict__ t_env,
                                                          int32_t* __restrict__ cur_step,
                                                          int32_t* __restrict__ episode_idx,
                                                          float* __restrict__ ep_return,
                                                          const uint8_t* __restrict__ mask, int N, int D,
                                                          int64_t seed_base) {
  const int nblk = (D + 3) / 4;
  const int e = blockIdx.x * blockDim.x + threadIdx.x;
  const int n = e / nblk, b = e - n * nblk;
  if (n >= N || (mask && !mask[n])) return;
  const int ep = episode_idx[n] + 1;
  float z[4];
  philox_normals4((uint32_t)ep, 0u, (uint32_t)b, TRL_TAG_RESET, seed_base + n, z);
  for (int c = 0; c < 4; ++c) if (4 * b + c < D) cur_obs[(size_t)n * D + 4 * b + c] = z[c];
  if (b == 0) {
    t_env[n] = 0;
    if (!mask) { cur_step[n] = 0; ep_return[n] = 0.0f; }
  }
}
__global__ __launch_bounds__(256) void synth_bump_episode_kernel(int32_t* __restrict__ episode_idx,
                                                                 const uint8_t* __restrict__ mask, int N) {
  const int n = blockIdx.x * blockDim.x + threadIdx.x;
  if (n < N && (!mask || mask[n])) episode_idx[n] += 1;
}

extern "C" int trl_synth_reset_f32(float* cur_obs, int32_t* t_env, int32_t* cur_step, int32_t* episode_idx,
                                   float* ep_return, const uint8_t* mask, int N, int D, int64_t env_seed_base,
                                   void* stream) {
  TRL_REQUIRE(cur_obs && t_env && cur_step && episode_idx && ep_return, "null pointer");
  TRL_REQUIRE(N >= 0 && D > 0, "bad sizes");
  if (N == 0) return TRL_OK;
  const int nblk = (D + 3) / 4;
  hipStream_t s = (hipStream_t)stream;
  hipLaunchKernelGGL(synth_reset_kernel, dim3(trl_ceil_div((int64_t)N * nblk, 256)), dim3(256), 0, s, cur_obs,
                     t_env, cur_step, episode_idx, ep_return, mask, N, D, env_seed_base);
  TRL_LAUNCH_CHECK();
  hipLaunchKernelGGL(synth_bump_episode_kernel, dim3(trl_ceil_div(N, 256)), dim3(256), 0, s, episode_idx, mask, N);
  TRL_LAUNCH_CHECK();
  return TRL_OK;
}

__global__ __launch_bounds__(256) void gauss_logp_kernel(const float* __restrict__ mean, const float* __restrict__ acts,
                                                         const float* __restrict__ logstd, float* __restrict__ out,
                                                         int B, int A, int tanh_action) {
  const int b = blockIdx.x * blockDim.x + threadIdx.x;
  if (b >= B) return;
  float lp = 0.0f;
  for (int o = 0; o < A; ++o) {
    const float ls = fminf(fmaxf(logstd[o], -20.0f), 2.0f);
    float zc;
    lp += gauss_logp_term(acts[(size_t)b * A + o], mean[(size_t)b * A + o], __expf(-2.0f * ls), ls, tanh_action, zc);
  }
  out[b] = lp;
}

extern "C" int trl_gauss_logp_f32(const float* mean, const float* acts, const float* logstd, float* out, int B,
                                  int A, int tanh_action, void* stream) {
  TRL_REQUIRE(B >= 0 && A > 0, "bad sizes");
  if (B == 0) return TRL_OK;
  TRL_REQUIRE(mean && acts && logstd && out, "null pointer");
  hipLaunchKernelGGL(gauss_logp_kernel, dim3(trl_ceil_div(B, 256)), dim3(256), 0, (hipStream_t)stream, mean, acts,
                     logstd, out, B, A, tanh_action);
  TRL_LAUNCH_CHECK();
  return TRL_OK;
}


__global__ __launch_bounds__(256) void gauss_explore_kernel(const float* __restrict__ mean, const float* __restrict__ logstd,
                                                            const float* __restrict__ eps, float* __restrict__ act,
                                                            float* __restrict__ logp, int N, int A, int tanh_action) {
  const int n = blockIdx.x * blockDim.x + threadIdx.x;
  if (n >= N) return;
  float lp = 0.0f;
  for (int o = 0; o < A; ++o) {
    const float ls = fminf(fmaxf(logstd[o], -20.0f), 2.0f);
    const float m = mean[(size_t)n * A + o];
    const float z = fmaf(__expf(ls), eps ? eps[(size_t)n * A + o] : 0.0f, m);
    const float a = tanh_action ? trl_tanh(z) : z;
    act[(size_t)n * A + o] = a;
    float zc;
    lp += gauss_logp_term(a, m, __expf(-2.0f * ls), ls, tanh_action, zc);
  }
  if (logp) logp[n] = lp;
}

extern "C" int trl_gauss_explore_f32(const float* mean, const float* logstd, const float* eps, float* act, float* logp,
                                     int N, int A, int tanh_action, void* stream) {
  TRL_REQUIRE(N >= 0 && A > 0, "bad sizes");
  if (N == 0) return TRL_OK;
  TRL_REQUIRE(mean && logstd && act, "null pointer");
  hipLaunchKernelGGL(gauss_explore_kernel, dim3(trl_ceil_div(N, 256)), dim3(256), 0, (hipStream_t)stream, mean, logstd,
                     eps, act, logp, N, A, tanh_action);
  TRL_LAUNCH_CHECK();
  return TRL_OK;
}

__global__ __launch_bounds__(256) void onpolicy_bookkeep_kernel(float* __restrict__ rew, const float* __restrict__ done,
                                                                const float* __restrict__ v_next, float discount,
                                                                float* __restrict__ terminals, int32_t* __restrict__ cur_step,
                                                                float* __restrict__ ep_return, int max_frames,
                                                                uint8_t* __restrict__ mask, int32_t* __restrict__ any_flag,
                                                                double* __restrict__ epoch_reward, int32_t* __restrict__ ep_count,
                                                                float* __restrict__ ep_log, int ep_cap, int step, int N) {
  const int n = blockIdx.x * blockDim.x + threadIdx.x;
  double r = 0.0;
  bool flag = false;
  if (n < N) {
    const float raw = rew[n];
    r = (double)raw;
    const bool d = done[n] != 0.0f;
    const int cs = cur_step[n] + 1;
    float er = ep_return[n] + raw;
    if (d) {
      const int slot = atomicAdd(ep_count, 1);
      if (slot < ep_cap) { ep_log[slot * 3 + 0] = (float)step; ep_log[slot * 3 + 1] = (float)n; ep_log[slot * 3 + 2] = er; }
      er = 0.0f;
    }
    const bool surpass = cs >= max_frames;
    flag = d || surpass;
    rew[n] = raw + discount * v_next[n] * (surpass ? 1.0f : 0.0f);
    terminals[n] = flag ? 1.0f : 0.0f;
    cur_step[n] = flag ? 0 : cs;
    ep_return[n] = er;
    mask[n] = flag ? 1 : 0;
  }
  const double tot = wave_sum(r);
  if ((threadIdx.x & 63) == 0 && epoch_reward && tot != 0.0) atomicAdd(epoch_reward, tot);
  if (__ballot(flag) != 0ull && (threadIdx.x & 63) == 0) atomicOr(any_flag, 1);
}

extern "C" int trl_onpolicy_bookkeep_f32(float* rewards, const float* dones, const float* v_next, float discount,
                                         float* terminals, int32_t* cur_step, float* ep_return, int max_episode_frames,
                                         uint8_t* reset_mask, int32_t* any_flag, double* epoch_reward, int32_t* ep_count,
                                         float* ep_log, int ep_cap, int step, int N, void* stream) {
  TRL_REQUIRE(N >= 0 && ep_cap >= 0, "bad sizes");
  if (N == 0) return TRL_OK;
  TRL_REQUIRE(rewards && dones && v_next && terminals && cur_step && ep_return && reset_mask && any_flag && ep_count && ep_log,
              "null pointer");
  hipLaunchKernelGGL(onpolicy_bookkeep_kernel, dim3(trl_ceil_div(N, 256)), dim3(256), 0, (hipStream_t)stream, rewards,
                     dones, v_next, discount, terminals, cur_step, ep_return, max_episode_frames, reset_mask, any_flag,
                     epoch_reward, ep_count, ep_log, ep_cap, step, N);
  TRL_LAUNCH_CHECK();
  return TRL_OK;
}

__global__ __launch_bounds__(256) void select_on_flag_kernel(const int32_t* __restrict__ flag, const float* __restrict__ a,
                                                             const float* __restrict__ b, float* __restrict__ out, int64_t n) {
  const bool f = *flag != 0;
  for (int64_t e = (int64_t)blockIdx.x * 256 + threadIdx.x; e < n; e += (int64_t)gridDim.x * 256) out[e] = f ? a[e] : b[e];
}

extern "C" int trl_select_on_flag_f32(const int32_t* flag, const float* a, const float* b, float* out, int64_t n,
                                      void* stream) {
  TRL_REQUIRE(n >= 0, "negative size");
  if (n == 0) return TRL_OK;
  TRL_REQUIRE(flag && a && b && out, "null pointer");
  const int64_t blocks = (n + 255) / 256;
  hipLaunchKernelGGL(select_on_flag_kernel, dim3((unsigned)(blocks > 1024 ? 1024 : blocks)), dim3(256), 0,
                     (hipStream_t)stream, flag, a, b, out, n);
  TRL_LAUNCH_CHECK();
  return TRL_OK;
}

__global__ __launch_bounds__(256) void select_on_mask_kernel(const uint8_t* __restrict__ mask, int N, const float* __restrict__ a,
                                                             const float* __restrict__ b, float* __restrict__ out, int64_t n) {
  int any = 0;
  for (int e = threadIdx.x; e < N; e += 256) any |= mask[e];
  const bool f = __syncthreads_or(any) != 0;
  for (int64_t e = (int64_t)blockIdx.x * 256 + threadIdx.x; e < n; e += (int64_t)gridDim.x * 256) out[e] = f ? a[e] : b[e];
}

extern "C" int trl_select_on_mask_f32(const uint8_t* mask, int N, const float* a, const float* b, float* out, int64_t n,
                                      void* stream) {
  TRL_REQUIRE(n >= 0 && N >= 0, "negative size");
  if (n == 0) return TRL_OK;
  TRL_REQUIRE(mask && a && b && out, "null pointer");
  const int64_t blocks = (n + 255) / 256;
  hipLaunchKernelGGL(select_on_mask_kernel, dim3((unsigned)(blocks > 256 ? 256 : blocks)), dim3(256), 0,
                     (hipStream_t)stream, mask, N, a, b, out, n);
  TRL_LAUNCH_CHECK();
  return TRL_OK;
}
```

Before: 102.1 million.

## Preload hot kernel arguments into SGPRs and reorder kernel signatures accordingly

Adds the compiler flag that preloads the first 14 kernarg dwords into SGPRs. Kernel signatures for GAE, the PPO grad pass, the reduce/Adam step and the value pass are reordered so the arguments needed earliest come first. The PPO grad kernel now takes its leading fields as scalars and reads the remaining struct through the kernarg segment pointer. The reduce/Adam kernel also issues its first fold-row loads before the Adam setup, to hide that load latency. This trims kernel-prologue kernarg load latency in short kernels, at the cost of more complex signatures and raw kernarg offset reads.

Measured after the change: 102.7 million, median of 2. No clear change (+0.5%).

```diff
diff --git a/torchrl_amd/build.py b/torchrl_amd/build.py
--- a/torchrl_amd/build.py
+++ b/torchrl_amd/build.py
@@ -11,7 +11,8 @@
 NOISE_SRC = "trl_noise_ext.cpp"
 SOURCES = ["trl_host.cpp", "trl_mtjump.cpp", "k_gae.hip", "k_gather.hip", "k_ppo.hip", "k_ppo_generic.hip", "k_categorical.hip", "k_gauss_sd.hip", "k_layernorm.hip", "k_vmpo.hip", "k_trpo.hip", "k_rollout.hip", "k_gemm.hip", "k_mlp3.hip", "k_conv1.hip", "k_conv_dx.hip", "k_sac.hip", "k_conv.hip", "k_dqn.hip", "k_bootdqn.hip", "k_norm.hip", "k_frames.hip", "k_comm.hip", "k_peaks.hip"]
 FLAGS = ["--offload-arch=gfx950", "-O3", "-std=c++17", "-fPIC", "-fno-gpu-rdc", "-Wall",
-         "-Wno-unused-function", "-Wno-unused-variable"]
+         "-Wno-unused-function", "-Wno-unused-variable",
+         "-mllvm", "-amdgpu-kernarg-preload-count=14"]
 
 
 def _stale():
diff --git a/torchrl_amd/csrc/k_gae.hip b/torchrl_amd/csrc/k_gae.hip
--- a/torchrl_amd/csrc/k_gae.hip
+++ b/torchrl_amd/csrc/k_gae.hip
@@ -6,9 +6,9 @@
 
 template <int MODE>
 __global__ __launch_bounds__(GAE_THREADS) void gae_scan_kernel(
-    const float* __restrict__ rew, const float* __restrict__ val, const float* __restrict__ term,
-    const float* __restrict__ tl, const float* __restrict__ last_v, const float* __restrict__ last_t, float* __restrict__ adv,
-    float* __restrict__ ret, int T, int N, float gamma, float tau, int tl_filter) {
+    int T, int N, int tl_filter, float gamma, const float* __restrict__ rew, const float* __restrict__ val,
+    const float* __restrict__ term, const float* __restrict__ tl, const float* __restrict__ last_v,
+    const float* __restrict__ last_t, float* __restrict__ adv, float* __restrict__ ret, float tau) {
   constexpr int LDT = T_CHUNK + 1;
   __shared__ float s_a[ENV_TILE * LDT];
   __shared__ float s_c[ENV_TILE * LDT];
@@ -129,9 +129,9 @@
   dim3 grid(trl_ceil_div(N, ENV_TILE)), block(GAE_THREADS);
   hipStream_t s = (hipStream_t)stream;
   if (mode == 0)
-    hipLaunchKernelGGL(gae_scan_kernel<0>, grid, block, 0, s, rew, val, term, tl, last_v, last_t, adv, ret, T, N, gamma, tau, tl_filter);
+    hipLaunchKernelGGL(gae_scan_kernel<0>, grid, block, 0, s, T, N, tl_filter, gamma, rew, val, term, tl, last_v, last_t, adv, ret, tau);
   else
-    hipLaunchKernelGGL(gae_scan_kernel<1>, grid, block, 0, s, rew, val, term, tl, last_v, last_t, adv, ret, T, N, gamma, tau, tl_filter);
+    hipLaunchKernelGGL(gae_scan_kernel<1>, grid, block, 0, s, T, N, tl_filter, gamma, rew, val, term, tl, last_v, last_t, adv, ret, tau);
   TRL_LAUNCH_CHECK();
   return TRL_OK;
 }
diff --git a/torchrl_amd/csrc/k_ppo.hip b/torchrl_amd/csrc/k_ppo.hip
--- a/torchrl_amd/csrc/k_ppo.hip
+++ b/torchrl_amd/csrc/k_ppo.hip
@@ -4,21 +4,26 @@
 #include "trl_head.h"
 #include "trl_comm.h"
 
+struct PpoLead {
+  const int64_t* row_idx;
+  const float *pf_params, *vf_params, *obs;
+  int rows_mb, N;
+  int n_wg, n_pf;
+  int D, A;
+};
+static_assert(sizeof(PpoLead) == 14 * 4, "the leading arguments fill the 14 preloadable dwords");
 struct PpoDev {
-  const float *obs, *acts, *advs, *rets, *old_values, *old_logp;
-  const int64_t* row_idx;
-  int rows_mb, N;
+  const float *acts, *advs, *rets, *old_values, *old_logp;
   const double* adv_raw;
   double n_global;
-  const float *pf_params, *vf_params;
   float clip_para, entropy_coeff;
   int clipped_value_loss, tanh_action;
   int loss_mode;
+  int p_stride;
   float* partial;
   double* scal_partial;
-  int n_wg, n_pf, p_stride;
-  int D, A;
 };
+struct PpoGradArgs { PpoLead lead; PpoDev rest; };
 
 template <int D, int H, int A> struct PpoShape {
   static_assert(H == 64 && D > 16 && D <= 32 && A <= 8, "instantiated for 16 < D <= 32, H == 64, A <= 8");
@@ -75,7 +80,7 @@
 }
 
 template <int D, int H, int A, int ACT, bool IS_PF, bool CONTIG, bool RT, int HEAD = HEAD_GAUSS>
-__device__ void ppo_wave_pass(const PpoDev& a, float* lds, int wg_in_net, int n_wg_net) {
+__device__ void ppo_wave_pass(const PpoLead& h, const PpoDev& rest, float* lds, int wg_in_net, int n_wg_net) {
   using S = typename WvPick<D, H, A, HEAD>::T;
   constexpr bool WIDE = D > 17,
                  CAT = HEAD == HEAD_CAT, SD = HEAD == HEAD_SD,
@@ -84,17 +89,17 @@
   static_assert(!CAT || (IS_PF && RT), "the categorical head is a policy pass of the runtime-dims kernels");
   static_assert(!SD || RT, "the state-dependent-std head belongs to the runtime-dims kernels");
   constexpr int AS = CAT ? 1 : 0;
-  const int Dr = RT ? a.D : D;
-  const int O = IS_PF ? (RT ? a.A : A) : 1;
+  const int Dr = RT ? h.D : D;
+  const int O = IS_PF ? (RT ? h.A : A) : 1;
   const int OH = SDP ? 2 * O : O;
   const int F_W1 = 0, F_B1 = H * Dr, F_W2 = F_B1 + H, F_B2 = F_W2 + H * H, F_W3 = F_B2 + H, F_B3 = F_W3 + OH * H,
             F_LS = F_B3 + OH, F_END = (CAT || SDP) ? F_LS : F_LS + O;
   auto sd_has = [&](int o) -> bool { return (o & 7) < O; };
   auto sd_row = [&](int o) -> int { return o < 8 ? o : O + (o - 8); };
-  const int PS = RT ? a.p_stride : S::P_STRIDE;
   const int tid = threadIdx.x, lane = tid & 63, wave = tid >> 6;
   const int j = lane & 15, g = lane >> 4, i = j;
-  const float* gp = IS_PF ? a.pf_params : a.vf_params;
+  const float* gp = IS_PF ? h.pf_params : h.vf_params;
+  PpoDev a;
   WCLK_DECL
   float* W2F = lds + S::O_W2F;
   float* W2B = lds + S::O_W2B;
@@ -104,15 +109,14 @@
   float* DZ2S = scr + S::O_DZ2;
   float* DOS = scr + S::O_DO;
 
-  const double adv_s1 = IS_PF ? a.adv_raw[0] : 0.0, adv_s2 = IS_PF ? a.adv_raw[1] : 0.0;
-  const int B = a.rows_mb * a.N;
+  const int B = h.rows_mb * h.N;
   const int n_tiles = (B + 15) / 16;
   const int tile_stride = n_wg_net * WV_WAVES;
 
   float xq[5], xtq[4], lq[6];
   float xq2[4], xtq2[4];
   int tile = wg_in_net * WV_WAVES + wave;
-  const int tpr = a.N >> 4;
+  const int tpr = h.N >> 4;
   int p1r = 0, p1c = 0, p2r = 0, p2c = 0, st_r = 0, st_c = 0;
   int64_t ridx1 = 0, ridx2 = 0;
   bool fv[4], fv2[4];
@@ -135,12 +139,12 @@
   };
   auto pos_advance = [&](int& r, int& c) { c += st_c; r += st_r; if (c >= tpr) { c -= tpr; ++r; } };
   auto load_ridx = [&](int r) -> int64_t {
-    const int rr = r < a.rows_mb ? r : 0;
-    return a.row_idx ? a.row_idx[rr] : (int64_t)rr;
+    const int rr = r < h.rows_mb ? r : 0;
+    return h.row_idx ? h.row_idx[rr] : (int64_t)rr;
   };
   auto fetch_contig = [&](int64_t ridx, int r, int c) {
-    const int64_t cell0 = (r < a.rows_mb) ? ridx * a.N + 16 * c : 0;
-    const float* ob = a.obs + cell0 * Dr;
+    const int64_t cell0 = (r < h.rows_mb) ? ridx * h.N + 16 * c : 0;
+    const float* ob = h.obs + cell0 * Dr;
 #pragma unroll
     for (int q = 0; q < 4; ++q) xq[q] = ldb(ob, oxq[q]);
     xq[4] = ldb(ob, ox16);
@@ -165,19 +169,19 @@
       lq[5] = a.clipped_value_loss ? ldb(a.old_values + cell0, os) : 0.0f;
     }
   };
-  auto row_of = [&](int smp, int& e) -> int { const int sm = smp < B ? smp : 0; const int r = sm / a.N; e = sm - r * a.N; return r; };
+  auto row_of = [&](int smp, int& e) -> int { const int sm = smp < B ? smp : 0; const int r = sm / h.N; e = sm - r * h.N; return r; };
   auto fetch_inputs = [&](int64_t p, int s0) {
 #pragma unroll
-    for (int r = 0; r < 4; ++r) xq[r] = a.obs[p * Dr + (fv[r] ? 4 * g + r : 0)];
-    xq[4] = a.obs[p * Dr + (f16 ? 16 : 0)];
+    for (int r = 0; r < 4; ++r) xq[r] = h.obs[p * Dr + (fv[r] ? 4 * g + r : 0)];
+    xq[4] = h.obs[p * Dr + (f16 ? 16 : 0)];
 #pragma unroll
     for (int q = 0; q < 4; ++q) {
       const int sj = 4 * g + q;
       const int64_t pr = __shfl(p, sj, 64);
-      xtq[q] = a.obs[(s0 + sj < B ? pr : 0) * Dr + (jv ? i : 0)];
+      xtq[q] = h.obs[(s0 + sj < B ? pr : 0) * Dr + (jv ? i : 0)];
       if constexpr (WIDE) {
-        xq2[q] = a.obs[p * Dr + (fv2[q] ? 16 + 4 * g + q : 0)];
-        xtq2[q] = a.obs[(s0 + sj < B ? pr : 0) * Dr + (jv2 ? 16 + i : 0)];
+        xq2[q] = h.obs[p * Dr + (fv2[q] ? 16 + 4 * g + q : 0)];
+        xtq2[q] = h.obs[(s0 + sj < B ? pr : 0) * Dr + (jv2 ? 16 + i : 0)];
       }
     }
     if constexpr (IS_PF) {
@@ -199,7 +203,7 @@
   int64_t ridx_nn = 0;
   auto fetch_row = [&](int t) {
     const int r = row_of(t * 16 + j, e_nn);
-    ridx_nn = a.row_idx ? a.row_idx[r] : (int64_t)r;
+    ridx_nn = h.row_idx ? h.row_idx[r] : (int64_t)r;
   };
   auto prefetch_next = [&](int nt) {
     if constexpr (CONTIG) {
@@ -208,7 +212,7 @@
       pos_advance(p2r, p2c);
       ridx2 = load_ridx(p2r);
     } else {
-      const int64_t pn = (nt * 16 + j < B) ? ridx_nn * a.N + e_nn : 0;
+      const int64_t pn = (nt * 16 + j < B) ? ridx_nn * h.N + e_nn : 0;
       fetch_inputs(pn, nt * 16);
       fetch_row(nt + tile_stride);
     }
@@ -253,6 +257,7 @@
     im[k] = gp[ec < F_W2 ? ec : ec + H * H];
   }
   __builtin_amdgcn_sched_barrier(0);
+  a = rest;
   if constexpr (CONTIG) {
     fetch_contig(ridx0, r0, c0);
     p1r = r0; p1c = c0;
@@ -262,10 +267,11 @@
     pos_advance(p2r, p2c);
     ridx2 = load_ridx(p2r);
   } else {
-    const int64_t p0 = (tile * 16 + j < B) ? ridx_nn * a.N + e_nn : 0;
+    const int64_t p0 = (tile * 16 + j < B) ? ridx_nn * h.N + e_nn : 0;
     fetch_inputs(p0, tile * 16);
     fetch_row(tile + tile_stride);
   }
+  const double adv_s1 = IS_PF ? a.adv_raw[0] : 0.0, adv_s2 = IS_PF ? a.adv_raw[1] : 0.0;
 #ifdef TRL_EXP_CLK
   WCLK(22)
   __builtin_amdgcn_s_waitcnt(0);
@@ -761,6 +767,7 @@
     }
     WCLK(7)
     __syncthreads();
+    const int PS = RT ? a.p_stride : S::P_STRIDE;
     float* prow = a.partial + (size_t)wg * a.p_stride;
     auto fold4 = [&](int slot) -> f32x4 {
       const f32x4* p = xch + slot * 64 + lane;
@@ -816,7 +823,7 @@
   WCLK(8)
 #ifdef TRL_EXP_CLK
   __syncthreads();
-  if (tid == 0) for (int ph = 0; ph < 24; ++ph) a.partial[(size_t)wg * a.p_stride + PS - 40 + ph] = clk_acc[ph];
+  if (tid == 0) for (int ph = 0; ph < 24; ++ph) a.partial[(size_t)wg * a.p_stride + (RT ? a.p_stride : S::P_STRIDE) - 40 + ph] = clk_acc[ph];
 #endif
   __syncthreads();
   double* sred = reinterpret_cast<double*>(lds);
@@ -860,7 +867,7 @@
         const double o = sred[WV_WAVES * 8 + w * SD_SCAL + k];
         r = (k < 8 && (k & 2)) ? fmax(r, o) : r + o;
       }
-      a.scal_partial[(size_t)a.n_wg * 8 + (size_t)wg * SD_SCAL + k] = r;
+      a.scal_partial[(size_t)h.n_wg * 8 + (size_t)wg * SD_SCAL + k] = r;
     }
   }
 }
@@ -885,6 +892,32 @@
   for (int k = 0; k < RED_DEPTH; ++k) acc[k] = 0.0f;
   if (in_range) {
     for (; w < nrow; w += RED_DEPTH * RED_WAVES) {
+      float v[RED_DEPTH];
+#pragma unroll
+      for (int k = 0; k < RED_DEPTH; ++k) v[k] = (w + RED_WAVES * k < nrow) ? src[(size_t)(w + RED_WAVES * k) * p_stride] : 0.0f;
+#pragma unroll
+      for (int k = 0; k < RED_DEPTH; ++k) acc[k] += v[k];
+    }
+  }
+  return fold_chain_tree(acc);
+}
+__device__ __forceinline__ void fold_rows_request(const float* __restrict__ src, int nrow, int p_stride, int w,
+                                                  float (&v0)[RED_DEPTH]) {
+#pragma unroll
+  for (int k = 0; k < RED_DEPTH; ++k) {
+    const int r = w + RED_WAVES * k;
+    v0[k] = src[(size_t)(r < nrow ? r : nrow - 1) * p_stride];
+  }
+}
+__device__ __forceinline__ float fold_rows_finish(const float* __restrict__ src, int nrow, int p_stride, int w, bool in_range,
+                                                  const float (&v0)[RED_DEPTH]) {
+  float acc[RED_DEPTH];
+#pragma unroll
+  for (int k = 0; k < RED_DEPTH; ++k) acc[k] = 0.0f;
+#pragma unroll
+  for (int k = 0; k < RED_DEPTH; ++k) acc[k] += (in_range && w + RED_WAVES * k < nrow) ? v0[k] : 0.0f;
+  if (in_range) {
+    for (w += RED_DEPTH * RED_WAVES; w < nrow; w += RED_DEPTH * RED_WAVES) {
       float v[RED_DEPTH];
 #pragma unroll
       for (int k = 0; k < RED_DEPTH; ++k) v[k] = (w + RED_WAVES * k < nrow) ? src[(size_t)(w + RED_WAVES * k) * p_stride] : 0.0f;
@@ -994,19 +1027,27 @@
   }
 }
 
+struct FoldSrc { const float* src; int nrow; bool in_range; };
+__device__ __forceinline__ FoldSrc fold_src(const float* __restrict__ partial, int n_wg, int n_pf, int p_stride, int p_pf,
+                                            int p_vf, int net, int bx) {
+  const int row0 = net == 0 ? 0 : n_pf, p = bx * RED_CHUNK + (int)(threadIdx.x & 63);
+  return {partial + (size_t)row0 * p_stride + p, net == 0 ? n_pf : n_wg - n_pf, p < (net == 0 ? p_pf : p_vf)};
+}
 template <int HEAD = HEAD_GAUSS>
 __device__ __forceinline__ float ppo_reduce_block(const float* __restrict__ partial,
                                                   const double* __restrict__ scal, int n_wg, int n_pf,
                                                   int p_stride, int p_pf, int p_vf,
                                                   const float* __restrict__ logstd, int n_act,
                                                   float* __restrict__ grads, double* __restrict__ info,
-                                                  int net, int bx, bool stats) {
+                                                  int net, int bx, bool stats, const float (*v0)[RED_DEPTH] = nullptr) {
   __shared__ float s_acc[RED_WAVES][RED_CHUNK];
   const int row0 = net == 0 ? 0 : n_pf, nrow = net == 0 ? n_pf : n_wg - n_pf;
   const int lane = threadIdx.x & 63, wave = threadIdx.x >> 6;
   const int p = bx * RED_CHUNK + lane;
   const int pn = net == 0 ? p_pf : p_vf;
-  s_acc[wave][lane] = fold_rows_wave(partial + (size_t)row0 * p_stride + p, nrow, p_stride, wave, p < pn);
+  const FoldSrc f = fold_src(partial, n_wg, n_pf, p_stride, p_pf, p_vf, net, bx);
+  s_acc[wave][lane] = v0 ? fold_rows_finish(f.src, f.nrow, p_stride, wave, f.in_range, *v0)
+                         : fold_rows_wave(f.src, f.nrow, p_stride, wave, f.in_range);
   __syncthreads();
   float gval = 0.0f;
   if (wave == 0 && p < pn) {
@@ -1115,17 +1156,23 @@
 
 template <bool LOOP, int HEAD = HEAD_GAUSS>
 __global__ __launch_bounds__(64 * RED_WAVES, 4) void ppo_reduce_adam_kernel(const float* __restrict__ partial,
-                                                              const double* __restrict__ scal, int n_wg, int n_pf,
-                                                              int p_stride, int p_pf, int p_vf,
+                                                              float* __restrict__ ws, int n_wg, int n_pf,
+                                                              int p_stride, int p_pf, int p_vf, int only_net,
+                                                              int device_state, int xrank,
+                                                              const double* __restrict__ scal,
                                                               const float* __restrict__ logstd, int n_act,
                                                               float* __restrict__ grads, double* __restrict__ info,
-                                                              AdamDev a, float* __restrict__ ws, unsigned epoch,
-                                                              int device_state, int xrank, XrArgs xr, int only_net) {
+                                                              unsigned epoch, AdamDev a, XrArgs xr) {
   __shared__ float s_coef[2];
   __shared__ float s_hyper[4];
   const int tid = threadIdx.x, lane = tid & 63, wave = tid >> 6;
   const int nb = (p_stride + RED_CHUNK - 1) / RED_CHUNK, grid = gridDim.x, job0 = only_net == 1 ? nb : 0;
   const int n_jobs = only_net >= 0 ? job0 + nb : 2 * nb, blk = job0 + (int)blockIdx.x;
+  float v0[RED_DEPTH];
+  if constexpr (!LOOP) {
+    const FoldSrc f = fold_src(partial, n_wg, n_pf, p_stride, p_pf, p_vf, blk / nb, blk % nb);
+    fold_rows_request(f.src, f.nrow, p_stride, wave, v0);
+  }
   double* bpow = reinterpret_cast<double*>(ws + 4);
   double b1p = 0.0, b2p = 0.0;
   float lr0 = 0.0f, lr1 = 0.0f;
@@ -1144,7 +1191,8 @@
   for (int j = blk; j < (LOOP ? n_jobs : blk + 1); j += LOOP ? grid : 1) {
     const int net = j / nb, bx = j - net * nb;
     if (j != blk) __syncthreads();
-    float gval = ppo_reduce_block<HEAD>(partial, scal, n_wg, n_pf, p_stride, p_pf, p_vf, logstd, n_act, grads, info, net, bx, bx == nb - 1);
+    float gval = ppo_reduce_block<HEAD>(partial, scal, n_wg, n_pf, p_stride, p_pf, p_vf, logstd, n_act, grads, info, net, bx, bx == nb - 1,
+                                        LOOP ? nullptr : &v0);
     if (wave == 0) {
       if (xrank) {
         const int pe = bx * RED_CHUNK + lane;
@@ -1231,15 +1279,20 @@
 }
 
 template <int D, int H, int A, int ACT, bool CONTIG, bool RT, int HEAD = HEAD_GAUSS>
-__global__ __launch_bounds__(WV_THREADS, 1) void ppo_grad_wave_kernel(PpoDev a) {
+__global__ __launch_bounds__(WV_THREADS, 1) void ppo_grad_wave_kernel(const int64_t* row_idx, const float* pf_params,
+                                                                     const float* vf_params, const float* obs, int rows_mb,
+                                                                     int N, int n_wg, int n_pf, int Dr, int Ar, PpoDev rest) {
   static_assert(HEAD == HEAD_GAUSS || RT, "categorical / state-dependent-std head: runtime-dims tiles");
   constexpr int HEAD_VF = HEAD == HEAD_CAT ? HEAD_GAUSS : HEAD;
   extern __shared__ __attribute__((aligned(16))) float lds[];
+  const PpoLead h{row_idx, pf_params, vf_params, obs, rows_mb, N, n_wg, n_pf, Dr, Ar};
+  const PpoDev& a = *reinterpret_cast<const PpoDev*>(
+      (const char*)__builtin_amdgcn_kernarg_segment_ptr() + offsetof(PpoGradArgs, rest));
 #ifdef TRL_CHAIN_CLK
   const unsigned long long clk0 = wall_clock64();
 #endif
-  if ((int)blockIdx.x < a.n_pf) ppo_wave_pass<D, H, A, ACT, true, CONTIG, RT, HEAD>(a, lds, blockIdx.x, a.n_pf);
-  else                          ppo_wave_pass<D, H, A, ACT, false, CONTIG, RT, HEAD_VF>(a, lds, blockIdx.x - a.n_pf, a.n_wg - a.n_pf);
+  if ((int)blockIdx.x < h.n_pf) ppo_wave_pass<D, H, A, ACT, true, CONTIG, RT, HEAD>(h, a, lds, blockIdx.x, h.n_pf);
+  else                          ppo_wave_pass<D, H, A, ACT, false, CONTIG, RT, HEAD_VF>(h, a, lds, blockIdx.x - h.n_pf, h.n_wg - h.n_pf);
 #ifdef TRL_CHAIN_CLK
   __syncthreads();
   if (threadIdx.x == 0) {
@@ -1304,7 +1357,7 @@
 static_assert(WvShapeSD<32, 64, 8>::LDS_FLOATS * sizeof(float) <= 160 * 1024, "the wide tile's exchange area fits the LDS");
 
 template <int D, int H, int A, int ACT, bool CONTIG, bool RT, int HEAD>
-static int launch_ppo_v(const PpoDev& d, hipStream_t s) {
+static int launch_ppo_v(const PpoLead& h, const PpoDev& d, hipStream_t s) {
   using S = typename WvPick<D, H, A, HEAD>::T;
   const size_t lds = S::LDS_FLOATS * sizeof(float);
   static bool attr_set = false;
@@ -1314,13 +1367,14 @@
     if (e != hipSuccess) { trl_set_error("ppo_grad: hipFuncSetAttribute: %s", hipGetErrorString(e)); return (int)e; }
     attr_set = true;
   }
-  hipLaunchKernelGGL((ppo_grad_wave_kernel<D, H, A, ACT, CONTIG, RT, HEAD>), dim3(d.n_wg), dim3(WV_THREADS), lds, s, d);
+  hipLaunchKernelGGL((ppo_grad_wave_kernel<D, H, A, ACT, CONTIG, RT, HEAD>), dim3(h.n_wg), dim3(WV_THREADS), lds, s,
+                     h.row_idx, h.pf_params, h.vf_params, h.obs, h.rows_mb, h.N, h.n_wg, h.n_pf, h.D, h.A, d);
   TRL_LAUNCH_CHECK();
   return TRL_OK;
 }
 template <int D, int H, int A, int ACT, bool RT, int HEAD = HEAD_GAUSS>
-static int launch_ppo(const PpoDev& d, hipStream_t s) {
-  return (d.N % 16 == 0) ? launch_ppo_v<D, H, A, ACT, true, RT, HEAD>(d, s) : launch_ppo_v<D, H, A, ACT, false, RT, HEAD>(d, s);
+static int launch_ppo(const PpoLead& h, const PpoDev& d, hipStream_t s) {
+  return (h.N % 16 == 0) ? launch_ppo_v<D, H, A, ACT, true, RT, HEAD>(h, d, s) : launch_ppo_v<D, H, A, ACT, false, RT, HEAD>(h, d, s);
 }
 
 extern "C" int trl_ppo_wg_split(int D, int H, int A, int n_tiles, int n_wg) {
@@ -1365,24 +1419,25 @@
               "partial rows must be 16-byte aligned, parameter blocks 4-byte aligned");
   TRL_REQUIRE(head != HEAD_GAUSS || !SHAPE_IS(17, 64, 6) || (((uintptr_t)p->pf_params | (uintptr_t)p->vf_params) & 15) == 0,
               "parameter blocks of the benchmark shape must be 16-byte aligned");
+  PpoLead h;
+  h.row_idx = p->row_idx; h.pf_params = p->pf_params; h.vf_params = p->vf_params; h.obs = p->obs;
+  h.rows_mb = p->rows_mb; h.N = p->N; h.n_wg = p->n_wg; h.n_pf = resolve_pf_wgs(p->n_wg, p->n_wg_pf);
+  h.D = D; h.A = A;
   PpoDev d;
-  d.obs = p->obs; d.acts = p->acts; d.advs = p->advs; d.rets = p->rets; d.old_values = p->old_values;
-  d.old_logp = p->old_logp; d.row_idx = p->row_idx; d.rows_mb = p->rows_mb; d.N = p->N;
-  d.adv_raw = p->adv_raw; d.n_global = p->n_global; d.pf_params = p->pf_params; d.vf_params = p->vf_params;
+  d.acts = p->acts; d.advs = p->advs; d.rets = p->rets; d.old_values = p->old_values;
+  d.old_logp = p->old_logp; d.adv_raw = p->adv_raw; d.n_global = p->n_global;
   d.clip_para = p->clip_para; d.entropy_coeff = p->entropy_coeff;
   d.clipped_value_loss = p->clipped_value_loss; d.tanh_action = p->tanh_action;
   d.loss_mode = reinforce ? TRL_LOSS_A2C : p->loss_mode;
-  d.partial = p->partial; d.scal_partial = p->scal_partial; d.n_wg = p->n_wg;
-  d.n_pf = resolve_pf_wgs(p->n_wg, p->n_wg_pf);
-  d.D = D; d.A = A;
+  d.partial = p->partial; d.scal_partial = p->scal_partial;
   hipStream_t s = (hipStream_t)stream;
   d.p_stride = ppo_stride_for(D, H, A, head);
   if (head == HEAD_CAT) d.tanh_action = 0;
   if (head == HEAD_GAUSS && SHAPE_IS(17, 64, 6))
-    return p->act == TRL_ACT_TANH ? launch_ppo<17, 64, 6, TRL_ACT_TANH, false>(d, s) : launch_ppo<17, 64, 6, TRL_ACT_RELU, false>(d, s);
+    return p->act == TRL_ACT_TANH ? launch_ppo<17, 64, 6, TRL_ACT_TANH, false>(h, d, s) : launch_ppo<17, 64, 6, TRL_ACT_RELU, false>(h, d, s);
   return with_head(head, [&](auto hd) {
     return with_tile_act(D, p->act, [&](auto tile, auto act) {
-      return launch_ppo<decltype(tile)::value, 64, 8, decltype(act)::value, true, decltype(hd)::value>(d, s);
+      return launch_ppo<decltype(tile)::value, 64, 8, decltype(act)::value, true, decltype(hd)::value>(h, d, s);
     });
   });
 }
@@ -1482,8 +1537,8 @@
   with_head(head, [&](auto hd) {
     auto launch = [&](auto loop) {
       hipLaunchKernelGGL((ppo_reduce_adam_kernel<decltype(loop)::value, decltype(hd)::value>), dim3(grid), dim3(64 * RED_WAVES), 0,
-                         (hipStream_t)stream, partial, scal_partial, n_wg, n_pf, ps, p_pf, p_vf, logstd, A, grads, info, d,
-                         workspace, epoch, adam->device_state, xr ? 1 : 0, xr ? *xr : none, only_net);
+                         (hipStream_t)stream, partial, workspace, n_wg, n_pf, ps, p_pf, p_vf, only_net, adam->device_state,
+                         xr ? 1 : 0, scal_partial, logstd, A, grads, info, epoch, d, xr ? *xr : none);
     };
     if (grid == jobs) launch(std::false_type{}); else launch(std::true_type{});
     return 0;
diff --git a/torchrl_amd/csrc/k_rollout.hip b/torchrl_amd/csrc/k_rollout.hip
--- a/torchrl_amd/csrc/k_rollout.hip
+++ b/torchrl_amd/csrc/k_rollout.hip
@@ -594,8 +594,13 @@
 };
 
 template <int D, int H, int ACT, bool RT = false>
-__global__ __launch_bounds__(VP_THREADS, RT ? 1 : 2) void value_pass_kernel(ValueDev a) {
+__global__ __launch_bounds__(VP_THREADS, RT ? 1 : 2) void value_pass_kernel(const float* vf_params, const float* obs, float* values,
+                                                                            const float* next_obs, int rows, int top, int N,
+                                                                            int n_steps, int Drt, float discount, float* rewards,
+                                                                            float* boot, uint32_t* pub_dst, const uint32_t* pub_src,
+                                                                            int64_t pub_words) {
   static_assert(H == 64 && D > 16 && D <= 32, "instantiated for 16 < D <= 32, H == 64");
+  const ValueDev a{vf_params, obs, next_obs, values, rewards, rows, top, N, n_steps, discount, boot, pub_dst, pub_src, pub_words, Drt};
   constexpr bool WIDE = D > 17;
   static_assert(!WIDE || RT, "the wide tile exists as a runtime-dims instantiation only");
   constexpr int XK = WIDE ? 8 : 5;
@@ -777,7 +782,8 @@
                d.pub_dst, d.pub_src, d.pub_words, d.D};
     const int64_t n_tiles = ((int64_t)d.n_steps * d.N + 15) / 16;
     const int grid = (int)(n_tiles / 4 + 1 < 512 ? n_tiles / 4 + 1 : 512);
-    hipLaunchKernelGGL((value_pass_kernel<D, H, ACT, RT>), dim3(grid), dim3(VP_THREADS), 0, s, v);
+    hipLaunchKernelGGL((value_pass_kernel<D, H, ACT, RT>), dim3(grid), dim3(VP_THREADS), 0, s, v.vf_params, v.obs, v.values, v.next_obs,
+                       v.rows, v.top, v.N, v.n_steps, v.D, v.discount, v.rewards, v.boot, v.pub_dst, v.pub_src, v.pub_words);
     TRL_LAUNCH_CHECK();
   }
   return TRL_OK;
```
